# The-Learning-And-Vision-Atelier-LAVA/BUFFER

Measured on AMD Instinct MI355X. Metric: registration pairs/sec, higher is better.
Workload: dtype f32

## Files before the change

buffer_amd/_lib.py:

```python
import ctypes as C
import os

_HERE = os.path.dirname(os.path.abspath(__file__))
LIB_PATH = os.environ.get("BUF_LIB_PATH") or os.path.join(_HERE, "libbuffer_hip.so")

BUF_OK = 0


class BufferHipError(RuntimeError):
    pass


class buf_grid_t(C.Structure):
    _fields_ = [
        ("ws", C.c_void_p), ("ws_bytes", C.c_size_t),
        ("ns", C.c_int), ("nb", C.c_int),
        ("cells_per_elem", C.c_int64),
        ("radius", C.c_float),
        ("supports", C.c_void_p),
        ("desc", C.c_void_p), ("s_off", C.c_void_p), ("table", C.c_void_p),
        ("sorted", C.c_void_p), ("order", C.c_void_p), ("scan_tmp", C.c_void_p),
    ]


class buf_voxel_map_t(C.Structure):
    _fields_ = [
        ("buf", C.c_void_p), ("buf_bytes", C.c_size_t),
        ("nclouds", C.c_int), ("nrows", C.c_int), ("n", C.c_int),
        ("max_cells", C.c_int64),
        ("voxel", C.c_double), ("epsilon", C.c_double),
        ("clouds", C.c_void_p), ("table", C.c_void_p), ("rows", C.c_void_p), ("keys", C.c_void_p), ("row_off", C.c_void_p),
    ]


_lib = None

_vp, _i, _f, _i64, _sz = C.c_void_p, C.c_int, C.c_float, C.c_int64, C.c_size_t

_SIGNATURES = {
    "buf_last_error": (C.c_char_p, []),
    "buf_version": (_i, []),
    "buf_device_count": (_i, []),
    "buf_timing_enable": (None, [_i]),
    "buf_timing_collect": (C.c_longlong, [C.POINTER(C.c_double), C.POINTER(C.c_double)]),
    "buf_timing_collect_kernel": (C.c_longlong, [_i, C.POINTER(C.c_double), C.POINTER(C.c_double)]),
    "buf_grid_default_cells": (_i64, [_i, _i]),
    "buf_grid_ws_bytes": (_sz, [_i, _i, _i64]),
    "buf_grid_cell_dims": (_i, [C.POINTER(C.c_double), _f, _i64, C.POINTER(C.c_double), C.POINTER(C.c_int)]),
    "buf_grid_build": (_i, [C.POINTER(buf_grid_t), _vp, _i, _vp, _i, _f, _i64, _vp, _sz, _vp]),
    "buf_grid_query": (_i, [C.POINTER(buf_grid_t), _vp, _i, _vp, _vp, _f, _i, _vp, _vp, _vp, _vp, _vp]),
    "buf_radius_neighbors": (_i, [_vp, _i, _vp, _i, _vp, _vp, _i, _f, _i, _vp, _vp, _vp, _vp, _sz, _vp]),
    "buf_grid_subsample_ws_bytes": (_sz, [_i, _i, _i64, _i]),
    "buf_grid_subsample_batch": (_i, [_vp, _i, _vp, _i, _f, _i, _vp, _i, _vp, _vp, _vp, _vp, _i64, _vp, _sz, _vp]),
    "buf_fps_ws_bytes": (_sz, [_i, _i]),
    "buf_fps": (_i, [_vp, _i, _i, _i, _vp, _vp, _sz, _vp]),
    "buf_gather": (_i, [_vp, _vp, _i, _i, _i, _i, _vp, _vp]),
    "buf_group": (_i, [_vp, _vp, _i, _i, _i, _i, _i, _vp, _vp]),
    "buf_ball_query": (_i, [_vp, _vp, _i, _i, _i, _f, _i, _vp, _vp]),
    "buf_three_nn": (_i, [_vp, _vp, _i, _i, _i, _vp, _vp, _vp]),
    "buf_select_patches": (_i, [_vp, _vp, _i, _i, _f, _i, _vp, _vp]),
    "buf_select_patches_batched_ws_bytes": (_sz, [_i, _i]),
    "buf_select_patches_batched": (_i, [_vp, _vp, _i, _vp, _i, _f, _i, _vp, _vp, _sz, _vp]),
    "buf_permute_clouds": (_i, [_vp, _vp, _vp, _i, _vp, _vp]),
    "buf_compact_ws_bytes": (_sz, [_i]),
    "buf_compact_greater": (_i, [_vp, _i, _i, _f, _vp, _vp, _vp, _sz, _vp]),
    "buf_knn_ws_bytes": (_sz, [_i, _i, _i]),
    "buf_knn1_ws_bytes": (_sz, [_i, _i, _i]),
    "buf_knn": (_i, [_vp, _vp, _i, _i, _i, _i, _i, _vp, _vp, _vp, _sz, _vp]),
    "buf_fps_ragged": (_i, [_vp, _vp, _i, _i, _vp, _vp, _sz, _vp]),
    "buf_svd3x3_batched": (_i, [_vp, _i, _vp, _vp, _vp, _vp]),
    "buf_vn_gather_block": (_i, [_vp, _vp, _vp, _vp, _i, _i, _i, _i, _i, _i, _f, _vp, _vp, _vp, _vp, _f, _vp, _vp]),
    "buf_vn_gather_pre_supported": (_i, [_i, _i, _i]),
    "buf_vn_gather_pre_ws_bytes": (_sz, [_i, _i]),
    "buf_vn_gather_block_pre": (_i, [_vp, _vp, _vp, _vp, _i, _i, _i, _i, _i, _f, _vp, _vp, _vp, _vp, _f, _vp, _vp, _sz, _vp]),
    "buf_vn_pointwise": (_i, [_vp, _vp, _i, _i, _i, _vp, _i, _i, _i, _vp, _vp, _vp, _vp, _f, _vp, _vp, _vp]),
    "buf_gather_max": (_i, [_vp, _vp, _i, _i, _i, _i, _vp, _vp]),
    "buf_vn_std": (_i, [_vp, _vp, _i, _i, _vp, _vp]),
    "buf_score_head_ws_bytes": (_sz, [_i, _i]),
    "buf_score_head": (_i, [_vp, _i, _vp, _i, _vp, _vp, _vp, _vp, _f, _vp, _vp, _vp, _vp, _f, _vp, _vp, _vp, _vp, _vp, _i, _vp, _vp, _i, _f,
                            _vp, _vp, _sz, _vp]),
    "buf_patch_voxelize_ws_bytes": (_sz, [_i]),
    "buf_patch_voxelize": (_i, [_vp, _vp, _i, _i, _f, _vp, _i, _i, _vp, _f, _i, _vp, _vp, _vp, _vp, _vp, _vp, _vp,
                                _vp, _vp, _sz, _vp]),
    "buf_cylindrical_net_wg": (_i, [_vp, _i, _vp, _vp, _vp, _vp, _vp, _vp, _vp]),
    "buf_cylindrical_net_wg_form": (_i, [_vp, _i, _vp, _vp, _vp, _vp, _vp, _i, _vp, _vp]),
    "buf_cylindrical_net_wg_all": (_i, [_vp, _i, _vp, _vp, _vp, _vp, _vp, _vp, _vp, _vp]),
    "buf_cylindrical_net_wg_all_flags": (_i, [_vp, _vp, _vp, _vp]),
    "buf_cylindrical_net_wg_supports": (_i, [_vp, _vp]),
    "buf_cylindrical_net_wg_flags": (_i, [_vp, _vp, _vp]),
    "buf_cylindrical_net_split_safe": (_i, [_vp, _i, _vp, _vp, _vp, _vp, _vp, _vp, _vp, _vp, _vp, _vp, _vp, _vp]),
    "buf_cylindrical_net_split_safe_form": (_i, [_vp, _i, _vp, _vp, _vp, _vp, _vp, _vp, _i, _vp, _vp, _vp, _vp, _vp, _vp]),
    "buf_cost_volume_net_split_safe": (_i, [_vp, _vp, _i, _vp, _vp, _i, _vp, _vp, _vp, _vp, _vp, _vp, _vp, _vp]),
    "buf_cylindrical_net_split_safe_all": (_i, [_vp, _i, _vp, _vp, _vp, _vp, _vp, _vp, _vp, _vp, _vp, _vp, _vp, _vp, _vp]),
    "buf_cylindrical_net_split": (_i, [_vp, _i, _vp, _vp, _vp, _vp, _vp, _vp, _vp, _vp]),
    "buf_cylindrical_net_split_head": (_i, [_vp, _i, _vp, _vp, _vp, _vp, _vp, _vp, _vp, _vp, _vp, _vp]),
    "buf_split_gemm_count": (C.c_longlong, [_i, _i, _i, _i]),
    "buf_split_tile_gemm": (_i, [_vp, _i, _i, _i, _i, _vp]),
    "buf_cost_volume_net_split": (_i, [_vp, _vp, _i, _vp, _vp, _vp, _vp, _vp]),
    "buf_cost_volume_net_split_gather": (_i, [_vp, _i, _vp, _vp, _i, _vp, _vp, _vp, _vp, _vp]),
    "buf_split_filter_count": (C.c_longlong, [_i, _i]),
    "buf_split_tile_filters": (_i, [_vp, _i, _i, _vp]),
    "buf_winograd_tile_weights": (_i, [_vp, _i, _i, _vp]),
    "buf_winograd_f24_tile_weights": (_i, [_vp, _i, _i, _vp]),
    "buf_winograd_group": (_i, [_i, _i]),
    "buf_cost_winograd_group": (_i, [_i]),
    "buf_winograd_tile_filters": (_i, [_vp, _i, _i, _i, _i, _vp]),
    "buf_voxel_downsample_ws_bytes": (_sz, [_i, _i64]),
    "buf_voxel_downsample": (_i, [_vp, _vp, _i, _i, C.c_double, _vp, _vp, _vp, _i64, _vp, _sz, _vp]),
    "buf_voxel_downsample_batch_ws_bytes": (_sz, [_i, _i, _i64]),
    "buf_voxel_downsample_batch": (_i, [_vp, _i, _i, _vp, _i, C.c_double, _vp, _vp, _i64, _vp, _sz, _vp]),
    "buf_knn_normals": (_i, [_vp, _i, _vp, _i, _vp, _i, _i, _vp, _i, _vp, _vp, _vp]),
    "buf_icp_ws_bytes": (_sz, [_i, _i, _i, _i]),
    "buf_icp_batched": (_i, [_vp, _vp, _vp, _vp, _vp, _i, _i, _f, _vp, _i, C.c_double, C.c_double, _vp, _vp, _vp, _vp, _vp,
                             _vp, _sz, _vp]),
    "buf_gicp_batched": (_i, [_vp, _vp, _vp, _vp, _vp, _vp, _i, _f, C.c_double, _vp, _i, C.c_double, C.c_double, _vp, _vp, _vp, _vp,
                              _vp, _vp, _sz, _vp]),
    "buf_pair_stats_ws_bytes": (_sz, [_i, _i, _i, _i, _i64]),
    "buf_pair_stats": (_i, [_vp, _vp, _i, _vp, _vp, _i, _vp, _f, _i64, _vp, _vp, _vp, _vp, _sz, _vp]),
    "buf_pose_graph_ws_bytes": (_sz, [_i, _i, _i, _i]),
    "buf_pose_graph_optimize": (_i, [_vp, _vp, _i, _vp, _vp, _vp, _vp, _vp, _vp, _vp, _vp, _i, C.c_double, C.c_double, C.c_double,
                                     _vp, _vp, _vp, _vp, _vp, _sz, _vp]),
    "buf_fpfh_ws_bytes": (_sz, [_i]),
    "buf_fpfh": (_i, [_vp, _vp, _i, _vp, _i, _i, _vp, _vp, _vp, _sz, _vp]),
    "buf_fgr_ws_bytes": (_sz, [_i, _i, _i]),
    "buf_fgr_batched": (_i, [_vp, _vp, _vp, _vp, _vp, _vp, _i, _vp, C.c_double, _i, _i, C.c_double, C.c_double, _i, C.c_double, _i, _i,
                             _vp, _vp, _vp, _vp, _vp, _sz, _vp]),
    "buf_sc2_ws_bytes": (_sz, [_vp, _i, _i]),
    "buf_sc2_batched": (_i, [_vp, _vp, _vp, _vp, _vp, _vp, _i, C.c_double, C.c_double, C.c_double, _i, _i, C.c_double, _i, _i,
                             _vp, _vp, _vp, _vp, _vp, _vp, _vp, _vp, _sz, _vp]),
    "buf_clique_ws_bytes": (_sz, [_vp, _i, _i, _i]),
    "buf_clique_batched": (_i, [_vp, _vp, _vp, _vp, _vp, _vp, _i, C.c_double, C.c_double, C.c_double, C.c_double, _i, _i, C.c_double, _i,
                                _i, _vp, _vp, _vp, _vp, _vp, _vp, _vp, _vp, _vp, _vp, _vp, _sz, _vp]),
    "buf_voxel_map_bytes": (_sz, [_i, _i, _i64]),
    "buf_voxel_map_ws_bytes": (_sz, [_i, _i, _i64]),
    "buf_voxel_map_build": (_i, [C.POINTER(buf_voxel_map_t), _vp, _vp, _vp, _i, C.c_double, C.c_double, _i64, _vp, _sz, _vp, _sz, _vp]),
    "buf_voxel_map_export": (_i, [C.POINTER(buf_voxel_map_t), _i, _vp, _vp, _vp, _vp, _vp, _vp]),
    "buf_vgicp_ws_bytes": (_sz, [_i, _i]),
    "buf_vgicp_batched": (_i, [C.POINTER(buf_voxel_map_t), _vp, _vp, _vp, _vp, _i, _i, _vp, _i, C.c_double, C.c_double, _vp, _vp, _vp,
                               _vp, _vp, _vp, _sz, _vp]),
    "buf_match_metrics":(_i, [_vp, _vp, _vp, _i, _i, _vp, _vp, _f, _f, _f, _vp, _vp, _vp]),
    "buf_row_linear": (_i, [_vp, _i, _i, _i, _vp, _vp, _i, _vp, _vp]),
    "buf_segment_instance_norm_ws_bytes": (_sz, [_i, _i]),
    "buf_segment_instance_norm": (_i, [_vp, _i, _i, _vp, _i, _f, _vp, _vp, _sz, _vp]),
    "buf_descriptor_head": (_i, [_vp, _i, _vp, _vp, _vp, _vp]),
    "buf_cost_volume_net": (_i, [_vp, _vp, _i, _vp, _vp, _vp, _vp]),
    "buf_cost_volume_net_gather": (_i, [_vp, _i, _vp, _vp, _i, _vp, _vp, _vp, _vp]),
    "buf_hypotheses_score": (_i, [_vp, _vp, _vp, _vp, _vp, _i, _i, _f, _vp, _vp, _vp, _vp, _vp, _vp]),
    "buf_ransac_ws_bytes": (_sz, [_i]),
    "buf_ransac_kabsch": (_i, [_vp, _vp, _vp, _i, _i, C.c_uint64, _f, _f, _vp, _vp, _vp, _sz, _vp]),
    "buf_ransac_masked_ws_bytes": (_sz, [_i, _i]),
    "buf_ransac_kabsch_masked": (_i, [_vp, _vp, _vp, _i, _i, C.c_uint64, _f, _f, _vp, _vp, _vp, _sz, _vp]),
    "buf_post_refine": (_i, [_vp, _vp, _vp, _i, _f, _i, _vp, _vp, _vp]),
    "buf_recover_poses_ws_bytes": (_sz, [_i, _i, _i]),
    "buf_recover_poses_batched": (_i, [_vp, _vp, _vp, _vp, _vp, _vp, _i, _vp, _i, _f, _i, _f, _f, _f, _i, _vp, _vp, _sz, _vp]),
}


def exported_symbols():
    return sorted(_SIGNATURES)


def lib():
    global _lib
    if _lib is None:
        if not os.path.exists(LIB_PATH):
            raise BufferHipError(
                f"{LIB_PATH} is missing: build it with `python -m buffer_amd.build` "
                "(hipcc --offload-arch=gfx950). buffer_amd has no CPU fallback.")
        import torch
        l = C.CDLL(LIB_PATH)
        for name, (res, args) in _SIGNATURES.items():
            fn = getattr(l, name)
            fn.restype = res
            fn.argtypes = args
        _lib = l
    return _lib


def check(rc, what=""):
    if rc != BUF_OK:
        msg = lib().buf_last_error().decode(errors="replace")
        raise BufferHipError(f"{what} failed ({rc}): {msg}")
```

buffer_amd/csrc/buffer_hip.hip:

```cpp
#include <stdlib.h>
#include "core.hip"
#include "radius.hip"
#include "icp.hip"
#include "pairstats.hip"
#include "posegraph.hip"
#include "metrics.hip"
#include "subsample.hip"
#include "pointops.hip"
#include "vn.hip"
#include "voxelize.hip"
#include "registration.hip"
#include "convnet.hip"
#include "convnet_h3.hip"
#include "costnet_h3.hip"
#include "preprocess.hip"
#include "convnet_wg.hip"
#include "convnet_w24.hip"
#include "convnet_w24k.hip"
#include "convnet_w24p.hip"
#include "convnet_w24a.hip"
#include "costnet.hip"
#include "split_safe.hip"
#include "fpfh.hip"
#include "fgr.hip"
#include "sc2.hip"
#include "clique.hip"
#include "vgicp.hip"
```

buffer_amd/csrc/convnet_w24.hip:

```cpp
#include "common.h"

#define W24_WSTRIDE 768
#define W24_SET_F22(CIN) (16 * 128 * (CIN))

__device__ __forceinline__ void w24_tile(int li, int& ty, int& tx)
{
    const bool last = li == 15;
    ty = last ? 3 : li / 5;
    tx = last ? 4 : li - 5 * ty;
}

__device__ __forceinline__ unsigned w24_row_addr(unsigned act_addr, int a, int li, int lk)
{
    int ty, tx;
    w24_tile(li, ty, tx);
    const int row = 2 * ty - 1 + a;
    return act_addr + 4u * (unsigned)(lk * WG_CS + ((row >= 0 && row <= 6) ? row * WG_ROW + 4 * tx : WG_ZERO));
}

struct W24AddrPark { float a[4]; };
__device__ __forceinline__ void w24_park_addresses(const float* act, int li, int lk, W24AddrPark& pk)
{
    const unsigned act_addr = (unsigned)(size_t)(__attribute__((address_space(3))) const float*)act;
#pragma unroll
    for (int a = 0; a < 4; a++) {
        const unsigned v = w24_row_addr(act_addr, a, li, lk);
        asm volatile("v_accvgpr_write_b32 %0, %1" : "=a"(pk.a[a]) : "v"(v));
    }
}

#define W24_LOAD(DST, A0, A1_, OFS)                                                                       \
    {                                                                                                     \
        _Pragma("unroll") for (int q_ = 0; q_ < 3; q_++) {                                                \
            DST[q_] = *(wg_lds_f2)(size_t)((A0) + (OFS) + 8 * q_);                                        \
            asm volatile("" : "+v"(A0));                                                                  \
        }                                                                                                 \
        _Pragma("unroll") for (int q_ = 0; q_ < 3; q_++) {                                                \
            DST[3 + q_] = *(wg_lds_f2)(size_t)((A1_) + (OFS) + 8 * q_);                                   \
            asm volatile("" : "+v"(A1_));                                                                 \
        }                                                                                                 \
    }

__device__ __forceinline__ wgf2 w24_ldw2(__amdgpu_buffer_rsrc_t rs, unsigned uniform_float_ofs, unsigned lane_byte_ofs)
{
    return __builtin_bit_cast(wgf2, __builtin_amdgcn_raw_buffer_load_b64(rs, lane_byte_ofs, uniform_float_ofs * 4, 0));
}

#define W24_U(n, k, j) ((j) < 3 ? W4[n][k][j] : ((j) == 5 ? W4[n][k][3] : W2[n][k][(j) - 3]))

template <int I, bool PRIMED, int INEXT>
__device__ __forceinline__ void w24_pass(unsigned (&RA)[4], __amdgpu_buffer_rsrc_t rs, unsigned wp, unsigned wp_next, unsigned lofs4, unsigned lofs2,
                                         int niter, wgf4 (&W4)[2][2], wgf2 (&W2)[2][2], wgf4 (&acc)[2][6], wgf2 (&D)[2][6])
{
    constexpr int A1 = wg_a1(I), A2 = wg_a2(I);
    constexpr int A1N = wg_a1(INEXT < 0 ? 0 : INEXT), A2N = wg_a2(INEXT < 0 ? 0 : INEXT);
    float V[2][6];
    unsigned P0 = RA[A1], P1 = RA[A2];
    if constexpr (!PRIMED) {
        W24_LOAD(D[0], P0, P1, 0)
        W24_LOAD(D[1], P0, P1, WG_KSTEP)
    }
#define W24_XFORM(BUF)                                                                                    \
    {                                                                                                     \
        float r_[6];                                                                                      \
        _Pragma("unroll") for (int b = 0; b < 6; b++) {                                                   \
            const float da_ = D[BUF][b >> 1][b & 1];                                                      \
            const float db_ = D[BUF][3 + (b >> 1)][b & 1];                                                \
            r_[b] = I == 1 ? wg_add(da_, db_) : (I == 2 ? wg_sub(db_, da_) : wg_sub(da_, db_));           \
        }                                                                                                 \
        const float c_ = wg_sub(r_[4], r_[2]), e_ = wg_sub(r_[3], r_[1]);                                 \
        const float a_ = __builtin_fmaf(-4.f, r_[2], r_[4]), b_ = __builtin_fmaf(-4.f, r_[1], r_[3]);     \
        V[BUF][0] = __builtin_fmaf(4.f, r_[0], __builtin_fmaf(-4.f, r_[2], c_));                          \
        V[BUF][1] = wg_add(a_, b_); V[BUF][2] = wg_sub(a_, b_);                                           \
        V[BUF][3] = __builtin_fmaf(2.f, e_, c_); V[BUF][4] = __builtin_fmaf(-2.f, e_, c_);                \
        V[BUF][5] = __builtin_fmaf(-4.f, e_, wg_sub(r_[5], r_[3]));                                       \
    }
    W24_XFORM(0)
#pragma unroll 1
    for (int it = 0; it < niter; it++) {
        const bool more = it + 1 < niter;
        const unsigned wcur = wp + 4 * it * W24_WSTRIDE;
        const unsigned wn = more ? wcur + 4 * W24_WSTRIDE : wp_next;
        const unsigned adv = more ? 4u * WG_KSTEP : 0u;
        __builtin_amdgcn_sched_barrier(0);
#pragma unroll
        for (int s = 0; s < 4; s++) {
            if (s < 2) W24_LOAD(D[s & 1], P0, P1, (s + 2) * WG_KSTEP)
            else {
                if (s == 2) { P0 += adv; P1 += adv; }
                if constexpr (INEXT >= 0) {
                    unsigned q0 = more ? P0 : RA[A1N], q1 = more ? P1 : RA[A2N];
                    W24_LOAD(D[s & 1], q0, q1, (s - 2) * WG_KSTEP)
                } else
                    W24_LOAD(D[s & 1], P0, P1, (s - 2) * WG_KSTEP)
            }
            __builtin_amdgcn_sched_barrier(0);
#pragma unroll
            for (int n = 0; n < 2; n++)
#pragma unroll
                for (int j = 0; j < 6; j++)
                    acc[n][j] = __builtin_amdgcn_mfma_f32_16x16x4f32(W24_U(n, s & 1, j), V[s & 1][j], acc[n][j], 0, 0, 0);
            __builtin_amdgcn_sched_barrier(0);
            W24_XFORM((s + 1) & 1)
#pragma unroll
            for (int n = 0; n < 2; n++) {
                const unsigned o = s < 2 ? wcur + (s + 2) * W24_WSTRIDE : wn + (s - 2) * W24_WSTRIDE;
                W4[n][s & 1] = wg_ldw(rs, o + n * 256, lofs4);
                W2[n][s & 1] = w24_ldw2(rs, o + 512 + n * 128, lofs2);
            }
            __builtin_amdgcn_sched_barrier(0);
        }
    }
#undef W24_XFORM
}

template <bool NOBIAS = false>
__device__ __forceinline__ void w24_round(unsigned (&RA)[4], __amdgpu_buffer_rsrc_t rs, unsigned wp, unsigned wp_after, unsigned lofs4, unsigned lofs2,
                                          int niter, unsigned pstride, const float* __restrict__ bias_lane, wgf4 (&W4)[2][2], wgf2 (&W2)[2][2],
                                          wgf4 (&Y)[2][2][4])
{
    using std::integral_constant;
    wgf2 D[2][6];
    wgf4 bv[2];
#pragma unroll
    for (int n = 0; n < 2; n++) {
        if constexpr (NOBIAS) bv[n] = bias_lane ? *reinterpret_cast<const wgf4*>(bias_lane + n * 16) : (wgf4){ 0.f, 0.f, 0.f, 0.f };
        else bv[n] = *reinterpret_cast<const wgf4*>(bias_lane + n * 16);
    }
    wgf4 acc[2][6];
    float zero = 0.f;
    asm volatile("" : "+v"(zero));
#pragma unroll
    for (int n = 0; n < 2; n++)
#pragma unroll
        for (int j = 0; j < 6; j++) acc[n][j] = (wgf4){ zero, zero, zero, zero };
    auto run = [&](auto ic) __attribute__((always_inline)) {
        constexpr int I = decltype(ic)::value;
        constexpr int INEXT = I == 3 ? 0 : I + 1;
        if constexpr (I == 1) {
#pragma unroll
            for (int n = 0; n < 2; n++) acc[n][1] += bv[n];
        }
        constexpr int ICHAIN = (INEXT != 0 && wg_chains(I)) ? INEXT : -1;
        w24_pass<I, wg_chains(I - 1), ICHAIN>(RA, rs, wp + I * pstride, INEXT == 0 ? wp_after : wp + (I + 1) * pstride, lofs4, lofs2, niter, W4, W2, acc, D);
        __builtin_amdgcn_sched_barrier(0);
#pragma unroll
        for (int n = 0; n < 2; n++) {
            wgf4 f[4];
#pragma unroll
            for (int r = 0; r < 4; r++) {
                const float p = acc[n][1][r] + acc[n][2][r], q = acc[n][1][r] - acc[n][2][r];
                const float t = acc[n][3][r] + acc[n][4][r], d = acc[n][3][r] - acc[n][4][r];
                f[0][r] = acc[n][0][r] + p + t;
                f[1][r] = __builtin_fmaf(2.f, d, q);
                f[2][r] = __builtin_fmaf(4.f, t, p);
                f[3][r] = __builtin_fmaf(8.f, d, q) + acc[n][5][r];
            }
#pragma unroll
            for (int v = 0; v < 4; v++) {
                if constexpr (I == 0) Y[n][1][v] = f[v];
                else if constexpr (I == 1) {
#pragma unroll
                    for (int r = 0; r < 4; r++) Y[n][1][v][r] = __builtin_fmaf(2.f, f[v][r], -Y[n][1][v][r]);
                }
                else if constexpr (I == 2) Y[n][0][v] = f[v];
                else Y[n][1][v] -= f[v];
                if constexpr (I == 2) asm volatile("" : "+v"(Y[n][0][v]));
                else asm volatile("" : "+v"(Y[n][1][v]));
            }
        }
    };
    run(integral_constant<int, 0>{});
    run(integral_constant<int, 1>{});
    run(integral_constant<int, 2>{});
    run(integral_constant<int, 3>{});
}

template <bool NOBIAS = false>
__device__ __forceinline__ void w24_round_direct(unsigned row5, __amdgpu_buffer_rsrc_t rs, unsigned wp, unsigned lofs, int niter, unsigned pstride,
                                                 const float* __restrict__ bias_lane, wgf4 (&W4)[2][2], wgf4 (&Y)[2])
{
    constexpr int wstride = W24_WSTRIDE;
    wgf4 Wr[3][2][2];
#pragma unroll
    for (int n = 0; n < 2; n++)
#pragma unroll
        for (int k = 0; k < 2; k++) {
            Wr[0][n][k] = W4[n][k];
            Wr[1][n][k] = wg_ldw(rs, wp + pstride + n * 256 + k * wstride, lofs);
            Wr[2][n][k] = wg_ldw(rs, wp + 2 * pstride + n * 256 + k * wstride, lofs);
        }
    float X[2][6];
    unsigned pa = row5;
    WG_LOADD(X[0], pa, 0)
    WG_LOADD(X[1], pa, WG_KSTEP)
    wgf4 acc[2][3];
    float zero = 0.f;
    asm volatile("" : "+v"(zero));
#pragma unroll
    for (int n = 0; n < 2; n++) {
        acc[n][0] = (wgf4){ zero, zero, zero, zero };
        acc[n][1] = (wgf4){ zero, zero, zero, zero };
        if constexpr (NOBIAS) acc[n][2] = bias_lane ? *reinterpret_cast<const wgf4*>(bias_lane + n * 16) : (wgf4){ zero, zero, zero, zero };
        else acc[n][2] = *reinterpret_cast<const wgf4*>(bias_lane + n * 16);
    }
    float G[2][6];
#define W24_TAPS(SLOT)                                                                                    \
    _Pragma("unroll") for (int n = 0; n < 2; n++) {                                                       \
        const wgf4 u0_ = Wr[0][n][SLOT], u1_ = Wr[1][n][SLOT], u2_ = Wr[2][n][SLOT];                      \
        const float d1_ = wg_sub(u1_[1], u2_[1]), d2_ = wg_sub(u1_[2], u2_[2]);                           \
        G[n][0] = u0_[0]; G[n][1] = wg_sub(u0_[1], u0_[2]); G[n][2] = u0_[3];                             \
        G[n][3] = wg_sub(u1_[0], u2_[0]); G[n][4] = wg_sub(d1_, d2_); G[n][5] = wg_sub(u1_[3], u2_[3]);   \
    }
#define W24_RELOAD(SLOT, OFS)                                                                             \
    _Pragma("unroll") for (int n = 0; n < 2; n++)                                                         \
        _Pragma("unroll") for (int blk = 0; blk < 3; blk++) Wr[blk][n][SLOT] = wg_ldw(rs, (OFS) + blk * pstride + n * 256, lofs);
    W24_TAPS(0)
    W24_RELOAD(0, wp + 2 * wstride)
#pragma unroll 1
    for (int it = 0; it < niter; it++) {
        const bool more = it + 1 < niter;
        const unsigned wcur = wp + 4 * it * wstride;
        const unsigned wn = more ? wcur + 4 * wstride : wp;
        const unsigned adv = more ? 4u * WG_KSTEP : 0u;
        __builtin_amdgcn_sched_barrier(0);
#pragma unroll
        for (int s = 0; s < 4; s++) {
#pragma unroll
            for (int b = 0; b < 3; b++)
#pragma unroll
                for (int a = 0; a < 2; a++)
#pragma unroll
                    for (int n = 0; n < 2; n++)
                        acc[n][b] = __builtin_amdgcn_mfma_f32_16x16x4f32(G[n][a * 3 + b], X[s & 1][a * 3 + b], acc[n][b], 0, 0, 0);
            __builtin_amdgcn_sched_barrier(0);
            if (s < 2) WG_LOADD(X[s & 1], pa, (s + 2) * WG_KSTEP)
            else {
                if (s == 2) pa += adv;
                WG_LOADD(X[s & 1], pa, (s - 2) * WG_KSTEP)
            }
            __builtin_amdgcn_sched_barrier(0);
            W24_TAPS((s + 1) & 1)
            if (s == 0) W24_RELOAD(1, wcur + 3 * wstride)
            else W24_RELOAD((s + 1) & 1, wn + (s - 1) * wstride)
            __builtin_amdgcn_sched_barrier(0);
        }
    }
#undef W24_TAPS
#undef W24_RELOAD
#pragma unroll
    for (int n = 0; n < 2; n++)
#pragma unroll
        for (int r = 0; r < 4; r++) Y[n][r] = __builtin_fmaf(4.f, acc[n][0][r], __builtin_fmaf(-3.f, acc[n][1][r], acc[n][2][r]));
}

__device__ __forceinline__ void w24_store_tile(const wgf4 (&Yt)[2][4], int nt, int relu, float* __restrict__ act, int li, int lk)
{
    const int n0 = nt * 16 + lk * 4;
    const float lo = relu ? 0.f : -__builtin_inff();
    int ty, tx;
    w24_tile(li, ty, tx);
#pragma unroll
    for (int u = 0; u < 2; u++) {
        const int row = 2 * ty + u;
        const bool ok = row < 7;
        int pos[4];
#pragma unroll
        for (int v = 0; v < 4; v++) pos[v] = ok ? row * WG_ROW + 4 * tx + 1 + v : WG_ZERO + 4;
        const int h0 = (ok && tx == 0) ? row * WG_ROW + 21 : WG_ZERO + 4;
        const int h1 = (ok && tx == 4) ? row * WG_ROW : WG_ZERO + 5;
        float* p = act + n0 * WG_CS;
#pragma unroll
        for (int r = 0; r < 4; r++) {
            float val[4];
#pragma unroll
            for (int v = 0; v < 4; v++) { val[v] = fmaxf(Yt[u][v][r], lo); p[r * WG_CS + pos[v]] = val[v]; }
            p[r * WG_CS + h0] = val[0]; p[r * WG_CS + h1] = val[3];
        }
    }
}

__device__ __forceinline__ void w24_layer_pair(float* __restrict__ act, const float* __restrict__ wt, const float* __restrict__ bias, int cin, int relu,
                                               int pair, const WgAddrPark& pk, const W24AddrPark& pk24)
{
    act[(threadIdx.x >> 1) * WG_CS + WG_ZERO + 4 + (threadIdx.x & 1)] = 0.f;
    __syncthreads();
    int lane = threadIdx.x & (WAVE - 1);
    asm volatile("" : "+v"(lane));
    const int lk = lane >> 4;
    const int k4 = cin >> 2;
    unsigned RA[4];
#pragma unroll
    for (int a = 0; a < 4; a++) asm volatile("v_accvgpr_read_b32 %0, %1" : "=v"(RA[a]) : "a"(pk24.a[a]));
    const unsigned row5 = wg_parked(pk, 2, 0);
    const __amdgpu_buffer_rsrc_t rs = wg_weights(wt);
    const unsigned pstride = (unsigned)(k4 * W24_WSTRIDE);
    const unsigned wp = (unsigned)pair * 4 * pstride;
    const unsigned lofs4 = lane * 16, lofs2 = lane * 8;
    const float* bv = bias + (2 * pair) * 16 + lk * 4;
    wgf4 W4[2][2];
    wgf2 W2[2][2];
#pragma unroll
    for (int n = 0; n < 2; n++)
#pragma unroll
        for (int k = 0; k < 2; k++) {
            W4[n][k] = wg_ldw(rs, wp + k * W24_WSTRIDE + n * 256, lofs4);
            W2[n][k] = w24_ldw2(rs, wp + k * W24_WSTRIDE + 512 + n * 128, lofs2);
        }
    wgf4 Y[2][2][4];
    float park[2][36];
    w24_round(RA, rs, wp, wp, lofs4, lofs2, k4 >> 2, pstride, bv, W4, W2, Y);
#pragma unroll
    for (int n = 0; n < 2; n++)
#pragma unroll
        for (int q = 0; q < 32; q++) asm volatile("v_accvgpr_write_b32 %0, %1" : "=a"(park[n][q]) : "v"(Y[n][q >> 4][(q >> 2) & 3][q & 3]));
    wgf4 Yb[2];
    w24_round_direct(row5, rs, wp, lofs4, k4 >> 2, pstride, bv, W4, Yb);
#pragma unroll
    for (int n = 0; n < 2; n++)
#pragma unroll
        for (int q = 0; q < 4; q++) asm volatile("v_accvgpr_write_b32 %0, %1" : "=a"(park[n][32 + q]) : "v"(Yb[n][q]));
    __syncthreads();
    int lane_s = threadIdx.x & (WAVE - 1);
    asm volatile("" : "+v"(lane_s));
#pragma unroll
    for (int n = 0; n < 2; n++) {
#pragma unroll
        for (int q = 0; q < 32; q++) asm volatile("v_accvgpr_read_b32 %0, %1" : "=v"(Y[n][q >> 4][(q >> 2) & 3][q & 3]) : "a"(park[n][q]));
#pragma unroll
        for (int q = 0; q < 4; q++) asm volatile("v_accvgpr_read_b32 %0, %1" : "=v"(Yb[n][q]) : "a"(park[n][32 + q]));
        w24_store_tile(Y[n], 2 * pair + n, relu, act, lane_s & 15, lane_s >> 4);
        wg_store_row6<false>(Yb[n], 2 * pair + n, relu, act, nullptr, lane_s & 15, lane_s >> 4);
    }
}

__device__ __forceinline__ void cyl_net_w24_body(const float* __restrict__ x, const CylWgParams& P, float* __restrict__ y, float* __restrict__ lds)
{
    float* act = lds;
    const int patch = blockIdx.x;
    const int w = __builtin_amdgcn_readfirstlane(threadIdx.x / WAVE);
    wg_load_input(x, P, act, patch);
    WgAddrPark pk;
    W24AddrPark pk24;
    {
        int lane0 = threadIdx.x & (WAVE - 1);
        asm volatile("" : "+v"(lane0));
        wg_park_addresses(act, lane0 & 15, lane0 >> 4, pk);
        w24_park_addresses(act, lane0 & 15, lane0 >> 4, pk24);
    }
#pragma unroll 1
    for (int l = 0; l < WG_LAYERS; l++) {
        const int cin = P.cin[l], cout = P.cout[l];
        if (cout == 128) w24_layer_pair(act, P.wt[l], P.bias[l], cin, P.relu[l], w, pk, pk24);
        else if (cout == 64) wg_layer_msplit(act, P.wt[l], P.bias[l], cin, cout, P.relu[l], w, pk);
        else if (l < WG_LAYERS - 1) wg_layer_mksplit<false>(act, nullptr, P.wt[l], P.bias[l], cin, cout, P.relu[l], w, pk);
        else wg_layer_mksplit<true>(act, y + (size_t)patch * cout * 140, P.wt[l], P.bias[l], cin, cout, P.relu[l], w, pk);
        __syncthreads();
    }
}

__global__ void __launch_bounds__(WG_THREADS, 2) k_cyl_net_w24(const float* __restrict__ x, CylWgParams P, float* __restrict__ y)
{
    extern __shared__ float lds[];
    cyl_net_w24_body(x, P, y, lds);
}

__global__ void __launch_bounds__(WG_THREADS, 2) k_cyl_net_w24_rerun(const float* __restrict__ x, CylWgParams P, float* __restrict__ y)
{
    extern __shared__ float lds[];
    if (P.only_if[blockIdx.x] == 0) return;
    cyl_net_w24_body(x, P, y, lds);
}

extern "C" int buf_winograd_f24_tile_weights(const float* w_host, int cout, int cin, float* out_host)
{
    BUF_REQUIRE(w_host && out_host, BUF_EINVAL, "buf_winograd_f24_tile_weights: null argument");
    BUF_REQUIRE(cout > 0 && cin > 0 && cout % 32 == 0 && cin % 4 == 0, BUF_EINVAL, "buf_winograd_f24_tile_weights: widths %d -> %d", cin, cout);
    static const double G2[4][3] = { { 1, 0, 0 }, { .5, .5, .5 }, { .5, -.5, .5 }, { 0, 0, 1 } };
    const double s6 = 1.0 / 6, s12 = 1.0 / 12, s24 = 1.0 / 24;
    const double G4[6][3] = { { .25, 0, 0 }, { -s6, -s6, -s6 }, { -s6, s6, -s6 }, { s24, s12, s6 }, { s24, -s12, s6 }, { 0, 0, 1 } };
    const int k4 = cin / 4;
    for (int o = 0; o < cout; o++)
        for (int c = 0; c < cin; c++) {
            const float* g = w_host + ((size_t)o * cin + c) * 9;
            const int n = o / 16, lane = (c % 4) * 16 + o % 16;
            for (int i = 0; i < 4; i++) {
                float* blk = out_host + (((size_t)(n / 2) * 4 + i) * k4 + c / 4) * W24_WSTRIDE;
                for (int j = 0; j < 6; j++) {
                    double u = 0;
                    for (int a = 0; a < 3; a++)
                        for (int b = 0; b < 3; b++) u += G2[i][a] * (double)g[3 * a + b] * G4[j][b];
                    if (j == 3 || j == 4) blk[512 + (n % 2) * 128 + lane * 2 + (j - 3)] = (float)u;
                    else blk[(n % 2) * 256 + lane * 4 + (j == 5 ? 3 : j)] = (float)u;
                }
            }
        }
    return BUF_OK;
}

static int w24_check_flags(const int* cin, const int* cout, const int* relu)
{
    for (int l = 0; l < WG_LAYERS; l++) {
        BUF_REQUIRE(relu[l] >= 0 && relu[l] <= (BUF_CYL_F24K | WG_F24_FLAG | 1), BUF_EINVAL,
                    "buf_cylindrical_net_wg: layer %d has the relu word %d (bit 0: ReLU, bits 1 and 2: the F(2x4) flags, nothing above)", l, relu[l]);
        BUF_REQUIRE(!(relu[l] & BUF_CYL_F24K) || (cout[l] == 64 && cin[l] % 64 == 0), BUF_EINVAL,
                    "buf_cylindrical_net_wg: the K-split F(2x4) flag (bit 2) goes only on layers with 64 output channels and Cin %% 64 == 0 "
                    "(layer %d: %d -> %d, flags %d)", l, cin[l], cout[l], relu[l]);
        BUF_REQUIRE(((relu[l] & WG_F24_FLAG) != 0) == (cout[l] == 128), BUF_EINVAL,
                    "buf_cylindrical_net_wg: the F(2x4) flag goes on every layer with 128 output channels and on no other (layer %d: %d -> %d, flags %d)",
                    l, cin[l], cout[l], relu[l]);
    }
    return BUF_OK;
}

extern "C" int buf_cylindrical_net_wg_flags(const int* cin_host, const int* cout_host, const int* relu_host)
{
    BUF_REQUIRE(cin_host && cout_host && relu_host, BUF_EINVAL, "buf_cylindrical_net_wg_flags: null argument");
    if (int rc = wg_check_widths(cin_host, cout_host)) return rc;
    for (int l = 0; l < WG_LAYERS; l++)
        if (relu_host[l] >= 2) return w24_check_flags(cin_host, cout_host, relu_host);
    return BUF_OK;
}

#define BUF_CYL_FORM_LIBRARY BUF_CYL_FORM_PASS_SPLIT
static int w24k_launch(const float* x, int npatch, CylWgParams P, float* y, void* stream);
static int w24p_launch(const float* x, int npatch, CylWgParams P, float* y, void* stream);
static int w24_launch(const float* x, int npatch, CylWgParams P, float* y, void* stream, int form)
{
    if (int rc = w24_check_flags(P.cin, P.cout, P.relu)) return rc;
    bool ksplit = false;
    for (int l = 0; l < WG_LAYERS; l++) {
        if (P.relu[l] & WG_F24_FLAG) P.wt[l] += W24_SET_F22(P.cin[l]);
        ksplit |= (P.relu[l] & BUF_CYL_F24K) != 0;
        P.relu[l] &= ~WG_F24_FLAG;
    }
    if (form == BUF_CYL_FORM_DEFAULT) form = BUF_CYL_FORM_LIBRARY;
    if (ksplit) return form == BUF_CYL_FORM_PASS_SPLIT ? w24p_launch(x, npatch, P, y, stream) : w24k_launch(x, npatch, P, y, stream);
    size_t lds = sizeof(float) * WG_BUF;
    static LdsGrant grant, grant_rerun;
    if (int rc = P.only_if ? grant_dynamic_lds((const void*)k_cyl_net_w24_rerun, lds, grant_rerun) : grant_dynamic_lds((const void*)k_cyl_net_w24, lds, grant)) return rc;
    double macs = 0;
    for (int l = 0; l < WG_LAYERS; l++) macs += 9.0 * P.cin[l] * P.cout[l];
    TimedSpan span;
    bool timed = !P.only_if && timing_begin((hipStream_t)stream, &span, 2.0 * 140 * macs * npatch, BUF_TIMED_CYL_NET);
    if (P.only_if) k_cyl_net_w24_rerun<<<npatch, WG_THREADS, lds, (hipStream_t)stream>>>(x, P, y);
    else k_cyl_net_w24<<<npatch, WG_THREADS, lds, (hipStream_t)stream>>>(x, P, y);
    if (timed) timing_end((hipStream_t)stream, &span);
    BUF_LAUNCH_CHECK();
    return BUF_OK;
}
```

buffer_amd/csrc/costnet.hip:

```cpp
#include "common.h"
#include <type_traits>

#define CV_THREADS 256
#define CV_BUF 20480
#define CV_LAYERS 10
#define CV_C32 36
#define CV_C64 68
#define CV_C128 132

typedef float cvx4 __attribute__((ext_vector_type(4)));

#define CV_SCHED_TAIL(NMFMA, NMEM)                                                      \
    _Pragma("unroll") for (int i_ = 0; i_ < (NMFMA); i_++) {                            \
        __builtin_amdgcn_sched_group_barrier(0x008, 1, 0);                              \
        __builtin_amdgcn_sched_group_barrier(0x006, 4, 0);                              \
        __builtin_amdgcn_sched_group_barrier(0x120, ((NMEM) + (NMFMA) - 1) / (NMFMA), 0); \
    }
typedef const __attribute__((address_space(1))) cvx4* cv_gptr;

struct CostNetParams {
    const float* wt[CV_LAYERS];
    const float* bias[CV_LAYERS];
    const long long* s_rows;
    const long long* t_rows;
    int row_floats, chan_floats, skip_floats;
    const int* only_if;
};

template <int MT, int NT, int D, int TOTAL, typename Loader>
__device__ __forceinline__ void cv_gemm_static(cvx4 (&acc)[MT][NT], Loader& L, const float* __restrict__ wl, int ntot)
{
    float a[D][4][MT], b[D][4][NT];
#define CVS_LOAD(SLOT, G)                                                                                 \
    {                                                                                                     \
                           \
        cv_gptr wg_ = (cv_gptr)(wl + (size_t)(G) * ntot * 256);                                           \
        asm volatile("" : "+v"(wg_));                                                                     \
        _Pragma("unroll") for (int u = 0; u < NT; u++) {                                                  \
            const cvx4 bv_ = wg_[u * 64];                                                                 \
            _Pragma("unroll") for (int p = 0; p < 4; p++) b[SLOT][p][u] = bv_[p];                         \
        }                                                                                                 \
        L.load(a[SLOT], (G));                                                                             \
    }
#pragma unroll
    for (int i = 0; i < D - 1; i++) CVS_LOAD(i, i)
#pragma unroll
    for (int g = 0; g < TOTAL; g++) {
        __builtin_amdgcn_sched_barrier(0);
        if (g + D - 1 < TOTAL) CVS_LOAD((g + D - 1) % D, g + D - 1)
#pragma unroll
        for (int p = 0; p < 4; p++)
#pragma unroll
            for (int t = 0; t < MT; t++)
#pragma unroll
                for (int u = 0; u < NT; u++)
                    acc[t][u] = __builtin_amdgcn_mfma_f32_16x16x4f32(a[g % D][p][t], b[g % D][p][u], acc[t][u], 0, 0, 0);
        CV_SCHED_TAIL(4 * MT * NT, MT + NT)
    }
#undef CVS_LOAD
}

#define CVA_SP 0
#define CVA_TP 4320
#define CVA_SM 16376
#define CVA_TB 18536
#define CVA_XC 0
#define CW_RSX 18
#define CW_CSX 112
#define CVA_XCH (96 * CW_CSX)
static_assert(CVA_XCH + 2 * 8 * 64 * 4 <= CVA_SM, "the exchange slots fit between the chunk and the layer-0 maps");

struct SLoader {
    const float* base;
    __device__ __forceinline__ void load(float (&a)[4][1], int g) const
    {
        const int tap = g >> 1, cg = g & 1, dk = tap / 5, e2 = tap - dk * 5;
        const cvx4 v = *reinterpret_cast<const cvx4*>(base + (dk * 24 + e2) * CV_C32 + cg * 16);
#pragma unroll
        for (int p = 0; p < 4; p++) a[p][0] = v[p];
    }
};

struct TLoader {
    const float* base;
    __device__ __forceinline__ void load(float (&a)[4][1], int g) const
    {
        const int tap = g >> 1, cg = g & 1, dk = tap / 3, dl = tap - dk * 3;
        const cvx4 v = *reinterpret_cast<const cvx4*>(base + (dk * 20 + dl) * CV_C32 + cg * 16);
#pragma unroll
        for (int p = 0; p < 4; p++) a[p][0] = v[p];
    }
};

template <int MT, int NT, int CIN, int COUT, int WIN, int KW, bool INPLACE>
__device__ __forceinline__ void cv_conv_layer(const float* in, float* out, const float* __restrict__ wt,
                                              const float* __restrict__ bias, int nt0, bool relu)
{
    constexpr int WOUT = WIN - KW + 1, P = WOUT * WOUT, GPT = CIN / 16, TAPS = KW * KW, NTOT = COUT / 16;
    constexpr int CSI = CIN + 4, CSO = COUT + 4;
    static_assert(GPT % 2 == 0, "two pipeline slots alternate per channel group");
    int lane = threadIdx.x & (WAVE - 1);
    asm volatile("" : "+v"(lane));
    const int li = lane & 15, lk = lane >> 4;
    const float* pa[MT];
#pragma unroll
    for (int t = 0; t < MT; t++) {
        int m = t * 16 + li;
        m = m < P ? m : P - 1;
        pa[t] = in + ((m / WOUT) * WIN + (m % WOUT)) * CSI + lk * 4;
    }
    const float* wl = wt + ((size_t)nt0 * 64 + lane) * 4;
    cvx4 acc[MT][NT];
#pragma unroll
    for (int u = 0; u < NT; u++) {
        const float bv = bias[(nt0 + u) * 16 + li];
#pragma unroll
        for (int t = 0; t < MT; t++) acc[t][u] = (cvx4){ bv, bv, bv, bv };
    }
    float a[2][4][MT], b[2][4][NT];
#define CVC_LOAD(SLOT, PTRS, WTAP, CG)                                                                    \
    {                                                                                                     \
        cv_gptr wg_ = (cv_gptr)((WTAP) + (size_t)(CG) * NTOT * 256);                                      \
        asm volatile("" : "+v"(wg_));                                                                     \
        _Pragma("unroll") for (int u = 0; u < NT; u++) {                                                  \
            const cvx4 bv_ = wg_[u * 64];                                                                 \
            _Pragma("unroll") for (int p = 0; p < 4; p++) b[SLOT][p][u] = bv_[p];                         \
        }                                                                                                 \
        _Pragma("unroll") for (int t = 0; t < MT; t++) {                                                  \
            const cvx4 av_ = *reinterpret_cast<const cvx4*>(PTRS[t] + (CG) * 16);                         \
            _Pragma("unroll") for (int p = 0; p < 4; p++) a[SLOT][p][t] = av_[p];                         \
        }                                                                                                 \
    }
    const float* cur[MT];
    const float* nxt[MT];
#pragma unroll
    for (int t = 0; t < MT; t++) cur[t] = pa[t];
    const float* wcur = wl;
    CVC_LOAD(0, cur, wcur, 0)
#pragma unroll 1
    for (int tap = 0; tap < TAPS; tap++) {
        const int tn = tap + 1 < TAPS ? tap + 1 : tap;
        const int offn = ((tn / KW) * WIN + (tn % KW)) * CSI;
#pragma unroll
        for (int t = 0; t < MT; t++) nxt[t] = pa[t] + offn;
        const float* wnxt = wl + (size_t)tn * GPT * NTOT * 256;
#pragma unroll
        for (int cg = 0; cg < GPT; cg++) {
            __builtin_amdgcn_sched_barrier(0);
            if (cg + 1 < GPT) CVC_LOAD((cg + 1) & 1, cur, wcur, cg + 1)
            else              CVC_LOAD((cg + 1) & 1, nxt, wnxt, 0)
    #pragma unroll
            for (int p = 0; p < 4; p++)
#pragma unroll
                for (int t = 0; t < MT; t++)
#pragma unroll
                    for (int u = 0; u < NT; u++)
                        acc[t][u] = __builtin_amdgcn_mfma_f32_16x16x4f32(a[cg & 1][p][t], b[cg & 1][p][u], acc[t][u], 0, 0, 0);
            CV_SCHED_TAIL(4 * MT * NT, MT + NT)
        }
#pragma unroll
        for (int t = 0; t < MT; t++) cur[t] = nxt[t];
        wcur = wnxt;
    }
#undef CVC_LOAD
    if constexpr (INPLACE) __syncthreads();
#pragma unroll
    for (int u = 0; u < NT; u++) {
        const int n = (nt0 + u) * 16 + li;
#pragma unroll
        for (int t = 0; t < MT; t++)
#pragma unroll
            for (int r = 0; r < 4; r++) {
                const int m = t * 16 + lk * 4 + r;
                float v = acc[t][u][r];
                if (relu) v = fmaxf(v, 0.f);
                if (m < P) out[m * CSO + n] = v;
            }
    }
}

template <int HIN, int TYPM>
__device__ __forceinline__ bool cw_tile(int t, int li, int& ty, int& tx)
{
    constexpr int NTY = (HIN - 2) / 2;
    const int q = li / NTY;
    ty = t * TYPM + q; tx = li - q * NTY;
    return q < TYPM && ty < NTY;
}

template <int HIN, int TYPM, int RSO, int CSO, bool POSMAJOR>
__device__ __forceinline__ void cw_store_tile(const wgf4 (&Yt)[2][2], int t, int nt, float* __restrict__ out, int li, int lk)
{
    int ty, tx;
    if (!cw_tile<HIN, TYPM>(t, li, ty, tx)) return;
    const int n0 = nt * 16 + lk * 4;
#pragma unroll
    for (int u = 0; u < 2; u++) {
        const int row = 2 * ty + u, col = 2 * tx;
        if constexpr (POSMAJOR) {
#pragma unroll
            for (int v = 0; v < 2; v++) {
                wgf4 y;
#pragma unroll
                for (int r = 0; r < 4; r++) y[r] = fmaxf(Yt[u][v][r], 0.f);
                *reinterpret_cast<wgf4*>(out + (row * (HIN - 2) + col + v) * CSO + n0) = y;
            }
        } else {
#pragma unroll
            for (int r = 0; r < 4; r++)
                *reinterpret_cast<wgf2*>(out + (n0 + r) * CSO + row * RSO + col) = (wgf2){ fmaxf(Yt[u][0][r], 0.f), fmaxf(Yt[u][1][r], 0.f) };
        }
    }
}

template <int HIN, int RS, int CS, int TYPM, int CIN, int NN, int MT, int MT2, int RSO, int CSO, bool POSMAJOR>
__device__ __forceinline__ void cw_layer(float* __restrict__ map, const float* __restrict__ wt, const float* __restrict__ bias, int ng, int t0)
{
    static_assert(MT >= 1 && MT <= 2 && MT2 >= 0 && MT2 <= 1 && RS % 2 == 0 && CS % 2 == 0, "");
    constexpr unsigned KSTEP = 16u * CS;
    constexpr int k4 = CIN / 4, wstride = 256 * NN;
    int lane = threadIdx.x & (WAVE - 1);
    asm volatile("" : "+v"(lane));
    const int li = lane & 15, lk = lane >> 4;
    const unsigned base = (unsigned)(size_t)(__attribute__((address_space(3))) const float*)map;
    auto rows = [&](int t, unsigned (&ra)[4]) __attribute__((always_inline)) {
        int ty, tx;
        if (!cw_tile<HIN, TYPM>(t, li, ty, tx)) { ty = 0; tx = 0; }
#pragma unroll
        for (int a = 0; a < 4; a++) ra[a] = base + 4u * (unsigned)(lk * CS + (2 * ty + a) * RS + 2 * tx);
    };
    unsigned RA[3][4];
    rows(t0, RA[0]);
    rows(t0 + (MT > 1 ? 1 : 0), RA[1]);
    rows(t0, RA[2]);
    const __amdgpu_buffer_rsrc_t rs = wg_weights(wt);
    const unsigned wp = (unsigned)ng * (CIN * NN * 256);
    const unsigned lofs = lane * 16;
    const float* bl = bias + ng * NN * 16 + lk * 4;
    wgf4 W[NN][2];
    wg_first_weights<NN, 0, 2>(rs, wp, lofs, wstride, W);
    wgf4 Y[NN][3][2][2];
    wg_round<NN, 0, MT, KSTEP, true>(RA, rs, wp, wp, lofs, k4 >> 2, wstride, (unsigned)(k4 * wstride), bl, W, Y);
    wgf4 Y2[NN][3][2][2];
    if constexpr (MT2 > 0) {
        rows(t0 + MT, RA[0]);
        wg_round<NN, 0, 1, KSTEP, true>(RA, rs, wp, wp, lofs, k4 >> 2, wstride, (unsigned)(k4 * wstride), bl, W, Y2);
    }
    __syncthreads();
#pragma unroll
    for (int n = 0; n < NN; n++) {
#pragma unroll
        for (int t = 0; t < MT; t++) cw_store_tile<HIN, TYPM, RSO, CSO, POSMAJOR>(Y[n][t], t0 + t, ng * NN + n, map, li, lk);
        if constexpr (MT2 > 0) cw_store_tile<HIN, TYPM, RSO, CSO, POSMAJOR>(Y2[n][0], t0 + MT, ng * NN + n, map, li, lk);
    }
}
#define CW_CS1 272
#define CW_CS2 208
#define CW_CS3 160

__device__ __forceinline__ void form_rows_cm(float* __restrict__ X, const float* __restrict__ SM, const float* __restrict__ TB, int r0)
{
    for (int i = threadIdx.x; i < 6 * 54 * 8; i += CV_THREADS) {
        const int c4 = i & 7, rem = i >> 3, t = rem / 54, pos = rem - t * 54;
        const int kq = pos / 18, lq = pos - kq * 18;
        int j = lq - (r0 + t);
        j = j < 0 ? j + 20 : j;
        const cvx4 sv = *reinterpret_cast<const cvx4*>(SM + (kq * 20 + j) * CV_C32 + c4 * 4);
        const cvx4 tv = *reinterpret_cast<const cvx4*>(TB + pos * CV_C32 + c4 * 4);
        float* d = X + (kq * 32 + c4 * 4) * CW_CSX + t * CW_RSX + lq;
#pragma unroll
        for (int q = 0; q < 4; q++) d[q * CW_CSX] = fmaxf(sv[q] + tv[q], 0.f);
    }
}

#ifdef CV_STAMP
__device__ long long* cv_stamp_ptr;
#define CV_STAMP_AT(SLOT) if (threadIdx.x == 0) cv_stamp_ptr[(size_t)blockIdx.x * 16 + (SLOT)] = __builtin_amdgcn_s_memtime();
#else
#define CV_STAMP_AT(SLOT)
#endif

__device__ __forceinline__ void cost_net_body(const float* __restrict__ s_eq, const float* __restrict__ t_eq, const CostNetParams& P,
                                              float* __restrict__ ind_out, float* __restrict__ lds)
{
    float* bufA = lds;
    float* bufB = lds;
    float* SP = bufB + CVA_SP;
    float* TP = bufB + CVA_TP;
    float* SM = bufB + CVA_SM;
    float* TB = bufB + CVA_TB;
    const int match = blockIdx.x;
    const int tid = threadIdx.x, lane = tid & (WAVE - 1), li = lane & 15, lk = lane >> 4;
    const int w = __builtin_amdgcn_readfirstlane(tid / WAVE);
    {
        const float* a = s_eq + (P.s_rows ? (size_t)P.s_rows[match] * P.row_floats + P.skip_floats : (size_t)match * 3200);
        const float* b = t_eq + (P.t_rows ? (size_t)P.t_rows[match] * P.row_floats + P.skip_floats : (size_t)match * 3200);
        for (int i = tid; i < 800; i += CV_THREADS) {
            const int c = i / 25, rem = i - c * 25, k = rem / 5, l0 = (rem - k * 5) * 4;
            const cvx4 sv = __builtin_nontemporal_load(reinterpret_cast<const cvx4*>(a + c * P.chan_floats + rem * 4));
            const cvx4 tv = __builtin_nontemporal_load(reinterpret_cast<const cvx4*>(b + c * P.chan_floats + rem * 4));
#pragma unroll
            for (int q = 0; q < 4; q++) {
                const int l = l0 + q;
                SP[(k * 24 + l + 2) * CV_C32 + c] = sv[q];
                if (l >= 18) SP[(k * 24 + l - 18) * CV_C32 + c] = sv[q];
                if (l < 2) SP[(k * 24 + l + 22) * CV_C32 + c] = sv[q];
                TP[(k * 20 + l) * CV_C32 + c] = tv[q];
            }
        }
    }
    __syncthreads();
    CV_STAMP_AT(0)

    {
        const float b0v[2] = { P.bias[0][li], P.bias[0][16 + li] };
        int ms = w * 16 + li, mt = ms;
        ms = ms < 60 ? ms : 59;
        mt = mt < 54 ? mt : 53;
        SLoader LS;
        LS.base = SP + ((ms / 20) * 24 + ms % 20) * CV_C32 + lk * 4;
        TLoader LT;
        LT.base = TP + ((mt / 18) * 20 + mt % 18) * CV_C32 + lk * 4;
        cvx4 accS[1][2] = { { (cvx4){ 0.f, 0.f, 0.f, 0.f }, (cvx4){ 0.f, 0.f, 0.f, 0.f } } };
        cvx4 accT[1][2] = { { (cvx4){ 0.f, 0.f, 0.f, 0.f }, (cvx4){ 0.f, 0.f, 0.f, 0.f } } };
        cv_gemm_static<1, 2, 4, 30>(accS, LS, P.wt[0] + (size_t)lane * 4, 2);
        cv_gemm_static<1, 2, 4, 18>(accT, LT, P.wt[0] + (size_t)30 * 2 * 256 + (size_t)lane * 4, 2);
#pragma unroll
        for (int u = 0; u < 2; u++)
#pragma unroll
            for (int r = 0; r < 4; r++) {
                const int m = w * 16 + lk * 4 + r;
                if (m < 60) SM[m * CV_C32 + u * 16 + li] = accS[0][u][r];
                if (m < 54) TB[m * CV_C32 + u * 16 + li] = b0v[u] - accT[0][u][r];
            }
    }
    __syncthreads();
    CV_STAMP_AT(1)

    {
        int lane_ = threadIdx.x & (WAVE - 1);
        asm volatile("" : "+v"(lane_));
        const int li_ = lane_ & 15, lk_ = lane_ >> 4;
        const int p_ = w & 1, kh = w >> 1;
        float* XC = bufB + CVA_XC;
        constexpr unsigned KSTEP = 16u * CW_CSX;
        const __amdgpu_buffer_rsrc_t rs = wg_weights(P.wt[1]);
        const unsigned wp = (unsigned)p_ * (96 * 512) + (unsigned)(12 * kh) * 512;
        const unsigned lofs = lane_ * 16;
        unsigned RA[3][4];
        {
            const unsigned base = (unsigned)(size_t)(__attribute__((address_space(3))) const float*)XC + (unsigned)(12 * kh) * KSTEP;
#pragma unroll
            for (int a = 0; a < 4; a++) RA[0][a] = RA[1][a] = RA[2][a] = base + 4u * (unsigned)(lk_ * CW_CSX + (2 * (li_ >> 3) + a) * CW_RSX + 2 * (li_ & 7));
        }
        const float* bl = kh ? nullptr : P.bias[1] + p_ * 32 + lk_ * 4;
        wgf4 W[2][2];
        wg_first_weights<2, 0, 2>(rs, wp, lofs, 512, W);
        wgf4* slot = reinterpret_cast<wgf4*>(bufB + CVA_XCH) + (size_t)p_ * 8 * WAVE + lane_;
        wgf4 Yown[2][2][3][2][2];
#pragma unroll
        for (int j = 0; j < 4; j++) {
            form_rows_cm(XC, SM, TB, 4 * j);
            __syncthreads();
            wgf4 Yt[2][3][2][2];
            wg_round<2, 0, 1, KSTEP, true>(RA, rs, wp, wp, lofs, 3, 512, 24u * 512u, bl, W, Yt);
            const bool own = (j < 2) == (kh == 0);
            if (!own) {
#pragma unroll
                for (int q = 0; q < 8; q++) slot[q * WAVE] = Yt[q >> 2][0][(q >> 1) & 1][q & 1];
            }
            __syncthreads();
            if (own) {
#pragma unroll
                for (int q = 0; q < 8; q++) Yown[j & 1][q >> 2][0][(q >> 1) & 1][q & 1] = Yt[q >> 2][0][(q >> 1) & 1][q & 1] + slot[q * WAVE];
            }
        }
        __syncthreads();
#pragma unroll
        for (int jj = 0; jj < 2; jj++)
#pragma unroll
            for (int n = 0; n < 2; n++)
                cw_store_tile<18, 2, 16, CW_CS1, false>(Yown[jj][n][0], 2 * kh + jj, 2 * p_ + n, bufA, li_, lk_);
        __syncthreads();
        CV_STAMP_AT(2)
    }
    cw_layer<16, 16, CW_CS1, 2, 64, 2, 2, 0, 14, CW_CS2, false>(bufA, P.wt[2], P.bias[2], w & 1, 2 * (w >> 1));
    __syncthreads();
    CV_STAMP_AT(3)
    cw_layer<14, 14, CW_CS2, 2, 64, 2, 2, 1, 12, CW_CS3, false>(bufA, P.wt[3], P.bias[3], w, 0);
    __syncthreads();
    CV_STAMP_AT(4)
    cw_layer<12, 12, CW_CS3, 3, 128, 2, 2, 0, 12, CW_CS3, false>(bufA, P.wt[4], P.bias[4], w, 0);
    __syncthreads();
    CV_STAMP_AT(5)
    cw_layer<10, 12, CW_CS3, 4, 128, 1, 1, 0, 0, CV_C64, true>(bufA, P.wt[5], P.bias[5], w, 0);
    __syncthreads();
    CV_STAMP_AT(6)
    cv_conv_layer<3, 1, 64, 64, 8, 3, true>(bufA, bufA, P.wt[6], P.bias[6], w, true);
    __syncthreads();
    CV_STAMP_AT(7)
    float* hop1 = lds + 4096;
    float* hop2 = lds + 8192;
    float* hop3 = lds + 12288;
    if (w < 2) cv_conv_layer<1, 1, 64, 32, 6, 3, false>(bufA, hop1, P.wt[7], P.bias[7], w, true);
    __syncthreads();
    if (w < 2) cv_conv_layer<1, 1, 32, 32, 4, 3, false>(hop1, hop2, P.wt[8], P.bias[8], w, true);
    __syncthreads();
    if (w < 2) cv_conv_layer<1, 1, 32, 32, 2, 2, false>(hop2, hop3, P.wt[9], P.bias[9], w, false);
    __syncthreads();
    CV_STAMP_AT(8)
    if (w == 0) {
        float v = lane < 20 ? hop3[lane] : -3.4e38f;
        float mx = v;
        for (int d = WAVE / 2; d > 0; d >>= 1) mx = fmaxf(mx, __shfl_xor(mx, d, WAVE));
        float e = lane < 20 ? expf(v - mx) : 0.f;
        float se = e, sw = e * (float)lane;
        for (int d = WAVE / 2; d > 0; d >>= 1) { se += __shfl_xor(se, d, WAVE); sw += __shfl_xor(sw, d, WAVE); }
        if (lane == 0) ind_out[match] = sw / se;
    }
}

__global__ void __launch_bounds__(CV_THREADS, 2) k_cost_net(const float* __restrict__ s_eq, const float* __restrict__ t_eq, CostNetParams P,
                                                        float* __restrict__ ind_out)
{
    extern __shared__ float lds[];
    cost_net_body(s_eq, t_eq, P, ind_out, lds);
}

__global__ void __launch_bounds__(CV_THREADS, 2) k_cost_net_rerun(const float* __restrict__ s_eq, const float* __restrict__ t_eq, CostNetParams P,
                                                              float* __restrict__ ind_out)
{
    extern __shared__ float lds[];
    if (P.only_if[blockIdx.x] == 0) return;
    cost_net_body(s_eq, t_eq, P, ind_out, lds);
}

extern "C" int buf_cost_winograd_group(int layer)
{
    static const int group[6] = { 0, 2, 2, 2, 2, 1 };
    return layer >= 0 && layer <= 5 ? group[layer] : 0;
}

static int cost_net_launch(const float* s_eq, const float* t_eq, int m, const float* const* wt_host, const float* const* bias_host,
                           const long long* s_rows, const long long* t_rows, int ele_n, float* ind_out, void* stream, const char* who,
                           const int* only_if = nullptr)
{
    CostNetParams P;
    for (int l = 0; l < CV_LAYERS; l++) {
        P.wt[l] = wt_host[l]; P.bias[l] = bias_host[l];
        BUF_REQUIRE(P.wt[l] && P.bias[l], BUF_EINVAL, "%s: null weights for layer %d", who, l);
    }
    P.s_rows = s_rows; P.t_rows = t_rows;
    P.chan_floats = s_rows ? ele_n * 20 : 100;
    P.row_floats = 32 * P.chan_floats;
    P.skip_floats = s_rows ? 20 : 0;
    P.only_if = only_if;
    size_t lds = sizeof(float) * CV_BUF;
    static LdsGrant grant, grant_rerun;
    if (int rc = only_if ? grant_dynamic_lds((const void*)k_cost_net_rerun, lds, grant_rerun) : grant_dynamic_lds((const void*)k_cost_net, lds, grant)) return rc;
    static const double macs_per_match =
        60.0 * 480 * 32 + 54.0 * 288 * 32 + 16.0 * 64 * 96 * 64 +
        16.0 * (49.0 * 64 * 64 + 36.0 * 64 * 128 + 25.0 * 128 * 128 + 16.0 * 128 * 64) +
        36.0 * 576 * 64 + 16.0 * 576 * 32 + 4.0 * 288 * 32 + 1.0 * 128 * 20;
    TimedSpan span;
    bool timed = !only_if && timing_begin((hipStream_t)stream, &span, 2.0 * macs_per_match * m, BUF_TIMED_COST_NET);
#ifdef CV_STAMP
    long long* stamps = nullptr;
    BUF_CHECK_HIP(hipMalloc(&stamps, (size_t)m * 16 * sizeof(long long)));
    BUF_CHECK_HIP(hipMemcpyToSymbol(HIP_SYMBOL(cv_stamp_ptr), &stamps, sizeof(stamps)));
#endif
    if (only_if) k_cost_net_rerun<<<m, CV_THREADS, lds, (hipStream_t)stream>>>(s_eq, t_eq, P, ind_out);
    else k_cost_net<<<m, CV_THREADS, lds, (hipStream_t)stream>>>(s_eq, t_eq, P, ind_out);
    if (timed) timing_end((hipStream_t)stream, &span);
    BUF_LAUNCH_CHECK();
#ifdef CV_STAMP
    if (m >= 2048) {
        BUF_CHECK_HIP(hipStreamSynchronize((hipStream_t)stream));
        long long* h = (long long*)malloc((size_t)m * 16 * sizeof(long long));
        BUF_CHECK_HIP(hipMemcpy(h, stamps, (size_t)m * 16 * sizeof(long long), hipMemcpyDeviceToHost));
        static const char* name[8] = { "A.1 (layer 0 maps)", "A.2 (layer 1)", "layer 2", "layer 3", "layer 4", "layer 5", "layer 6", "layers 7-9" };
        double d[8] = {};
        for (int b = m / 2; b < m; b++)
            for (int i = 0; i < 8; i++) d[i] += (double)(h[(size_t)b * 16 + i + 1] - h[(size_t)b * 16 + i]);
        for (int i = 0; i < 8; i++) fprintf(stderr, "  CV_STAMP %-20s %8.0f cycles per match\n", name[i], d[i] / (m - m / 2));
        free(h);
    }
    (void)hipFree(stamps);
#endif
    return BUF_OK;
}

extern "C" int buf_cost_volume_net(const float* s_eq, const float* t_eq, int m, const float* const* wt_host,
                                   const float* const* bias_host, float* ind_out, void* stream)
{
    BUF_REQUIRE(m >= 0, BUF_EINVAL, "buf_cost_volume_net: m=%d", m);
    if (m == 0) return BUF_OK;
    BUF_REQUIRE(s_eq && t_eq && wt_host && bias_host && ind_out, BUF_EINVAL, "buf_cost_volume_net: null argument");
    return cost_net_launch(s_eq, t_eq, m, wt_host, bias_host, nullptr, nullptr, 7, ind_out, stream, "buf_cost_volume_net");
}

extern "C" int buf_cost_volume_net_gather(const float* equi, int ele_n, const long long* s_rows, const long long* t_rows, int m,
                                          const float* const* wt_host, const float* const* bias_host, float* ind_out, void* stream)
{
    BUF_REQUIRE(m >= 0 && ele_n == 7, BUF_EINVAL, "buf_cost_volume_net_gather: m=%d ele_n=%d (the kernel is built for ele_n = 7)", m, ele_n);
    if (m == 0) return BUF_OK;
    BUF_REQUIRE(equi && s_rows && t_rows && wt_host && bias_host && ind_out, BUF_EINVAL, "buf_cost_volume_net_gather: null argument");
    return cost_net_launch(equi, equi, m, wt_host, bias_host, s_rows, t_rows, ele_n, ind_out, stream, "buf_cost_volume_net_gather");
}
```

buffer_amd/csrc/split_safe.hip:

```cpp
#include "common.h"

extern "C" int buf_cylindrical_net_split_safe_form(const float* x, int npatch, const void* const* wt_split_host, const float* const* wt_wg_host,
                                                   const float* const* bias_host, const int* cin_host, const int* cout_host, const int* relu_host,
                                                   int form, const float* head_params, float* y_or_equi, float* desc, int* status_dev,
                                                   int* flags_ws, void* stream)
{
    BUF_REQUIRE(npatch >= 0, BUF_EINVAL, "buf_cylindrical_net_split_safe: npatch=%d", npatch);
    if (npatch == 0) return BUF_OK;
    BUF_REQUIRE(x && y_or_equi && flags_ws && wt_split_host && wt_wg_host && bias_host && cin_host && cout_host && relu_host, BUF_EINVAL,
                "buf_cylindrical_net_split_safe: null argument");
    BUF_REQUIRE(!head_params || desc, BUF_EINVAL, "buf_cylindrical_net_split_safe: head without desc");
    BUF_REQUIRE(form >= BUF_CYL_FORM_DEFAULT && form <= BUF_CYL_FORM_PASS_SPLIT, BUF_EINVAL,
                "buf_cylindrical_net_split_safe: form=%d (-1: the library's default, 0: K split, 1: pass split)", form);
    if (int rc = buf_cylindrical_net_wg_flags(cin_host, cout_host, relu_host)) return rc;
    hipStream_t s = (hipStream_t)stream;
    BUF_CHECK_HIP(hipMemsetAsync(flags_ws, 0, sizeof(int) * (size_t)npatch, s));
    int relu_split[WG_LAYERS];
    for (int l = 0; l < WG_LAYERS; l++) relu_split[l] = wg_f24_flagged(relu_host[l]) ? (relu_host[l] & 1) : relu_host[l];
    int rc = h3_launch(x, npatch, wt_split_host, bias_host, cin_host, cout_host, relu_split, head_params ? nullptr : y_or_equi, head_params,
                       desc, head_params ? y_or_equi : nullptr, status_dev, stream, flags_ws);
    if (rc) return rc;
    rc = wg_launch(x, npatch, wt_wg_host, bias_host, cin_host, cout_host, relu_host, y_or_equi, flags_ws, stream, form);
    if (rc) return rc;
    if (head_params) {
        k_desc_head_masked<<<npatch, DH_THREADS, 0, s>>>(y_or_equi, head_params, desc, y_or_equi, flags_ws);
        BUF_LAUNCH_CHECK();
    }
    return BUF_OK;
}

extern "C" int buf_cylindrical_net_split_safe(const float* x, int npatch, const void* const* wt_split_host, const float* const* wt_wg_host,
                                              const float* const* bias_host, const int* cin_host, const int* cout_host, const int* relu_host,
                                              const float* head_params, float* y_or_equi, float* desc, int* status_dev, int* flags_ws,
                                              void* stream)
{
    return buf_cylindrical_net_split_safe_form(x, npatch, wt_split_host, wt_wg_host, bias_host, cin_host, cout_host, relu_host, BUF_CYL_FORM_DEFAULT,
                                               head_params, y_or_equi, desc, status_dev, flags_ws, stream);
}

extern "C" int buf_cylindrical_net_split_safe_all(const float* x, int npatch, const void* const* wt_split_host, const float* const* wt_wg_host,
                                                  const float* const* bias_host, const int* cin_host, const int* cout_host, const int* relu_host,
                                                  const float* const* wt24_host, const float* head_params, float* y_or_equi, float* desc,
                                                  int* status_dev, int* flags_ws, void* stream)
{
    BUF_REQUIRE(npatch >= 0, BUF_EINVAL, "buf_cylindrical_net_split_safe_all: npatch=%d", npatch);
    if (npatch == 0) return BUF_OK;
    BUF_REQUIRE(x && y_or_equi && flags_ws && wt_split_host, BUF_EINVAL, "buf_cylindrical_net_split_safe_all: null argument");
    BUF_REQUIRE(!head_params || desc, BUF_EINVAL, "buf_cylindrical_net_split_safe_all: head without desc");
    CylWgParams P;
    if (int rc = w24a_prepare(wt_wg_host, bias_host, cin_host, cout_host, relu_host, wt24_host, P)) return rc;
    hipStream_t s = (hipStream_t)stream;
    BUF_CHECK_HIP(hipMemsetAsync(flags_ws, 0, sizeof(int) * (size_t)npatch, s));
    int relu_split[WG_LAYERS];
    for (int l = 0; l < WG_LAYERS; l++) relu_split[l] = relu_host[l] & 1;
    int rc = h3_launch(x, npatch, wt_split_host, bias_host, cin_host, cout_host, relu_split, head_params ? nullptr : y_or_equi, head_params,
                       desc, head_params ? y_or_equi : nullptr, status_dev, stream, flags_ws);
    if (rc) return rc;
    P.only_if = flags_ws;
    rc = w24a_launch(x, npatch, P, y_or_equi, stream);
    if (rc) return rc;
    if (head_params) {
        k_desc_head_masked<<<npatch, DH_THREADS, 0, s>>>(y_or_equi, head_params, desc, y_or_equi, flags_ws);
        BUF_LAUNCH_CHECK();
    }
    return BUF_OK;
}

extern "C" int buf_cost_volume_net_split_safe(const float* s_eq, const float* t_eq, int ele_n, const long long* s_rows, const long long* t_rows,
                                              int m, const void* const* wt_split_host, const float* const* bias_split_host,
                                              const float* const* wt_f32_host, const float* const* bias_f32_host, float* ind_out,
                                              int* status_dev, int* flags_ws, void* stream)
{
    BUF_REQUIRE(m >= 0, BUF_EINVAL, "buf_cost_volume_net_split_safe: m=%d", m);
    if (m == 0) return BUF_OK;
    BUF_REQUIRE(s_eq && t_eq && wt_split_host && bias_split_host && wt_f32_host && bias_f32_host && ind_out && flags_ws, BUF_EINVAL,
                "buf_cost_volume_net_split_safe: null argument");
    BUF_REQUIRE((s_rows == nullptr) == (t_rows == nullptr), BUF_EINVAL, "buf_cost_volume_net_split_safe: one row list without the other");
    BUF_REQUIRE(!s_rows || ele_n == 7, BUF_EINVAL, "buf_cost_volume_net_split_safe: ele_n=%d (the kernels are built for ele_n = 7)", ele_n);
    hipStream_t s = (hipStream_t)stream;
    BUF_CHECK_HIP(hipMemsetAsync(flags_ws, 0, sizeof(int) * (size_t)m, s));
    int rc = cost_net_h3_launch(s_eq, t_eq, m, wt_split_host, bias_split_host, s_rows, t_rows, ele_n, ind_out, status_dev, stream,
                                "buf_cost_volume_net_split_safe", flags_ws);
    if (rc) return rc;
    return cost_net_launch(s_eq, t_eq, m, wt_f32_host, bias_f32_host, s_rows, t_rows, ele_n, ind_out, stream, "buf_cost_volume_net_split_safe", flags_ws);
}
```

buffer_amd/ops.py:

```python
import ctypes as C
import time
import os
import numpy as np
import torch

from . import _lib
from ._lib import buf_grid_t, check


def _stream():
    return C.c_void_p(torch.cuda.current_stream().cuda_stream)


def _dev(t, dtype, what):
    if not isinstance(t, torch.Tensor) or not t.is_cuda:
        raise _lib.BufferHipError(f"{what}: expected a tensor in device memory (buffer_amd has no CPU path)")
    if t.dtype != dtype:
        t = t.to(dtype)
    return t.contiguous()


def _ptr(t):
    return C.c_void_p(t.data_ptr()) if t is not None else C.c_void_p(0)


def _host_i32(a):
    if isinstance(a, torch.Tensor):
        a = a.detach().cpu().numpy()
    return np.ascontiguousarray(a, dtype=np.int32).reshape(-1)


def _hptr(a):
    return C.c_void_p(a.ctypes.data)


class CellGrid:

    def __init__(self, supports, s_lengths, radius, cells_per_elem=0):
        L = _lib.lib()
        self.supports = _dev(supports, torch.float32, "CellGrid.supports")
        if self.supports.dim() != 2 or self.supports.shape[1] != 3:
            raise _lib.BufferHipError("Wrong dimensions : support.shape is not (N, 3)")
        self.s_lengths = _host_i32(s_lengths)
        self.ns = int(self.supports.shape[0])
        self.nb = int(self.s_lengths.shape[0])
        self.radius = float(radius)
        if cells_per_elem <= 0:
            cells_per_elem = L.buf_grid_default_cells(self.ns, self.nb)
            f = int(os.environ.get('BUF_GRID_CELLS_PER_POINT', 0))
            if f > 0:
                per = (self.ns + self.nb - 1) // max(self.nb, 1)
                cells_per_elem = min(cells_per_elem, f * per + 65536)
        nbytes = L.buf_grid_ws_bytes(self.ns, self.nb, cells_per_elem)
        self.ws = torch.empty(nbytes, dtype=torch.uint8, device=self.supports.device)
        self.g = buf_grid_t()
        check(L.buf_grid_build(C.byref(self.g), _ptr(self.supports), self.ns, _hptr(self.s_lengths), self.nb,
                               self.radius, cells_per_elem, _ptr(self.ws), nbytes, _stream()), "buf_grid_build")

    @property
    def order(self):
        n = max(self.ns, 1)
        off = self.g.order - self.ws.data_ptr()
        return self.ws[off:off + 4 * n].view(torch.int32)[:self.ns]

    def query(self, queries, q_lengths, k, radius=None, q_order=None, counts=False, max_count=None):
        L = _lib.lib()
        queries = _dev(queries, torch.float32, "CellGrid.query")
        if queries.dim() != 2 or queries.shape[1] != 3:
            raise _lib.BufferHipError("Wrong dimensions : query.shape is not (N, 3)")
        q_lengths = _host_i32(q_lengths)
        if q_lengths.shape[0] != self.nb:
            raise _lib.BufferHipError("Wrong number of batch elements: different for queries and supports ")
        nq = int(queries.shape[0])
        out = torch.empty((nq, k), dtype=torch.int32, device=queries.device)
        cnt = torch.empty((nq,), dtype=torch.int32, device=queries.device) if counts else None
        if q_order is not None:
            q_order = _dev(q_order, torch.int32, "q_order")
        r = self.radius if radius is None else float(radius)
        todo = torch.empty((max(nq, 1),), dtype=torch.int32, device=queries.device) if (k > 0 or q_order is not None) else None
        check(L.buf_grid_query(C.byref(self.g), _ptr(queries), nq, _hptr(q_lengths), _ptr(q_order), r, int(k),
                               _ptr(out), _ptr(cnt), _ptr(max_count), _ptr(todo), _stream()), "buf_grid_query")
        return (out, cnt) if counts else out


def radius_neighbors(queries, supports, q_lengths, s_lengths, radius, k=None):
    grid = CellGrid(supports, s_lengths, radius)
    if k is None:
        mc = torch.zeros(1, dtype=torch.int32, device=grid.supports.device)
        grid.query(queries, q_lengths, 0, max_count=mc)
        k = int(mc.item())
    return grid.query(queries, q_lengths, k)


def grid_cell_dims(ext, radius, cells_per_elem):
    e = (C.c_double * 3)(*[float(v) for v in ext])
    edge, dim = C.c_double(), (C.c_int * 3)()
    check(_lib.lib().buf_grid_cell_dims(e, float(radius), int(cells_per_elem), C.byref(edge), dim), "buf_grid_cell_dims")
    return edge.value, tuple(dim)


HOST_WAIT_S = [0.0]


def grid_subsample_batch(points, lengths, dl, max_p=0, max_cells=0, features=None):
    L = _lib.lib()
    points = _dev(points, torch.float32, "grid_subsample_batch.points")
    if points.dim() != 2 or points.shape[1] != 3:
        raise _lib.BufferHipError("Wrong dimensions : points.shape is not (N, 3)")
    lengths = _host_i32(lengths)
    n, nb = int(points.shape[0]), int(lengths.shape[0])
    if max_cells <= 0:
        max_cells = max(1 << 16, int(os.environ.get('BUF_VOX_CELLS_PER_POINT', 4)) * n, 2 * nb)
    fd = 0
    out_f = None
    if features is not None:
        features = _dev(features, torch.float32, "grid_subsample_batch.features")
        fd = int(features.shape[1])
        out_f = torch.empty((max(n, 1), fd), dtype=torch.float32, device=points.device)
    nbytes = L.buf_grid_subsample_ws_bytes(n, nb, max_cells, fd)
    ws = torch.empty(nbytes, dtype=torch.uint8, device=points.device)
    out = torch.empty((max(n, 1), 3), dtype=torch.float32, device=points.device)
    out_b = np.zeros(nb, np.int32)
    m = C.c_int(0)
    t0 = time.perf_counter()
    check(L.buf_grid_subsample_batch(_ptr(points), n, _hptr(lengths), nb, float(dl), int(max_p), _ptr(features), fd,
                                     _ptr(out), _ptr(out_f), _hptr(out_b), C.byref(m), max_cells, _ptr(ws), nbytes,
                                     _stream()), "buf_grid_subsample_batch")
    HOST_WAIT_S[0] += time.perf_counter() - t0
    if features is not None:
        return out[:m.value], out_b, out_f[:m.value]
    return out[:m.value], out_b


def furthest_point_sample(xyz, npoint):
    L = _lib.lib()
    xyz = _dev(xyz, torch.float32, "furthest_point_sample")
    b, n, _ = xyz.shape
    out = torch.empty((b, npoint), dtype=torch.int32, device=xyz.device)
    nbytes = L.buf_fps_ws_bytes(b, n)
    ws = torch.empty(nbytes, dtype=torch.uint8, device=xyz.device)
    check(L.buf_fps(_ptr(xyz), b, n, int(npoint), _ptr(out), _ptr(ws), nbytes, _stream()), "buf_fps")
    return out


def furthest_point_sample_ragged(xyz, lengths, npoint):
    L = _lib.lib()
    xyz = _dev(xyz, torch.float32, "furthest_point_sample_ragged")
    lengths = _host_i32(lengths)
    b = int(lengths.shape[0])
    out = torch.empty((b, npoint), dtype=torch.int32, device=xyz.device)
    nbytes = L.buf_fps_ws_bytes(1, int(xyz.shape[0]))
    ws = torch.empty(nbytes, dtype=torch.uint8, device=xyz.device)
    check(L.buf_fps_ragged(_ptr(xyz), _hptr(lengths), b, int(npoint), _ptr(out), _ptr(ws), nbytes, _stream()),
          "buf_fps_ragged")
    return out


def gather_operation(feat, idx):
    L = _lib.lib()
    feat, idx = _dev(feat, torch.float32, "gather_operation"), _dev(idx, torch.int32, "gather_operation")
    b, c, n = feat.shape
    m = idx.shape[1]
    out = torch.empty((b, c, m), dtype=torch.float32, device=feat.device)
    check(L.buf_gather(_ptr(feat), _ptr(idx), b, c, n, m, _ptr(out), _stream()), "buf_gather")
    return out


def grouping_operation(feat, idx):
    L = _lib.lib()
    feat, idx = _dev(feat, torch.float32, "grouping_operation"), _dev(idx, torch.int32, "grouping_operation")
    b, c, n = feat.shape
    _, m, s = idx.shape
    out = torch.empty((b, c, m, s), dtype=torch.float32, device=feat.device)
    check(L.buf_group(_ptr(feat), _ptr(idx), b, c, n, m, s, _ptr(out), _stream()), "buf_group")
    return out


def ball_query(radius, nsample, xyz, new_xyz):
    L = _lib.lib()
    xyz, new_xyz = _dev(xyz, torch.float32, "ball_query"), _dev(new_xyz, torch.float32, "ball_query")
    b, n, _ = xyz.shape
    m = new_xyz.shape[1]
    out = torch.zeros((b, m, nsample), dtype=torch.int32, device=xyz.device)
    check(L.buf_ball_query(_ptr(xyz), _ptr(new_xyz), b, n, m, float(radius), int(nsample), _ptr(out), _stream()),
          "buf_ball_query")
    return out


def three_nn(unknown, known):
    L = _lib.lib()
    unknown, known = _dev(unknown, torch.float32, "three_nn"), _dev(known, torch.float32, "three_nn")
    b, n, _ = unknown.shape
    m = known.shape[1]
    dist = torch.empty((b, n, 3), dtype=torch.float32, device=unknown.device)
    idx = torch.empty((b, n, 3), dtype=torch.int32, device=unknown.device)
    check(L.buf_three_nn(_ptr(unknown), _ptr(known), b, n, m, _ptr(dist), _ptr(idx), _stream()), "buf_three_nn")
    return dist, idx


def select_patches(pts, kpts, radius, nsample, out=None):
    L = _lib.lib()
    pts, kpts = _dev(pts, torch.float32, "select_patches"), _dev(kpts, torch.float32, "select_patches")
    if out is None:
        out = torch.empty((kpts.shape[0], nsample, 3), dtype=torch.float32, device=pts.device)
    elif not out.is_contiguous() or tuple(out.shape) != (kpts.shape[0], nsample, 3):
        raise _lib.BufferHipError("select_patches: out must be a contiguous [P,nsample,3] tensor")
    check(L.buf_select_patches(_ptr(pts), _ptr(kpts), pts.shape[0], kpts.shape[0], float(radius), int(nsample),
                               _ptr(out), _stream()), "buf_select_patches")
    return out


_MASK64 = (1 << 64) - 1


def perm_key(seed, cloud):
    x = ((int(seed) * 2 + int(cloud)) * 0x9E3779B97F4A7C15 + 0xD1B54A32D192ED03) & _MASK64
    x = ((x ^ (x >> 30)) * 0xBF58476D1CE4E5B9) & _MASK64
    x = ((x ^ (x >> 27)) * 0x94D049BB133111EB) & _MASK64
    return x ^ (x >> 31)


def permute_clouds(clouds, keys):
    L = _lib.lib()
    clouds = [_dev(c, torch.float32, "permute_clouds") for c in clouds]
    lens = np.array([c.shape[0] for c in clouds], np.int32)
    out = torch.empty((int(lens.sum()), 3), dtype=torch.float32, device=clouds[0].device)
    nc = len(clouds)
    ptrs = (C.c_void_p * nc)(*[c.data_ptr() for c in clouds])
    ks = (C.c_ulonglong * nc)(*[int(k) & _MASK64 for k in keys])
    check(L.buf_permute_clouds(ptrs, _hptr(lens), ks, nc, _ptr(out), _stream()), "buf_permute_clouds")
    return out, lens


def select_patches_batched(sup, lengths, kpts, m, radius, nsample, out=None):
    L = _lib.lib()
    sup = _dev(sup, torch.float32, "select_patches_batched.sup")
    kpts = _dev(kpts, torch.float32, "select_patches_batched.kpts")
    lengths = _host_i32(lengths)
    nc = int(lengths.shape[0])
    if kpts.shape[0] != nc * m:
        raise _lib.BufferHipError(f"select_patches_batched: {kpts.shape[0]} keypoints for {nc} clouds x {m}")
    if out is None:
        out = torch.empty((nc * m, nsample, 3), dtype=torch.float32, device=sup.device)
    nbytes = L.buf_select_patches_batched_ws_bytes(int(sup.shape[0]), nc)
    ws = torch.empty(nbytes, dtype=torch.uint8, device=sup.device)
    check(L.buf_select_patches_batched(_ptr(sup), _hptr(lengths), nc, _ptr(kpts), int(m), float(radius), int(nsample), _ptr(out),
                                       _ptr(ws), nbytes, _stream()), "buf_select_patches_batched")
    return out


def compact_greater(x, threshold):
    L = _lib.lib()
    x = _dev(x, torch.float32, "compact_greater").reshape(-1)
    n = int(x.shape[0])
    idx = torch.empty((max(n, 1),), dtype=torch.int32, device=x.device)
    cnt = torch.zeros((1,), dtype=torch.int32, device=x.device)
    nbytes = L.buf_compact_ws_bytes(n)
    ws = torch.empty(nbytes, dtype=torch.uint8, device=x.device)
    check(L.buf_compact_greater(_ptr(x), 1, n, float(threshold), _ptr(idx), _ptr(cnt), _ptr(ws), nbytes, _stream()),
          "buf_compact_greater")
    return idx[:int(cnt.item())]


def knn(ref, query, k):
    L = _lib.lib()
    ref, query = _dev(ref, torch.float32, "knn"), _dev(query, torch.float32, "knn")
    b, n, d = ref.shape
    q = query.shape[1]
    dist = torch.empty((b, q, k), dtype=torch.float32, device=ref.device)
    idx = torch.empty((b, q, k), dtype=torch.int64, device=ref.device)
    nbytes = L.buf_knn1_ws_bytes(b, n, q) if (int(k) == 1 and d == 32 and n > 0) else L.buf_knn_ws_bytes(b, q, int(k))
    ws = torch.empty(nbytes, dtype=torch.uint8, device=ref.device)
    check(L.buf_knn(_ptr(ref), _ptr(query), b, n, q, d, int(k), _ptr(dist), _ptr(idx), _ptr(ws), nbytes, _stream()),
          "buf_knn")
    return dist, idx


def svd3x3(a):
    L = _lib.lib()
    a = _dev(a, torch.float32, "svd3x3")
    n = a.shape[0]
    u, v = torch.empty_like(a), torch.empty_like(a)
    s = torch.empty((n, 3), dtype=torch.float32, device=a.device)
    check(L.buf_svd3x3_batched(_ptr(a), n, _ptr(u), _ptr(s), _ptr(v), _stream()), "buf_svd3x3_batched")
    return u, s, v


class VnLayer:

    def __init__(self, W, prefix, device, slope=0.2, linear_only=False):
        if linear_only:
            self.wf = torch.as_tensor(W[prefix + '.weight'], dtype=torch.float32, device=device).contiguous()
            self.wd = self.bsc = self.bsh = None
        else:
            self.wf = torch.as_tensor(W[prefix + '.map_to_feat.weight'], dtype=torch.float32, device=device).contiguous()
            self.wd = torch.as_tensor(W[prefix + '.map_to_dir.weight'], dtype=torch.float32, device=device).contiguous()
            self.bsc = self.bsh = None
            if self.wf.shape[0] != 1:
                g = np.asarray(W[prefix + '.batchnorm.bn.weight'], np.float64)
                b = np.asarray(W[prefix + '.batchnorm.bn.bias'], np.float64)
                m = np.asarray(W[prefix + '.batchnorm.bn.running_mean'], np.float64)
                v = np.asarray(W[prefix + '.batchnorm.bn.running_var'], np.float64)
                sc = g / np.sqrt(v + 1e-5)
                self.bsc = torch.tensor(sc, dtype=torch.float32, device=device)
                self.bsh = torch.tensor(b - m * sc, dtype=torch.float32, device=device)
        self.cout, self.cin = int(self.wf.shape[0]), int(self.wf.shape[1])
        self.slope = float(slope)


PF_BYTES = [0.0]


def vn_gather_block(layer, q_pts, s_pts, feats, idx, mode, scale=1.0):
    L = _lib.lib()
    nq, k = idx.shape
    ns = s_pts.shape[0]
    cin = feats.shape[1] // 3
    out = torch.empty((nq, 3 * layer.cout), dtype=torch.float32, device=feats.device)
    if int(mode) == 1 and not os.environ.get('BUF_VN_GATHER_DIRECT') and L.buf_vn_gather_pre_supported(k, cin, layer.cout):
        wsb = L.buf_vn_gather_pre_ws_bytes(ns, layer.cout)
        ws = torch.empty((wsb,), dtype=torch.uint8, device=feats.device)
        PF_BYTES[0] += 48.0 * layer.cout * ns
        check(L.buf_vn_gather_block_pre(_ptr(q_pts), _ptr(s_pts), _ptr(feats), _ptr(idx), nq, ns, k, cin, layer.cout, float(scale),
                                        _ptr(layer.wf), _ptr(layer.wd), _ptr(layer.bsc), _ptr(layer.bsh), layer.slope, _ptr(out),
                                        _ptr(ws), wsb, _stream()), "buf_vn_gather_block_pre")
        return out
    check(L.buf_vn_gather_block(_ptr(q_pts), _ptr(s_pts), _ptr(feats), _ptr(idx), nq, ns, k, cin, layer.cout, int(mode),
                                float(scale), _ptr(layer.wf), _ptr(layer.wd), _ptr(layer.bsc), _ptr(layer.bsh),
                                layer.slope, _ptr(out), _stream()), "buf_vn_gather_block")
    return out


def vn_pointwise(layer, b, a=None, ind_a=None, residual=None):
    L = _lib.lib()
    n = b.shape[0] if b is not None else (ind_a.shape[0] if ind_a is not None else a.shape[0])
    ca = a.shape[1] // 3 if a is not None else 0
    cb = b.shape[1] // 3 if b is not None else 0
    dev = (b if b is not None else a).device
    out = torch.empty((n, 3 * layer.cout), dtype=torch.float32, device=dev)
    stride = ind_a.shape[1] if ind_a is not None else 0
    check(L.buf_vn_pointwise(_ptr(a), _ptr(ind_a), stride, a.shape[0] if a is not None else 0, ca, _ptr(b), cb, n,
                             layer.cout, _ptr(layer.wf), _ptr(layer.wd), _ptr(layer.bsc), _ptr(layer.bsh), layer.slope,
                             _ptr(residual), _ptr(out), _stream()), "buf_vn_pointwise")
    return out


def gather_max(feats, idx):
    L = _lib.lib()
    nq, k = idx.shape
    out = torch.empty((nq, feats.shape[1]), dtype=torch.float32, device=feats.device)
    check(L.buf_gather_max(_ptr(feats), _ptr(idx), nq, feats.shape[0], k, feats.shape[1], _ptr(out), _stream()),
          "buf_gather_max")
    return out


def vn_std(x, z):
    L = _lib.lib()
    n, c = x.shape[0], x.shape[1] // 3
    out = torch.empty((n, 3 * c), dtype=torch.float32, device=x.device)
    check(L.buf_vn_std(_ptr(x), _ptr(z), n, c, _ptr(out), _stream()), "buf_vn_std")
    return out


def patch_voxelize(patches, axis, des_r, centres, azi_cs, voxel_r, nsample, mlp_w, mlp_b, bn_scale, bn_shift,
                   azi_n=20, want_patches=False):
    L = _lib.lib()
    P, S, _ = patches.shape
    nc = centres.shape[0]
    dev = patches.device
    x = torch.empty((P, 16, nc), dtype=torch.float32, device=dev)
    R = torch.empty((P, 3, 3), dtype=torch.float32, device=dev)
    ra = torch.empty((P, 3), dtype=torch.float32, device=dev)
    pn = torch.empty((P, S, 3), dtype=torch.float32, device=dev) if want_patches else None
    hw = [np.ascontiguousarray(a, dtype=np.float32) for a in (mlp_w, mlp_b, bn_scale, bn_shift)]
    wsb = L.buf_patch_voxelize_ws_bytes(nc)
    ws = torch.empty((wsb,), dtype=torch.uint8, device=dev)
    check(L.buf_patch_voxelize(_ptr(patches), _ptr(axis), P, S, float(des_r), _ptr(centres), nc, int(azi_n),
                               _ptr(azi_cs), float(voxel_r), int(nsample), _hptr(hw[0]), _hptr(hw[1]), _hptr(hw[2]),
                               _hptr(hw[3]), _ptr(x), _ptr(R), _ptr(ra), _ptr(pn), _ptr(ws), wsb, _stream()), "buf_patch_voxelize")
    return x, R, ra, pn


def row_linear(x, w, b, activation=None):
    L = _lib.lib()
    x = _dev(x, torch.float32, "row_linear")
    n, cin = int(x.shape[0]), int(x.shape[1])
    cout = int(w.shape[0])
    out = torch.empty((n, cout), dtype=torch.float32, device=x.device)
    act = {None: 0, 'sigmoid': 1, 'softplus': 2}[activation]
    check(L.buf_row_linear(_ptr(x), n, cin, cout, _ptr(w.contiguous()), _ptr(b.contiguous()), act, _ptr(out), _stream()),
          "buf_row_linear")
    return out


def score_head(x, seg_lengths, vn1, vn2, lin, w, b, final, eps=1e-5):
    L = _lib.lib()
    x = _dev(x, torch.float32, "score_head")
    n = int(x.shape[0])
    lens = _host_i32(seg_lengths)
    nseg = int(lens.shape[0])
    out = torch.empty((n, 1), dtype=torch.float32, device=x.device)
    nbytes = L.buf_score_head_ws_bytes(n, nseg)
    ws = torch.empty(nbytes, dtype=torch.uint8, device=x.device)
    act = {None: 0, 'sigmoid': 1, 'softplus': 2}[final]
    check(L.buf_score_head(_ptr(x), n, _hptr(lens), nseg, _ptr(vn1.wf), _ptr(vn1.wd), _ptr(vn1.bsc), _ptr(vn1.bsh), vn1.slope,
                           _ptr(vn2.wf), _ptr(vn2.wd), _ptr(vn2.bsc), _ptr(vn2.bsh), vn2.slope, _ptr(lin.wf),
                           _ptr(w[0]), _ptr(b[0]), _ptr(w[1]), _ptr(b[1]), int(w[1].shape[0]), _ptr(w[2]), _ptr(b[2]), act, float(eps),
                           _ptr(out), _ptr(ws), nbytes, _stream()), "buf_score_head")
    return out


def score_head_supported(x_width, vn1, vn2, lin, w):
    return (x_width == 30 and tuple(vn1.wf.shape) == (10, 10) and tuple(vn2.wf.shape) == (5, 10) and tuple(lin.wf.shape) == (3, 5)
            and vn1.wd is not None and vn2.wd is not None and tuple(w[0].shape) == (20, 30) and w[1].shape[1] == 20 and w[1].shape[0] <= 10
            and tuple(w[2].shape) == (1, int(w[1].shape[0])))


def segment_instance_norm(x, seg_lengths, eps=1e-5):
    L = _lib.lib()
    x = _dev(x, torch.float32, "segment_instance_norm")
    n, c = int(x.shape[0]), int(x.shape[1])
    lens = _host_i32(seg_lengths)
    nseg = int(lens.shape[0])
    out = torch.empty_like(x)
    nbytes = L.buf_segment_instance_norm_ws_bytes(nseg, c)
    ws = torch.empty(nbytes, dtype=torch.uint8, device=x.device)
    check(L.buf_segment_instance_norm(_ptr(x), n, c, _hptr(lens), nseg, float(eps), _ptr(out), _ptr(ws), nbytes, _stream()),
          "buf_segment_instance_norm")
    return out


def hypotheses_score(ind, ss_kpts, tt_kpts, ss_R, tt_R, azi_n=20, inlier_th=1 / 3):
    L = _lib.lib()
    m = ind.shape[0]
    dev = ind.device
    R = torch.empty((m, 3, 3), dtype=torch.float32, device=dev)
    t = torch.empty((m, 3), dtype=torch.float32, device=dev)
    num = torch.empty((m,), dtype=torch.int32, device=dev)
    best = torch.zeros((1,), dtype=torch.int32, device=dev)
    mask = torch.zeros((m,), dtype=torch.uint8, device=dev)
    check(L.buf_hypotheses_score(_ptr(ind.contiguous()), _ptr(ss_kpts.contiguous()), _ptr(tt_kpts.contiguous()),
                                 _ptr(ss_R.contiguous()), _ptr(tt_R.contiguous()), m, int(azi_n), float(inlier_th),
                                 _ptr(R), _ptr(t), _ptr(num), _ptr(best), _ptr(mask), _stream()),
          "buf_hypotheses_score")
    return R, t, num, best, mask


def ransac_kabsch(src, tgt, corr, nhyp=4096, seed=0, max_dist=0.10, edge_similarity=0.8):
    L = _lib.lib()
    dev = src.device
    corr = _dev(corr, torch.int32, "ransac_kabsch")
    T = torch.empty((4, 4), dtype=torch.float32, device=dev)
    info = torch.zeros((2,), dtype=torch.int32, device=dev)
    nbytes = L.buf_ransac_ws_bytes(int(nhyp))
    ws = torch.empty(nbytes, dtype=torch.uint8, device=dev)
    check(L.buf_ransac_kabsch(_ptr(src.contiguous()), _ptr(tgt.contiguous()), _ptr(corr), corr.shape[0], int(nhyp),
                              int(seed), float(max_dist), float(edge_similarity), _ptr(T), _ptr(info), _ptr(ws), nbytes,
                              _stream()), "buf_ransac_kabsch")
    return T, info


def ransac_kabsch_masked(src, tgt, mask, nhyp=4096, seed=0, max_dist=0.10, edge_similarity=0.8):
    L = _lib.lib()
    dev = src.device
    mask = _dev(mask, torch.uint8, "ransac_kabsch_masked")
    m = int(mask.shape[0])
    T = torch.empty((4, 4), dtype=torch.float32, device=dev)
    info = torch.zeros((2,), dtype=torch.int32, device=dev)
    nbytes = L.buf_ransac_masked_ws_bytes(m, int(nhyp))
    ws = torch.empty(nbytes, dtype=torch.uint8, device=dev)
    check(L.buf_ransac_kabsch_masked(_ptr(src.contiguous()), _ptr(tgt.contiguous()), _ptr(mask), m, int(nhyp), int(seed),
                                     float(max_dist), float(edge_similarity), _ptr(T), _ptr(info), _ptr(ws), nbytes, _stream()),
          "buf_ransac_kabsch_masked")
    return T, info


def post_refine(T_init, src, tgt, thr=0.10, iters=20):
    L = _lib.lib()
    dev = src.device
    T_init = _dev(T_init, torch.float32, "post_refine").reshape(4, 4)
    T = torch.empty((4, 4), dtype=torch.float32, device=dev)
    info = torch.zeros((2,), dtype=torch.int32, device=dev)
    check(L.buf_post_refine(_ptr(T_init), _ptr(src.contiguous()), _ptr(tgt.contiguous()), src.shape[0], float(thr),
                            int(iters), _ptr(T), _ptr(info), _stream()), "buf_post_refine")
    return T, info


ICP_METHODS = {'point_to_point': 0, 'point_to_plane': 1, 'generalized': 2}


def icp_batched(src, src_lengths, tgt, tgt_lengths, max_dist, T_init, method='point_to_point', tgt_normals=None, max_iteration=30,
                relative_fitness=1e-6, relative_rmse=1e-6, correspondences=False, src_normals=None, epsilon=1e-3):
    L = _lib.lib()
    src, tgt = _dev(src, torch.float32, "icp_batched.src"), _dev(tgt, torch.float32, "icp_batched.tgt")
    sl, tl = _host_i32(src_lengths), _host_i32(tgt_lengths)
    B, dev = int(sl.shape[0]), src.device
    m = ICP_METHODS[method]
    nrm = _dev(tgt_normals, torch.float32, "icp_batched.tgt_normals") if tgt_normals is not None else None
    T_init = _dev(T_init, torch.float64, "icp_batched.T_init").reshape(B, 4, 4)
    T = torch.empty((B, 4, 4), dtype=torch.float64, device=dev)
    fit = torch.empty((B,), dtype=torch.float64, device=dev)
    rmse = torch.empty((B,), dtype=torch.float64, device=dev)
    iters = torch.empty((B,), dtype=torch.int32, device=dev)
    nn = torch.empty((max(int(src.shape[0]), 1),), dtype=torch.int32, device=dev) if correspondences else None
    nbytes = max(L.buf_icp_ws_bytes(int(src.shape[0]), int(tgt.shape[0]), max(B, 1), m), 1)
    ws = torch.empty(nbytes, dtype=torch.uint8, device=dev)
    if method == 'generalized':
        if src_normals is None or nrm is None:
            raise ValueError("icp_batched: method 'generalized' needs src_normals and tgt_normals")
        if not (0.0 < float(epsilon) <= 1.0):
            raise ValueError(f"icp_batched: epsilon={epsilon} (must be in (0, 1])")
        snrm = _dev(src_normals, torch.float32, "icp_batched.src_normals")
        if tuple(snrm.shape) != tuple(src.shape) or tuple(nrm.shape) != tuple(tgt.shape):
            raise ValueError("icp_batched: src_normals / tgt_normals must be shaped like src / tgt")
        check(L.buf_gicp_batched(_ptr(src), _ptr(snrm), _hptr(sl), _ptr(tgt), _ptr(nrm), _hptr(tl), B, float(max_dist), float(epsilon),
                                 _ptr(T_init), int(max_iteration), float(relative_fitness), float(relative_rmse), _ptr(T), _ptr(fit),
                                 _ptr(rmse), _ptr(iters), _ptr(nn), _ptr(ws), nbytes, _stream()), "buf_gicp_batched")
    else:
        check(L.buf_icp_batched(_ptr(src), _hptr(sl), _ptr(tgt), _ptr(nrm), _hptr(tl), B, m, float(max_dist), _ptr(T_init),
                                int(max_iteration), float(relative_fitness), float(relative_rmse), _ptr(T), _ptr(fit), _ptr(rmse),
                                _ptr(iters), _ptr(nn), _ptr(ws), nbytes, _stream()), "buf_icp_batched")
    return T, fit, rmse, iters, (nn[:int(src.shape[0])] if nn is not None else None)


VGICP_NEIGHBORS = (1, 7, 27)
VOXEL_MAP_CELLS = (1 << 22, 1 << 25, 1 << 28)


class VoxelMap:

    def __init__(self, m, buf):
        self.m, self.buf = m, buf
        self.nclouds, self.nrows, self.voxel, self.epsilon = int(m.nclouds), int(m.nrows), float(m.voxel), float(m.epsilon)

    def rows(self):
        dev, R = self.buf.device, self.nrows
        out = dict(keys=torch.empty((R,), dtype=torch.int64, device=dev), counts=torch.empty((R,), dtype=torch.int32, device=dev),
                   means=torch.empty((R, 3), dtype=torch.float64, device=dev), covs=torch.empty((R, 6), dtype=torch.float64, device=dev),
                   row_off=torch.empty((self.nclouds + 1,), dtype=torch.int32, device=dev))
        check(_lib.lib().buf_voxel_map_export(C.byref(self.m), R, _ptr(out['keys']), _ptr(out['counts']), _ptr(out['means']),
                                              _ptr(out['covs']), _ptr(out['row_off']), _stream()), "buf_voxel_map_export")
        return out


def voxel_map_build(points, lengths, voxel, normals=None, epsilon=1e-3, max_cells=0):
    L = _lib.lib()
    points = _dev(points, torch.float32, "voxel_map_build.points").reshape(-1, 3)
    lengths = _host_i32(lengths)
    n, nb = int(points.shape[0]), int(lengths.shape[0])
    if normals is not None:
        normals = _dev(normals, torch.float32, "voxel_map_build.normals").reshape(-1, 3)
        if tuple(normals.shape) != tuple(points.shape):
            raise ValueError("voxel_map_build: normals must be shaped like points")
    sizes = (int(max_cells),) if max_cells > 0 else VOXEL_MAP_CELLS
    for k, cells in enumerate(sizes):
        nbytes, wbytes = max(L.buf_voxel_map_bytes(n, nb, cells), 1), max(L.buf_voxel_map_ws_bytes(n, nb, cells), 1)
        buf = torch.empty(nbytes, dtype=torch.uint8, device=points.device)
        ws = torch.empty(wbytes, dtype=torch.uint8, device=points.device)
        m = _lib.buf_voxel_map_t()
        rc = L.buf_voxel_map_build(C.byref(m), _ptr(points), _ptr(normals), _hptr(lengths), nb, float(voxel), float(epsilon), cells,
                                   _ptr(buf), nbytes, _ptr(ws), wbytes, _stream())
        if rc == -4 and k + 1 < len(sizes):
            continue
        check(rc, "buf_voxel_map_build")
        return VoxelMap(m, buf)


def vgicp_batched(src, src_lengths, vmap, T_init, neighbors=7, src_normals=None, pair_cloud=None, max_iteration=30, rel_fitness=1e-6,
                  rel_rmse=1e-6, rows=False):
    L = _lib.lib()
    if neighbors not in VGICP_NEIGHBORS:
        raise ValueError(f"vgicp_batched: neighbors={neighbors} (one of {VGICP_NEIGHBORS})")
    src = _dev(src, torch.float32, "vgicp_batched.src").reshape(-1, 3)
    sl = _host_i32(src_lengths)
    B, dev, ns = int(sl.shape[0]), src.device, int(src.shape[0])
    snrm = None
    if src_normals is not None:
        snrm = _dev(src_normals, torch.float32, "vgicp_batched.src_normals").reshape(-1, 3)
        if tuple(snrm.shape) != tuple(src.shape):
            raise ValueError("vgicp_batched: src_normals must be shaped like src")
    pc = None
    if pair_cloud is not None:
        pc = _host_i32(pair_cloud)
        if pc.shape[0] != B:
            raise ValueError(f"vgicp_batched: {B} pairs but {pc.shape[0]} pair_cloud entries")
    T_init = _dev(T_init, torch.float64, "vgicp_batched.T_init").reshape(B, 4, 4)
    T = torch.empty((B, 4, 4), dtype=torch.float64, device=dev)
    fit = torch.empty((B,), dtype=torch.float64, device=dev)
    rmse = torch.empty((B,), dtype=torch.float64, device=dev)
    iters = torch.empty((B,), dtype=torch.int32, device=dev)
    row = torch.empty((max(ns, 1),), dtype=torch.int32, device=dev) if rows else None
    nbytes = max(L.buf_vgicp_ws_bytes(ns, max(B, 1)), 1)
    ws = torch.empty(nbytes, dtype=torch.uint8, device=dev)
    check(L.buf_vgicp_batched(C.byref(vmap.m), _ptr(src), _ptr(snrm), _hptr(sl), _hptr(pc) if pc is not None else C.c_void_p(0), B,
                              int(neighbors), _ptr(T_init), int(max_iteration), float(rel_fitness), float(rel_rmse), _ptr(T), _ptr(fit),
                              _ptr(rmse), _ptr(iters), _ptr(row), _ptr(ws), nbytes, _stream()), "buf_vgicp_batched")
    return T, fit, rmse, iters, (row[:ns] if row is not None else None)


def fpfh(points, normals, nbr, max_nn=100, return_spfh=False):
    L = _lib.lib()
    points, normals = _dev(points, torch.float32, "fpfh.points"), _dev(normals, torch.float32, "fpfh.normals")
    nbr = _dev(nbr, torch.int32, "fpfh.nbr")
    if points.dim() != 2 or points.shape[1] != 3 or normals.shape != points.shape:
        raise ValueError(f"fpfh: points {tuple(points.shape)} and normals {tuple(normals.shape)} are not both [N,3]")
    n = int(points.shape[0])
    if nbr.dim() != 2 or nbr.shape[0] != n:
        raise ValueError(f"fpfh: nbr {tuple(nbr.shape)} is not [{n},k]")
    out = torch.empty((n, 33), dtype=torch.float64, device=points.device)
    spfh = torch.empty((n, 33), dtype=torch.float64, device=points.device)
    check(L.buf_fpfh(_ptr(points), _ptr(normals), n, _ptr(nbr), int(nbr.shape[1]), int(max_nn), _ptr(out), _ptr(spfh), None, 0,
                     _stream()), "buf_fpfh")
    return (out, spfh) if return_spfh else out


FGR_STATUS = ('NOTHING', 'OK', 'FAILED')
FGR_MAX_TUPLES = 4096


def fgr_batched(src, src_lengths, tgt, tgt_lengths, corr, corr_lengths, seeds=None, tuple_scale=0.95, max_tuples=1000, trial_factor=100,
                mu_start=1.0, delta=0.025, delta_absolute=False, division_factor=1.4, decrease_every=4, iterations=64,
                return_rows=False):
    L = _lib.lib()
    src, tgt = _dev(src, torch.float32, "fgr_batched.src"), _dev(tgt, torch.float32, "fgr_batched.tgt")
    corr = _dev(corr, torch.int32, "fgr_batched.corr")
    sl, tl, cl = _host_i32(src_lengths), _host_i32(tgt_lengths), _host_i32(corr_lengths)
    B, dev = int(sl.shape[0]), src.device
    if tl.shape[0] != B or cl.shape[0] != B:
        raise ValueError(f"fgr_batched: {B} source lengths but {tl.shape[0]} target and {cl.shape[0]} correspondence lengths")
    for name, t, ln, w in (("src", src, sl, 3), ("tgt", tgt, tl, 3), ("corr", corr, cl, 2)):
        if t.dim() != 2 or t.shape[1] != w:
            raise ValueError(f"fgr_batched: {name} {tuple(t.shape)} is not [N,{w}]")
        if (ln < 0).any() or int(ln.astype(np.int64).sum()) != int(t.shape[0]):
            raise ValueError(f"fgr_batched: {name} lengths sum to {int(ln.astype(np.int64).sum())}, {name} holds {int(t.shape[0])} rows")
    if not (1 <= int(max_tuples) <= FGR_MAX_TUPLES):
        raise ValueError(f"fgr_batched: max_tuples={max_tuples} (1..{FGR_MAX_TUPLES})")
    sd = np.arange(B, dtype=np.uint64) if seeds is None else np.array([int(s) & _MASK64 for s in seeds], dtype=np.uint64).reshape(-1)
    if sd.shape[0] != B:
        raise ValueError(f"fgr_batched: {B} pairs but {sd.shape[0]} seeds")
    mt = int(max_tuples)
    T = torch.empty((B, 4, 4), dtype=torch.float64, device=dev)
    info = torch.zeros((B, 4), dtype=torch.int32, device=dev)
    rows = torch.empty((B, 3 * mt, 2), dtype=torch.int32, device=dev) if return_rows else None
    weights = torch.empty((B, 3 * mt), dtype=torch.float64, device=dev) if return_rows else None
    nbytes = max(L.buf_fgr_ws_bytes(int(corr.shape[0]), max(B, 1), mt), 1)
    ws = torch.empty(nbytes, dtype=torch.uint8, device=dev)
    check(L.buf_fgr_batched(_ptr(src), _hptr(sl), _ptr(tgt), _hptr(tl), _ptr(corr), _hptr(cl), B, _hptr(sd), float(tuple_scale), mt,
                            int(trial_factor), float(mu_start), float(delta), int(bool(delta_absolute)), float(division_factor),
                            int(decrease_every), int(iterations), _ptr(T), _ptr(info), _ptr(rows), _ptr(weights), _ptr(ws), nbytes,
                            _stream()), "buf_fgr_batched")
    return T, info, rows, weights


SC2_STATUS = ('NOTHING', 'OK')
SC2_MAX_ROWS, SC2_MAX_SEEDS, SC2_MAX_K1 = 16384, 1024, 128


def sc2_batched(src, src_lengths, tgt, tgt_lengths, corr, corr_lengths, d_thr, inlier_thr, seed_ratio=0.2, max_seeds=512, k1=30,
                nms_radius=0.0, power_iterations=10, refine_iterations=20, return_detail=False):
    L = _lib.lib()
    src, tgt = _dev(src, torch.float32, "sc2_batched.src"), _dev(tgt, torch.float32, "sc2_batched.tgt")
    corr = _dev(corr, torch.int32, "sc2_batched.corr")
    sl, tl, cl = _host_i32(src_lengths), _host_i32(tgt_lengths), _host_i32(corr_lengths)
    B, dev = int(sl.shape[0]), src.device
    if tl.shape[0] != B or cl.shape[0] != B:
        raise ValueError(f"sc2_batched: {B} source lengths but {tl.shape[0]} target and {cl.shape[0]} correspondence lengths")
    for name, t, ln, w in (("src", src, sl, 3), ("tgt", tgt, tl, 3), ("corr", corr, cl, 2)):
        if t.dim() != 2 or t.shape[1] != w:
            raise ValueError(f"sc2_batched: {name} {tuple(t.shape)} is not [N,{w}]")
        if (ln < 0).any() or int(ln.astype(np.int64).sum()) != int(t.shape[0]):
            raise ValueError(f"sc2_batched: {name} lengths sum to {int(ln.astype(np.int64).sum())}, {name} holds {int(t.shape[0])} rows")
    if B and int(cl.max()) > SC2_MAX_ROWS:
        raise ValueError(f"sc2_batched: {int(cl.max())} correspondences in one pair (at most {SC2_MAX_ROWS})")
    if not (1 <= int(max_seeds) <= SC2_MAX_SEEDS) or not (3 <= int(k1) <= SC2_MAX_K1):
        raise ValueError(f"sc2_batched: max_seeds={max_seeds} (1..{SC2_MAX_SEEDS}), k1={k1} (3..{SC2_MAX_K1})")
    ms, n = int(max_seeds), int(corr.shape[0])
    T = torch.empty((B, 4, 4), dtype=torch.float64, device=dev)
    info = torch.zeros((B, 6), dtype=torch.int32, device=dev)
    detail = None
    if return_detail:
        detail = dict(confidence=torch.empty(n, dtype=torch.float64, device=dev), seeds=torch.empty((B, ms), dtype=torch.int32, device=dev),
                      hyp_counts=torch.empty((B, ms), dtype=torch.int32, device=dev),
                      counts=torch.empty(ms * n, dtype=torch.int32, device=dev), inlier_mask=torch.empty(n, dtype=torch.uint8, device=dev))
    d = detail or {}
    nbytes = max(L.buf_sc2_ws_bytes(_hptr(cl), B, ms), 1) if B else 1
    ws = torch.empty(nbytes, dtype=torch.uint8, device=dev)
    check(L.buf_sc2_batched(_ptr(src), _hptr(sl), _ptr(tgt), _hptr(tl), _ptr(corr), _hptr(cl), B, float(d_thr), float(inlier_thr),
                            float(seed_ratio), ms, int(k1), float(nms_radius), int(power_iterations), int(refine_iterations), _ptr(T),
                            _ptr(info), _ptr(d.get('confidence')), _ptr(d.get('seeds')), _ptr(d.get('hyp_counts')), _ptr(d.get('counts')),
                            _ptr(d.get('inlier_mask')), _ptr(ws), nbytes, _stream()), "buf_sc2_batched")
    return T, info, detail


CLIQUE_STATUS = ('NOTHING', 'OK')
CLIQUE_MAX_SEEDS, CLIQUE_MAX_MEMBERS = 1024, 512


def clique_batched(src, src_lengths, tgt, tgt_lengths, corr, corr_lengths, d_thr, tim_thr=None, t_thr=None, inlier_thr=None,
                   max_seeds=64, max_members=256, gnc_factor=1.4, gnc_iterations=100, refine_iterations=20, return_detail=False):
    L = _lib.lib()
    src, tgt = _dev(src, torch.float32, "clique_batched.src"), _dev(tgt, torch.float32, "clique_batched.tgt")
    corr = _dev(corr, torch.int32, "clique_batched.corr")
    sl, tl, cl = _host_i32(src_lengths), _host_i32(tgt_lengths), _host_i32(corr_lengths)
    B, dev = int(sl.shape[0]), src.device
    if tl.shape[0] != B or cl.shape[0] != B:
        raise ValueError(f"clique_batched: {B} source lengths but {tl.shape[0]} target and {cl.shape[0]} correspondence lengths")
    for name, t, ln, w in (("src", src, sl, 3), ("tgt", tgt, tl, 3), ("corr", corr, cl, 2)):
        if t.dim() != 2 or t.shape[1] != w:
            raise ValueError(f"clique_batched: {name} {tuple(t.shape)} is not [N,{w}]")
        if (ln < 0).any() or int(ln.astype(np.int64).sum()) != int(t.shape[0]):
            raise ValueError(f"clique_batched: {name} lengths sum to {int(ln.astype(np.int64).sum())}, {name} holds {int(t.shape[0])} rows")
    if B and int(cl.max()) > SC2_MAX_ROWS:
        raise ValueError(f"clique_batched: {int(cl.max())} correspondences in one pair (at most {SC2_MAX_ROWS})")
    if not (1 <= int(max_seeds) <= CLIQUE_MAX_SEEDS) or not (3 <= int(max_members) <= CLIQUE_MAX_MEMBERS):
        raise ValueError(f"clique_batched: max_seeds={max_seeds} (1..{CLIQUE_MAX_SEEDS}), max_members={max_members} "
                         f"(3..{CLIQUE_MAX_MEMBERS})")
    d_thr = float(d_thr)
    tim_thr = d_thr if tim_thr is None else float(tim_thr)
    t_thr = d_thr / 2 if t_thr is None else float(t_thr)
    inlier_thr = d_thr if inlier_thr is None else float(inlier_thr)
    ms, mm, n = int(max_seeds), int(max_members), int(corr.shape[0])
    T = torch.empty((B, 4, 4), dtype=torch.float64, device=dev)
    info = torch.zeros((B, 8), dtype=torch.int32, device=dev)
    detail = None
    if return_detail:
        i32 = lambda *shape: torch.empty(shape, dtype=torch.int32, device=dev)
        detail = dict(deg=i32(n), core=i32(n), rank=i32(n), sizes=i32(B, ms), members=i32(B, mm),
                      weights=torch.empty((B, mm * (mm - 1) // 2), dtype=torch.float64, device=dev),
                      pose0=torch.empty((B, 12), dtype=torch.float64, device=dev), inlier_mask=torch.empty(n, dtype=torch.uint8, device=dev))
    d = detail or {}
    nbytes = max(L.buf_clique_ws_bytes(_hptr(cl), B, ms, mm), 1) if B else 1
    ws = torch.empty(nbytes, dtype=torch.uint8, device=dev)
    check(L.buf_clique_batched(_ptr(src), _hptr(sl), _ptr(tgt), _hptr(tl), _ptr(corr), _hptr(cl), B, d_thr, tim_thr, t_thr, inlier_thr, ms,
                               mm, float(gnc_factor), int(gnc_iterations), int(refine_iterations), _ptr(T), _ptr(info), _ptr(d.get('deg')),
                               _ptr(d.get('core')), _ptr(d.get('rank')), _ptr(d.get('sizes')), _ptr(d.get('members')),
                               _ptr(d.get('weights')), _ptr(d.get('pose0')), _ptr(d.get('inlier_mask')), _ptr(ws), nbytes, _stream()),
          "buf_clique_batched")
    return T, info, detail


def pair_stats(points, lengths, pair_src, pair_tgt, T, radius, correspondences=False, cells_per_elem=0):
    L = _lib.lib()
    points = _dev(points, torch.float32, "pair_stats.points")
    if points.dim() != 2 or points.shape[1] != 3:
        raise ValueError(f"pair_stats: points {tuple(points.shape)} is not [N,3]")
    ln, pa, pb = _host_i32(lengths), _host_i32(pair_src), _host_i32(pair_tgt)
    if pa.shape != pb.shape:
        raise ValueError(f"pair_stats: {pa.shape[0]} sources but {pb.shape[0]} targets")
    if int(ln.sum()) != int(points.shape[0]):
        raise ValueError(f"pair_stats: lengths sum to {int(ln.sum())}, points holds {int(points.shape[0])} rows")
    Cn, P, dev = int(ln.shape[0]), int(pa.shape[0]), points.device
    T = _dev(T, torch.float64, "pair_stats.T").reshape(P, 4, 4)
    ok = (pa >= 0) & (pa < Cn)
    rows = int(ln[pa[ok]].astype(np.int64).sum())
    matched = torch.zeros((P,), dtype=torch.int32, device=dev)
    moments = torch.zeros((P, 10), dtype=torch.float64, device=dev)
    nn = torch.empty((max(rows, 1),), dtype=torch.int32, device=dev) if correspondences else None
    nbytes = max(L.buf_pair_stats_ws_bytes(int(points.shape[0]), max(Cn, 1), max(P, 1), rows, int(cells_per_elem)), 1)
    ws = torch.empty(nbytes, dtype=torch.uint8, device=dev)
    check(L.buf_pair_stats(_ptr(points), _hptr(ln), Cn, _hptr(pa), _hptr(pb), P, _ptr(T), float(radius), int(cells_per_elem),
                           _ptr(matched), _ptr(moments), _ptr(nn), _ptr(ws), nbytes, _stream()), "buf_pair_stats")
    return matched, moments, (nn[:rows] if nn is not None else None)


PG_MAX_NODES = 128
PG_STATUS = ('NOTHING', 'CONVERGED_STEP', 'CONVERGED_COST', 'MAX_ITER', 'STALLED', 'FAILED')
PG_TICK_HZ = 1e8


def pose_graph_optimize(nodes, edges, edge_i, edge_j, Z, info, uncertain, fixed, mu, X_init, max_iterations=100, eps_step=1e-9,
                        eps_cost=1e-10, tau0=1e-5, want_ticks=False):
    L = _lib.lib()
    nd, ed, fx = _host_i32(nodes), _host_i32(edges), _host_i32(fixed)
    ei, ej = _host_i32(edge_i), _host_i32(edge_j)
    un = np.ascontiguousarray(uncertain, dtype=np.uint8).reshape(-1)
    mu = np.ascontiguousarray(mu, dtype=np.float64).reshape(-1)
    G = int(nd.shape[0])
    if not (ed.shape[0] == G and fx.shape[0] == G and mu.shape[0] == G):
        raise ValueError(f"pose_graph_optimize: {G} graphs but {ed.shape[0]} edge counts, {fx.shape[0]} fixed nodes, {mu.shape[0]} weights")
    if (nd < 0).any() or (ed < 0).any():
        raise ValueError("pose_graph_optimize: negative node or edge count")
    N, E = int(nd.astype(np.int64).sum()), int(ed.astype(np.int64).sum())
    if not (ei.shape[0] == E and ej.shape[0] == E and un.shape[0] == E):
        raise ValueError(f"pose_graph_optimize: {E} edges but {ei.shape[0]} / {ej.shape[0]} node ids, {un.shape[0]} flags")
    X_init = _dev(X_init, torch.float64, "pose_graph_optimize.X_init").reshape(N, 4, 4)
    dev = X_init.device
    Z = _dev(Z, torch.float64, "pose_graph_optimize.Z").reshape(E, 4, 4)
    info = _dev(info, torch.float64, "pose_graph_optimize.info").reshape(E, 6, 6)
    X = torch.empty((N, 4, 4), dtype=torch.float64, device=dev)
    status = torch.zeros((G, 3), dtype=torch.int32, device=dev)
    cost = torch.zeros((G, 2), dtype=torch.float64, device=dev)
    edge = torch.zeros((E, 2), dtype=torch.float64, device=dev)
    nbytes = max(L.buf_pose_graph_ws_bytes(max(G, 1), N, E, min(int(nd.max()) if G else 0, PG_MAX_NODES)), 1)
    ws = torch.zeros(nbytes, dtype=torch.uint8, device=dev)
    check(L.buf_pose_graph_optimize(_hptr(nd), _hptr(ed), G, _hptr(ei), _hptr(ej), _ptr(Z), _ptr(info), _hptr(un), _hptr(fx), _hptr(mu),
                                    _ptr(X_init), int(max_iterations), float(eps_step), float(eps_cost), float(tau0), _ptr(X), _ptr(status),
                                    _ptr(cost), _ptr(edge), _ptr(ws), nbytes, _stream()), "buf_pose_graph_optimize")
    if want_ticks:
        return X, status, cost, edge, ws[:32 * G].view(torch.int64).reshape(G, 4).clone()
    return X, status, cost, edge


METRIC_COLUMNS = ('rep_src', 'rep_tgt', 'nn_inl', 'mutual', 'mutual_inl', 'cons', 'cons_true')


def match_metrics(kp, s_nn, t_nn, T_gt, T_est, tau_kp, tau_match, dist_th, want_d2=False):
    L = _lib.lib()
    kp = _dev(kp, torch.float32, "match_metrics.kp")
    s_nn, t_nn = _dev(s_nn, torch.int32, "match_metrics.s_nn"), _dev(t_nn, torch.int32, "match_metrics.t_nn")
    if s_nn.dim() != 2 or s_nn.shape != t_nn.shape:
        raise ValueError(f"match_metrics: s_nn {tuple(s_nn.shape)} and t_nn {tuple(t_nn.shape)} must both be [B,P]")
    B, P = int(s_nn.shape[0]), int(s_nn.shape[1])
    if kp.dim() != 2 or tuple(kp.shape) != (2 * B * P, 3):
        raise ValueError(f"match_metrics: kp {tuple(kp.shape)} is not [2*{B}*{P},3]")
    dev = kp.device
    T_gt = torch.as_tensor(T_gt, dtype=torch.float64).to(dev).reshape(B, 4, 4).contiguous()
    T_est = _dev(T_est, torch.float32, "match_metrics.T_est").reshape(B, 4, 4).contiguous()
    counts = torch.empty((B, len(METRIC_COLUMNS)), dtype=torch.int32, device=dev)
    d2 = torch.empty((2 * B * P,), dtype=torch.float32, device=dev) if want_d2 else None
    check(L.buf_match_metrics(_ptr(kp), _ptr(s_nn), _ptr(t_nn), B, P, _ptr(T_gt), _ptr(T_est), float(tau_kp), float(tau_match),
                              float(dist_th), _ptr(counts), _ptr(d2), _stream()), "buf_match_metrics")
    return (counts, d2) if want_d2 else counts


def recover_poses_batched(ind, ss_kpts, tt_kpts, ss_R, tt_R, seg_lengths, seeds, cfg):
    L = _lib.lib()
    seg = _host_i32(seg_lengths)
    nb, M = int(seg.shape[0]), int(seg.sum())
    dev = ss_kpts.device
    poses = torch.empty((nb, 4, 4), dtype=torch.float32, device=dev)
    if nb == 0:
        return poses
    nbytes = L.buf_recover_poses_ws_bytes(M, nb, int(cfg.ransac_hypotheses))
    ws = torch.empty(nbytes, dtype=torch.uint8, device=dev)
    sd = (C.c_ulonglong * nb)(*[int(x) & _MASK64 for x in seeds])
    check(L.buf_recover_poses_batched(_ptr(ind.contiguous()), _ptr(ss_kpts.contiguous()), _ptr(tt_kpts.contiguous()),
                                      _ptr(ss_R.contiguous()), _ptr(tt_R.contiguous()), _hptr(seg), nb, sd, int(cfg.azi_n),
                                      float(cfg.inlier_th), int(cfg.ransac_hypotheses), float(cfg.dist_th), float(cfg.similar_th),
                                      float(cfg.refine_threshold), 20 if cfg.pose_refine else 0, _ptr(poses), _ptr(ws), nbytes,
                                      _stream()), "buf_recover_poses_batched")
    return poses


def mfma_tile_weights(wt, lk_major=False):
    K, cout = wt.shape
    assert K % 16 == 0 and cout % 16 == 0
    t = wt.reshape(K // 16, 4, 4, cout // 16, 16)
    perm = (0, 3, 1, 4, 2) if lk_major else (0, 3, 2, 4, 1)
    return np.ascontiguousarray(np.transpose(t, perm), dtype=np.float32).reshape(-1)


def winograd_tile_weights(w, ng=None, blocks=4):
    cout, cin = w.shape[0], w.shape[1]
    assert cin % 4 == 0 and cout % 16 == 0
    if ng is None:
        ng = _lib.lib().buf_winograd_group(cin, cout)
    G = np.array([[1, 0, 0], [.5, .5, .5], [.5, -.5, .5], [0, 0, 1]], np.float64)
    G5 = np.concatenate([G, [[0, 1, 0]]])
    U = np.einsum('ia,ocab,jb->ijoc', G5, np.asarray(w, np.float64), G)
    U = U[:blocks].reshape(blocks, 4, cout // (16 * ng), ng, 16, cin // 4, 4)
    return np.ascontiguousarray(np.transpose(U, (2, 0, 5, 3, 6, 4, 1)), dtype=np.float32).reshape(-1)


def winograd_f24_tile_weights(w):
    cout, cin = w.shape[0], w.shape[1]
    assert cin % 4 == 0 and cout % 32 == 0
    U = winograd_f24_filters(w)
    U = U.reshape(4, 6, cout // 32, 2, 16, cin // 4, 4)
    U = np.transpose(U, (2, 0, 5, 3, 6, 4, 1))
    lead = U.shape[:3]
    wide = U[..., [0, 1, 2, 5]].reshape(*lead, 512)
    narrow = U[..., [3, 4]].reshape(*lead, 256)
    return np.ascontiguousarray(np.concatenate([wide, narrow], axis=-1), dtype=np.float32).reshape(-1)


F24_G2 = np.array([[1, 0, 0], [.5, .5, .5], [.5, -.5, .5], [0, 0, 1]], np.float64)
F24_G4 = np.array([[.25, 0, 0], [-1 / 6, -1 / 6, -1 / 6], [-1 / 6, 1 / 6, -1 / 6], [1 / 24, 1 / 12, 1 / 6], [1 / 24, -1 / 12, 1 / 6], [0, 0, 1]],
                  np.float64)


def winograd_f24_filters(w):
    w64 = np.asarray(w, np.float64)
    U = np.zeros((4, 6) + w64.shape[:2], np.float64)
    for a in range(3):
        for b in range(3):
            U += (F24_G2[:, a][:, None, None, None] * w64[None, None, :, :, a, b]) * F24_G4[:, b][None, :, None, None]
    return U


F24_FLAG = 2
F24K_FLAG = 4
F24P_DEFAULT = True
F24A_DEFAULT = 'all'
F24A_PARTS = {'all': (64, 32), 'out64': (64,), 'out32': (32,), 'off': (), None: ()}


def cyl_layer_filters(w, f24k=True):
    wt = winograd_tile_weights(w)
    cout, cin = w.shape[0], w.shape[1]
    if cout == 128:
        flag = F24_FLAG
    elif f24k and cout == 64 and cin % 64 == 0:
        flag = F24K_FLAG
    else:
        return wt, 0
    return np.concatenate([wt, winograd_f24_tile_weights(w)]), flag


def cyl_f24a_parts(f24, f24k, f24p, f24a):
    explicit = not (f24 is None and f24k is None and f24p is None)
    f24, f24k, f24p = (True if f24 is None else f24), (True if f24k is None else f24k), (F24P_DEFAULT if f24p is None else f24p)
    if f24a is None:
        f24a = None if explicit else F24A_DEFAULT
    if f24a is True:
        f24a = 'all'
    if f24a is False:
        f24a = 'off'
    if f24a not in F24A_PARTS:
        raise ValueError(f"f24a = {f24a!r}: one of 'all', 'out64', 'out32', 'off'")
    if F24A_PARTS[f24a] and not (f24 and f24k and f24p):
        raise ValueError("f24a goes with the default forms of the other layers (f24, f24k, f24p left alone or true)")
    return f24, f24k, f24p, F24A_PARTS[f24a]


def cyl_f24a_filters(layers, flags, parts, device):
    sets = [torch.from_numpy(winograd_f24_tile_weights(w)).to(device)
            if (flag == 0 and w.shape[0] in parts and w.shape[0] in (32, 64) and w.shape[1] % 16 == 0) else None
            for (w, _, _), flag in zip(layers, flags)]
    return sets, (C.c_void_p * len(sets))(*[None if t is None else t.data_ptr() for t in sets])


class CylindricalNet:

    def __init__(self, layers, device, f24=None, f24k=None, f24p=None, f24a=None):
        f24, f24k, f24p, parts = cyl_f24a_parts(f24, f24k, f24p, f24a)
        self.wt, self.bias, self.cin, self.cout, self.relu = [], [], [], [], []
        self.entry = "buf_cylindrical_net_wg"
        self.form = 1 if f24p else 0
        flags = []
        for w, b, relu in layers:
            cout, cin = w.shape[0], w.shape[1]
            wt, flag = cyl_layer_filters(w, f24k) if f24 else (winograd_tile_weights(w), 0)
            flags.append(flag)
            self.wt.append(torch.from_numpy(wt).to(device))
            self.bias.append(torch.from_numpy(np.ascontiguousarray(b, dtype=np.float32)).to(device))
            self.cin.append(cin); self.cout.append(cout); self.relu.append(1 if relu else 0)
        n = len(layers)
        self._wp = (C.c_void_p * n)(*[t.data_ptr() for t in self.wt])
        self._bp = (C.c_void_p * n)(*[t.data_ptr() for t in self.bias])
        self._ci = (C.c_int * n)(*self.cin)
        self._co = (C.c_int * n)(*self.cout)
        self._re = (C.c_int * n)(*[r | f for r, f in zip(self.relu, flags)])
        self.wt24, self._w24p = cyl_f24a_filters(layers, flags, parts, device)
        self.f24_layers = [l for l, t in enumerate(self.wt24) if t is not None]
        self.f24_all = bool(self.f24_layers) and all(f or t is not None for f, t in zip(flags, self.wt24))

    def __call__(self, x):
        L = _lib.lib()
        x = x.contiguous()
        P = x.shape[0]
        y = torch.empty((P, self.cout[-1], 7, 20), dtype=torch.float32, device=x.device)
        if self.f24_layers:
            check(L.buf_cylindrical_net_wg_all(_ptr(x), P, self._wp, self._bp, self._ci, self._co, self._re, self._w24p, _ptr(y), _stream()),
                  "buf_cylindrical_net_wg_all")
            return y
        check(L.buf_cylindrical_net_wg_form(_ptr(x), P, self._wp, self._bp, self._ci, self._co, self._re, self.form, _ptr(y), _stream()), self.entry)
        return y


def split_tile_filters(w):
    L = _lib.lib()
    w = np.ascontiguousarray(w, dtype=np.float32)
    cout, cin = w.shape[0], w.shape[1]
    out = np.empty(L.buf_split_filter_count(cout, cin), dtype=np.uint16)
    check(L.buf_split_tile_filters(w.ctypes.data, cout, cin, out.ctypes.data), "buf_split_tile_filters")
    return out


class CylindricalNetSplit:

    def __init__(self, layers, device, f24k=None, f24p=None, f24a=None):
        _, f24k, f24p, parts = cyl_f24a_parts(None, f24k, f24p, f24a)
        self.wt, self.bias, self.cin, self.cout, self.relu = [], [], [], [], []
        self.entry = "buf_cylindrical_net_split"
        self.f24_layers, self.f24_all = [], False
        self.form = 1 if f24p else 0
        for w, b, relu in layers:
            cout, cin = w.shape[0], w.shape[1]
            self.wt.append(torch.from_numpy(split_tile_filters(w).view(np.int16)).to(device))
            self.bias.append(torch.from_numpy(np.ascontiguousarray(b, dtype=np.float32)).to(device))
            self.cin.append(cin); self.cout.append(cout); self.relu.append(1 if relu else 0)
        n = len(layers)
        self.status = torch.zeros(1, dtype=torch.int32, device=device)
        self._wp = (C.c_void_p * n)(*[t.data_ptr() for t in self.wt])
        self._bp = (C.c_void_p * n)(*[t.data_ptr() for t in self.bias])
        self._ci = (C.c_int * n)(*self.cin)
        self._co = (C.c_int * n)(*self.cout)
        self._re = (C.c_int * n)(*self.relu)
        self.last_flags = None
        self.safe = n == 8 and _lib.lib().buf_cylindrical_net_wg_supports(self._ci, self._co) == 0 and not os.environ.get('BUF_SPLIT_UNSAFE')
        if self.safe:
            tiled = [cyl_layer_filters(w, f24k) for w, _, _ in layers]
            self.wt_wg = [torch.from_numpy(wt).to(device) for wt, _ in tiled]
            self._wwp = (C.c_void_p * n)(*[t.data_ptr() for t in self.wt_wg])
            self._re_safe = (C.c_int * n)(*[r | f for r, (_, f) in zip(self.relu, tiled)])
            self.wt24, self._w24p = cyl_f24a_filters(layers, [f for _, f in tiled], parts, device)
            self.f24_layers = [l for l, t in enumerate(self.wt24) if t is not None]
            self.f24_all = bool(self.f24_layers) and all(f or t is not None for (_, f), t in zip(tiled, self.wt24))

    def _safe_call(self, x, head):
        L = _lib.lib()
        x = x.contiguous()
        P = x.shape[0]
        out = torch.empty((P, self.cout[-1], 7, 20), dtype=torch.float32, device=x.device)
        desc = torch.empty((P, 32), dtype=torch.float32, device=x.device) if head is not None else None
        self.last_flags = torch.empty((max(P, 1),), dtype=torch.int32, device=x.device)
        if self.f24_layers:
            check(L.buf_cylindrical_net_split_safe_all(_ptr(x), P, self._wp, self._wwp, self._bp, self._ci, self._co, self._re_safe, self._w24p,
                                                       _ptr(head.params) if head is not None else None, _ptr(out), _ptr(desc), _ptr(self.status),
                                                       _ptr(self.last_flags), _stream()), "buf_cylindrical_net_split_safe_all")
            return (desc, out) if head is not None else out
        check(L.buf_cylindrical_net_split_safe_form(_ptr(x), P, self._wp, self._wwp, self._bp, self._ci, self._co, self._re_safe, self.form,
                                                    _ptr(head.params) if head is not None else None, _ptr(out), _ptr(desc), _ptr(self.status),
                                                    _ptr(self.last_flags), _stream()), "buf_cylindrical_net_split_safe_form")
        return (desc, out) if head is not None else out

    def __call__(self, x):
        if self.safe:
            return self._safe_call(x, None)
        L = _lib.lib()
        x = x.contiguous()
        P = x.shape[0]
        y = torch.empty((P, self.cout[-1], 7, 20), dtype=torch.float32, device=x.device)
        check(L.buf_cylindrical_net_split(_ptr(x), P, self._wp, self._bp, self._ci, self._co, self._re, _ptr(y), _ptr(self.status), _stream()),
              self.entry)
        return y

    def with_head(self, x, head):
        if self.safe:
            return self._safe_call(x, head)
        L = _lib.lib()
        x = x.contiguous()
        P = x.shape[0]
        desc = torch.empty((P, 32), dtype=torch.float32, device=x.device)
        equi = torch.empty((P, 32, 7, 20), dtype=torch.float32, device=x.device)
        check(L.buf_cylindrical_net_split_head(_ptr(x), P, self._wp, self._bp, self._ci, self._co, self._re, _ptr(head.params),
                                               _ptr(desc), _ptr(equi), _ptr(self.status), _stream()), "buf_cylindrical_net_split_head")
        return desc, equi

    def range_fallbacks(self):
        return 0 if self.last_flags is None else int((self.last_flags != 0).sum().item())

    def check_range(self):
        if int(self.status.item()) != 0:
            self.status.zero_()
            if not self.safe:
                raise FloatingPointError("buf_cylindrical_net_split: an activation left the f16 range (|v| >= 65504); use the fp32 kernel")


class DescriptorHead:

    def __init__(self, w0, b0, w3, b3, device):
        f = lambda a, n: np.asarray(a, dtype=np.float32).reshape(n)
        self.params = torch.from_numpy(np.concatenate([f(w0, 512), f(b0, 16), f(w3, 16), f(b3, 1)])).to(device)

    def __call__(self, y):
        L = _lib.lib()
        y = y.contiguous()
        P = y.shape[0]
        assert y.dtype == torch.float32 and y.numel() == P * 32 * 140
        desc = torch.empty((P, 32), dtype=torch.float32, device=y.device)
        equi = torch.empty((P, 32, 7, 20), dtype=torch.float32, device=y.device)
        check(L.buf_descriptor_head(_ptr(y), P, _ptr(self.params), _ptr(desc), _ptr(equi), _stream()), "buf_descriptor_head")
        return desc, equi


def split_tile_gemm(w, nt):
    L = _lib.lib()
    w = np.ascontiguousarray(w, dtype=np.float32)
    cout, cin, ntaps = w.shape
    out = np.empty(L.buf_split_gemm_count(cout, cin, ntaps, nt), dtype=np.uint16)
    check(L.buf_split_tile_gemm(w.ctypes.data, cout, cin, ntaps, nt, out.ctypes.data), "buf_split_tile_gemm")
    return out


def separate_cost_layer0(w):
    w = np.asarray(w, np.float64)
    cout, cin = w.shape[0], w.shape[1]
    ws = np.zeros((3, 5, cin, cout))
    for dn in range(3):
        for dl in range(3):
            ws[:, dl - dn + 2] += np.transpose(w[:, :, dn, :, dl], (2, 1, 0))
    wt = np.transpose(w.sum(2), (2, 3, 1, 0))
    return ws.reshape(-1, cout).astype(np.float32), wt.reshape(-1, cout).astype(np.float32)


class CostVolumeNet:

    def __init__(self, layers, device):
        assert len(layers) == 10
        self.wt, self.bias = [], []
        for i, (w, b) in enumerate(layers):
            cout, cin = w.shape[0], w.shape[1]
            b = np.asarray(b, np.float32)
            if i == 0:
                assert tuple(w.shape) == (32, 32, 3, 3, 3), w.shape
                tiled = np.concatenate([mfma_tile_weights(m, lk_major=True) for m in separate_cost_layer0(w)])
                self.wt.append(torch.from_numpy(tiled).to(device))
                self.bias.append(torch.from_numpy(np.ascontiguousarray(b)).to(device))
                continue
            if i == 1:
                assert tuple(w.shape) == (64, 32, 3, 3, 3), w.shape
                w2d = np.ascontiguousarray(np.transpose(w, (0, 3, 1, 2, 4)).reshape(64, 96, 3, 3))
                self.wt.append(torch.from_numpy(winograd_tile_weights(w2d, ng=_lib.lib().buf_cost_winograd_group(1))).to(device))
                self.bias.append(torch.from_numpy(np.ascontiguousarray(b)).to(device))
                continue
            if 2 <= i <= 5:
                assert tuple(w.shape[2:]) == (3, 1, 3), w.shape
                tiled = winograd_tile_weights(np.ascontiguousarray(w[:, :, :, 0, :]), ng=_lib.lib().buf_cost_winograd_group(i))
                self.wt.append(torch.from_numpy(tiled).to(device))
                self.bias.append(torch.from_numpy(np.ascontiguousarray(b)).to(device))
                continue
            wt = np.transpose(w, (2, 3, 4, 1, 0)).reshape(-1, cout)
            if i == 9:
                wt = np.concatenate([wt, np.zeros((wt.shape[0], 32 - cout), np.float32)], 1)
                b = np.concatenate([b, np.zeros(32 - cout, np.float32)])
            self.wt.append(torch.from_numpy(mfma_tile_weights(np.ascontiguousarray(wt, dtype=np.float32), lk_major=True)).to(device))
            self.bias.append(torch.from_numpy(np.ascontiguousarray(b)).to(device))
        self._wp = (C.c_void_p * 10)(*[t.data_ptr() for t in self.wt])
        self._bp = (C.c_void_p * 10)(*[t.data_ptr() for t in self.bias])

    def __call__(self, s_eq, t_eq):
        L = _lib.lib()
        s_eq, t_eq = s_eq.contiguous(), t_eq.contiguous()
        m = s_eq.shape[0]
        out = torch.empty((m,), dtype=torch.float32, device=s_eq.device)
        check(L.buf_cost_volume_net(_ptr(s_eq), _ptr(t_eq), m, self._wp, self._bp, _ptr(out), _stream()),
              "buf_cost_volume_net")
        return out

    def gathered(self, equi, s_rows, t_rows):
        L = _lib.lib()
        equi = _dev(equi, torch.float32, "CostVolumeNet.gathered")
        if equi.dim() != 4 or tuple(equi.shape[1:]) != (32, 7, 20):
            raise _lib.BufferHipError(f"CostVolumeNet.gathered: expected [rows,32,7,20] maps, got {tuple(equi.shape)}")
        s_rows, t_rows = _dev(s_rows, torch.int64, "s_rows"), _dev(t_rows, torch.int64, "t_rows")
        m = int(s_rows.shape[0])
        out = torch.empty((m,), dtype=torch.float32, device=equi.device)
        check(L.buf_cost_volume_net_gather(_ptr(equi), 7, _ptr(s_rows), _ptr(t_rows), m, self._wp, self._bp, _ptr(out), _stream()),
              "buf_cost_volume_net_gather")
        return out


class CostVolumeNetSplit:

    def __init__(self, layers, device):
        assert len(layers) == 10
        mats = []
        w0 = layers[0][0]
        assert tuple(w0.shape) == (32, 32, 3, 3, 3), w0.shape
        ws, wt = separate_cost_layer0(w0)
        mats.append((np.transpose(ws.reshape(15, 32, 32), (2, 1, 0)), 2))
        mats.append((np.transpose(wt.reshape(9, 32, 32), (2, 1, 0)), 2))
        w1 = layers[1][0]
        assert tuple(w1.shape) == (64, 32, 3, 3, 3), w1.shape
        mats.append((np.transpose(w1, (0, 3, 1, 2, 4)).reshape(64, 96, 9), 2))
        for i in range(2, 9):
            w = layers[i][0]
            assert tuple(w.shape[2:]) == (3, 1, 3), w.shape
            mats.append((np.ascontiguousarray(w[:, :, :, 0, :]).reshape(w.shape[0], w.shape[1], 9), 2 if i < 7 else 1))
        w9 = layers[9][0]
        assert tuple(w9.shape) == (20, 32, 2, 1, 2), w9.shape
        mats.append((np.ascontiguousarray(w9[:, :, :, 0, :]).reshape(20, 32, 4), 1))
        self.wt = [torch.from_numpy(split_tile_gemm(m, nt).view(np.int16)).to(device) for m, nt in mats]
        self.bias = []
        for i, (_, b) in enumerate(layers):
            b = np.asarray(b, np.float32)
            if i == 9:
                b = np.concatenate([b, np.zeros(32 - b.shape[0], np.float32)])
            self.bias.append(torch.from_numpy(np.ascontiguousarray(b)).to(device))
        self.status = torch.zeros(1, dtype=torch.int32, device=device)
        self._wp = (C.c_void_p * 11)(*[t.data_ptr() for t in self.wt])
        self._bp = (C.c_void_p * 10)(*[t.data_ptr() for t in self.bias])
        self.safe = not os.environ.get('BUF_SPLIT_UNSAFE')
        self.f32 = CostVolumeNet(layers, device) if self.safe else None
        self.last_flags = None

    def _safe(self, s_eq, t_eq, s_rows, t_rows, m, dev):
        L = _lib.lib()
        out = torch.empty((m,), dtype=torch.float32, device=dev)
        self.last_flags = torch.empty((max(m, 1),), dtype=torch.int32, device=dev)
        check(L.buf_cost_volume_net_split_safe(_ptr(s_eq), _ptr(t_eq), 7, _ptr(s_rows), _ptr(t_rows), m, self._wp, self._bp, self.f32._wp,
                                               self.f32._bp, _ptr(out), _ptr(self.status), _ptr(self.last_flags), _stream()),
              "buf_cost_volume_net_split_safe")
        return out

    def __call__(self, s_eq, t_eq):
        L = _lib.lib()
        s_eq, t_eq = s_eq.contiguous(), t_eq.contiguous()
        m = s_eq.shape[0]
        if self.safe:
            return self._safe(s_eq, t_eq, None, None, m, s_eq.device)
        out = torch.empty((m,), dtype=torch.float32, device=s_eq.device)
        check(L.buf_cost_volume_net_split(_ptr(s_eq), _ptr(t_eq), m, self._wp, self._bp, _ptr(out), _ptr(self.status), _stream()),
              "buf_cost_volume_net_split")
        return out

    def gathered(self, equi, s_rows, t_rows):
        L = _lib.lib()
        equi = _dev(equi, torch.float32, "CostVolumeNetSplit.gathered")
        if equi.dim() != 4 or tuple(equi.shape[1:]) != (32, 7, 20):
            raise _lib.BufferHipError(f"CostVolumeNetSplit.gathered: expected [rows,32,7,20] maps, got {tuple(equi.shape)}")
        s_rows, t_rows = _dev(s_rows, torch.int64, "s_rows"), _dev(t_rows, torch.int64, "t_rows")
        m = int(s_rows.shape[0])
        if self.safe:
            return self._safe(equi, equi, s_rows, t_rows, m, equi.device)
        out = torch.empty((m,), dtype=torch.float32, device=equi.device)
        check(L.buf_cost_volume_net_split_gather(_ptr(equi), 7, _ptr(s_rows), _ptr(t_rows), m, self._wp, self._bp, _ptr(out),
                                                 _ptr(self.status), _stream()), "buf_cost_volume_net_split_gather")
        return out

    def range_fallbacks(self):
        return 0 if self.last_flags is None else int((self.last_flags != 0).sum().item())

    def check_range(self):
        if int(self.status.item()) != 0:
            self.status.zero_()
            if not self.safe:
                raise FloatingPointError("buf_cost_volume_net_split: a value left the f16 range (|v| >= 65504); use the fp32 kernel")
```

buffer_amd/registration.py:

```python
import numpy as np

from . import ops
from .patch_embedder import _fold_bn


class CostVolume:

    def __init__(self, W, device, azi_n=20, arith='f32'):
        if arith not in ('f32', 'split'):
            raise ValueError(f"cnn_arith must be 'f32' or 'split', got {arith!r}")
        if azi_n != 20:
            raise NotImplementedError(f'CostVolume: the fused kernel is built for azi_n = 20 (got {azi_n})')
        self.azi_n = azi_n
        p = 'Inlier.conv.ops'
        layers = []
        for i, bn in ((0, 1), (3, 4), (6, 7), (9, 10), (12, 13), (15, 16), (18, 19), (21, 22), (24, 25)):
            layers.append(_fold_bn(W[f'{p}.{i}.weight'], W[f'{p}.{i}.bias'], W[f'{p}.{bn}.running_mean'], W[f'{p}.{bn}.running_var']))
        layers.append((np.asarray(W[f'{p}.27.weight'], np.float32), np.asarray(W[f'{p}.27.bias'], np.float32)))
        self.fused = ops.CostVolumeNetSplit(layers, device) if arith == 'split' else ops.CostVolumeNet(layers, device)

    def __call__(self, d1, d2):
        if tuple(d1.shape[1:]) != (32, 5, 20) or d1.shape != d2.shape:
            raise ValueError(f'CostVolume: expected two [M,32,5,20] maps, got {tuple(d1.shape)} and {tuple(d2.shape)}')
        return self.fused(d1, d2)

    def gathered(self, equi, s_rows, t_rows):
        return self.fused.gathered(equi, s_rows, t_rows)
```

include/buffer_hip.h:

```cpp
#ifndef BUFFER_HIP_H
#define BUFFER_HIP_H
#include <stddef.h>
#include <stdint.h>
#ifdef __cplusplus
extern "C" {
#endif

#define BUF_OK            0
#define BUF_EINVAL       -1
#define BUF_EHIP         -2
#define BUF_EWORKSPACE   -3
#define BUF_ECAPACITY    -4
#define BUF_ENODEVICE    -5

const char* buf_last_error(void);
int         buf_version(void);
int         buf_device_count(void);
#define BUF_TIMED_GRID_QUERY 0
#define BUF_TIMED_CYL_NET    1
#define BUF_TIMED_COST_NET   2
#define BUF_TIMED_SELECT_PATCHES 3
#define BUF_TIMED_PATCH_VOXELIZE 4
#define BUF_TIMED_FPS            5
#define BUF_TIMED_NN1            6
#define BUF_TIMED_VN_GATHER      7
#define BUF_TIMED_GRID_SUBSAMPLE 8
#define BUF_TIMED_DESC_HEAD      9
#define BUF_TIMED_CYL_NET_SPLIT  10
#define BUF_TIMED_COST_NET_SPLIT 11
#define BUF_TIMED_SPFH           12
#define BUF_TIMED_FPFH           13
#define BUF_TIMED_SC2_COMPAT     14
#define BUF_TIMED_SC2_CONF       15
#define BUF_TIMED_SC2_COUNTS     16
#define BUF_TIMED_SC2_HYP        17
#define BUF_TIMED_SC2_REFINE     18
#define BUF_TIMED_CLIQUE_GRAPH   19
#define BUF_TIMED_CLIQUE_PEEL    20
#define BUF_TIMED_CLIQUE_ORDER   21
#define BUF_TIMED_CLIQUE_WALK    22
#define BUF_TIMED_CLIQUE_POSE    23
#define BUF_TIMED_CLIQUE_POLISH  24
#define BUF_TIMED_NKERNELS       25
void        buf_timing_enable(int on);
long long   buf_timing_collect(double* total_ms, double* total_bytes);
long long   buf_timing_collect_kernel(int kernel_id, double* total_ms, double* total_work);

typedef struct buf_grid {
    void*   ws;
    size_t  ws_bytes;
    int     ns, nb;
    int64_t cells_per_elem;
    float   radius;
    const float* supports;
    void*   desc;
    int*    s_off;
    int*    table;
    void*   sorted;
    int*    order;
    void*   scan_tmp;
} buf_grid_t;

int64_t buf_grid_default_cells(int ns, int nb);
size_t  buf_grid_ws_bytes(int ns, int nb, int64_t cells_per_elem);
int     buf_grid_cell_dims(const double* ext, float radius, int64_t cells_per_elem, double* edge_out, int* dim_out);
int     buf_grid_build(buf_grid_t* g, const float* supports, int ns, const int* s_batches_host, int nb,
                       float radius, int64_t cells_per_elem, void* ws, size_t ws_bytes, void* stream);
int     buf_grid_query(const buf_grid_t* g, const float* queries, int nq, const int* q_batches_host,
                       const int* q_order, float radius, int k_out, int* nbr_out, int* counts_out,
                       int* max_count_out, void* todo_ws, void* stream);
int     buf_radius_neighbors(const float* queries, int nq, const float* supports, int ns,
                             const int* q_batches_host, const int* s_batches_host, int nb, float radius,
                             int k_out, int* nbr_out, int* counts_out, int* max_count_out,
                             void* ws, size_t ws_bytes, void* stream);

size_t  buf_grid_subsample_ws_bytes(int n, int nb, int64_t max_cells, int fdim);
int     buf_grid_subsample_batch(const float* pts, int n, const int* batches_host, int nb, float dl,
                                 int max_p, const float* feats, int fdim, float* out_pts, float* out_feats,
                                 int* out_batches_host, int* out_m_host,
                                 int64_t max_cells, void* ws, size_t ws_bytes, void* stream);

size_t  buf_fps_ws_bytes(int b, int n);
int     buf_fps(const float* xyz, int b, int n, int m, int* idx_out, void* ws, size_t ws_bytes, void* stream);
int     buf_fps_ragged(const float* xyz, const int* lengths_host, int b, int m, int* idx_out, void* ws, size_t ws_bytes,
                       void* stream);
int     buf_gather(const float* feat, const int* idx, int b, int c, int n, int m, float* out, void* stream);
int     buf_group(const float* feat, const int* idx, int b, int c, int n, int m, int nsample, float* out, void* stream);
int     buf_ball_query(const float* xyz, const float* new_xyz, int b, int n, int m, float radius, int nsample,
                       int* idx, void* stream);
int     buf_three_nn(const float* unknown, const float* known, int b, int n, int m, float* dist, int* idx, void* stream);
int     buf_select_patches(const float* pts, const float* kpts, int n, int m, float radius, int nsample,
                           float* patches, void* stream);
size_t  buf_select_patches_batched_ws_bytes(int n_total, int nc);
int     buf_select_patches_batched(const float* pts, const int* lengths_host, int nc, const float* kpts, int m, float radius,
                                   int nsample, float* patches, void* ws, size_t ws_bytes, void* stream);
int     buf_permute_clouds(const float* const* clouds_host, const int* lengths_host, const unsigned long long* keys_host,
                           int nc, float* out, void* stream);

size_t  buf_compact_ws_bytes(int n);
int     buf_compact_greater(const float* x, int stride, int n, float threshold, int* idx_out, int* count_out,
                            void* ws, size_t ws_bytes, void* stream);

size_t  buf_knn_ws_bytes(int b, int q, int k);
size_t  buf_knn1_ws_bytes(int b, int n, int q);
int     buf_knn(const float* ref, const float* query, int b, int n, int q, int d, int k, float* dist,
                long long* idx, void* ws, size_t ws_bytes, void* stream);

int     buf_svd3x3_batched(const float* a, int n, float* u, float* s, float* v, void* stream);

int     buf_vn_gather_block(const float* q_pts, const float* s_pts, const float* feats, const int* idx,
                            int nq, int ns, int k, int cin, int cout, int mode, float scale,
                            const float* wf, const float* wd, const float* bn_scale, const float* bn_shift,
                            float slope, float* out, void* stream);
int     buf_vn_gather_pre_supported(int k, int cin, int cout);
size_t  buf_vn_gather_pre_ws_bytes(int ns, int cout);
int     buf_vn_gather_block_pre(const float* q_pts, const float* s_pts, const float* feats, const int* idx,
                                int nq, int ns, int k, int cin, int cout, float scale,
                                const float* wf, const float* wd, const float* bn_scale, const float* bn_shift,
                                float slope, float* out, void* ws, size_t ws_bytes, void* stream);
int     buf_vn_pointwise(const float* a, const int* ind_a, int ind_stride, int na, int ca, const float* b, int cb,
                         int n, int cout, const float* wf, const float* wd, const float* bn_scale,
                         const float* bn_shift, float slope, const float* residual, float* out, void* stream);
int     buf_gather_max(const float* feats, const int* idx, int nq, int ns, int k, int width, float* out, void* stream);
int     buf_row_linear(const float* x, int n, int cin, int cout, const float* w, const float* b, int activation, float* out,
                       void* stream);
size_t  buf_segment_instance_norm_ws_bytes(int nseg, int c);
int     buf_segment_instance_norm(const float* x, int n, int c, const int* lens_host, int nseg, float eps, float* out,
                                  void* ws, size_t ws_bytes, void* stream);
int     buf_vn_std(const float* x, const float* z, int n, int c, float* out, void* stream);
size_t  buf_score_head_ws_bytes(int n, int nseg);
int     buf_score_head(const float* x, int n, const int* lens_host, int nseg,
                       const float* vn1_wf, const float* vn1_wd, const float* vn1_bsc, const float* vn1_bsh, float vn1_slope,
                       const float* vn2_wf, const float* vn2_wd, const float* vn2_bsc, const float* vn2_bsh, float vn2_slope,
                       const float* lin, const float* w0, const float* b0, const float* w1, const float* b1, int c1,
                       const float* w2, const float* b2, int final_activation, float eps, float* out,
                       void* ws, size_t ws_bytes, void* stream);

size_t  buf_patch_voxelize_ws_bytes(int ncentres);
int     buf_patch_voxelize(const float* patches, const float* axis, int npatch, int npts, float des_r,
                           const float* centres, int ncentres, int azi_n, const float* azi_cs, float voxel_r,
                           int nsample, const float* mlp_w_host, const float* mlp_b_host, const float* bn_scale_host,
                           const float* bn_shift_host, float* out_x, float* out_R, float* out_rand, float* out_patches,
                           void* ws, size_t ws_bytes, void* stream);

int     buf_winograd_group(int cin, int cout);
int     buf_winograd_tile_weights(const float* w_host, int cout, int cin, float* out_host);
int     buf_winograd_tile_filters(const float* w_host, int cout, int cin, int ng, int nblk, float* out_host);
#define BUF_CYL_F24 2
#define BUF_CYL_F24K 4
int     buf_cylindrical_net_wg_flags(const int* cin_host, const int* cout_host, const int* relu_host);
int     buf_winograd_f24_tile_weights(const float* w_host, int cout, int cin, float* out_host);
int     buf_cylindrical_net_wg(const float* x, int npatch, const float* const* wt_host, const float* const* bias_host,
                               const int* cin_host, const int* cout_host, const int* relu_host, float* y, void* stream);
#define BUF_CYL_FORM_DEFAULT (-1)
#define BUF_CYL_FORM_K_SPLIT 0
#define BUF_CYL_FORM_PASS_SPLIT 1
int     buf_cylindrical_net_wg_form(const float* x, int npatch, const float* const* wt_host, const float* const* bias_host,
                                    const int* cin_host, const int* cout_host, const int* relu_host, int form, float* y, void* stream);
int     buf_cylindrical_net_wg_supports(const int* cin_host, const int* cout_host);
int     buf_cylindrical_net_wg_all_flags(const int* cin_host, const int* cout_host, const int* relu_host, const float* const* wt24_host);
int     buf_cylindrical_net_wg_all(const float* x, int npatch, const float* const* wt_host, const float* const* bias_host,
                                   const int* cin_host, const int* cout_host, const int* relu_host, const float* const* wt24_host,
                                   float* y, void* stream);

long long buf_split_filter_count(int cout, int cin);
int     buf_split_tile_filters(const float* w_host, int cout, int cin, unsigned short* out_host);
int     buf_cylindrical_net_split(const float* x, int npatch, const void* const* wt_host, const float* const* bias_host,
                                  const int* cin_host, const int* cout_host, const int* relu_host, float* y, int* status_dev, void* stream);
int     buf_cylindrical_net_split_head(const float* x, int npatch, const void* const* wt_host, const float* const* bias_host,
                                       const int* cin_host, const int* cout_host, const int* relu_host, const float* head_params,
                                       float* desc, float* equi, int* status_dev, void* stream);

int     buf_cylindrical_net_split_safe(const float* x, int npatch, const void* const* wt_split_host, const float* const* wt_wg_host,
                                       const float* const* bias_host, const int* cin_host, const int* cout_host, const int* relu_host,
                                       const float* head_params, float* y_or_equi, float* desc, int* status_dev, int* flags_ws, void* stream);

int     buf_cylindrical_net_split_safe_form(const float* x, int npatch, const void* const* wt_split_host, const float* const* wt_wg_host,
                                            const float* const* bias_host, const int* cin_host, const int* cout_host, const int* relu_host,
                                            int form, const float* head_params, float* y_or_equi, float* desc, int* status_dev, int* flags_ws,
                                            void* stream);
int     buf_cylindrical_net_split_safe_all(const float* x, int npatch, const void* const* wt_split_host, const float* const* wt_wg_host,
                                           const float* const* bias_host, const int* cin_host, const int* cout_host, const int* relu_host,
                                           const float* const* wt24_host, const float* head_params, float* y_or_equi, float* desc,
                                           int* status_dev, int* flags_ws, void* stream);

int     buf_descriptor_head(const float* y, int npatch, const float* params, float* desc, float* equi, void* stream);

int     buf_cost_winograd_group(int layer);
int     buf_cost_volume_net(const float* s_eq, const float* t_eq, int m, const float* const* wt_host,
                            const float* const* bias_host, float* ind_out, void* stream);
int     buf_cost_volume_net_gather(const float* equi, int ele_n, const long long* s_rows, const long long* t_rows, int m,
                                   const float* const* wt_host, const float* const* bias_host, float* ind_out, void* stream);

long long buf_split_gemm_count(int cout, int cin, int ntaps, int nt);
int     buf_split_tile_gemm(const float* w_host, int cout, int cin, int ntaps, int nt, unsigned short* out_host);
int     buf_cost_volume_net_split(const float* s_eq, const float* t_eq, int m, const void* const* wt_host,
                                  const float* const* bias_host, float* ind_out, int* status_dev, void* stream);
int     buf_cost_volume_net_split_gather(const float* equi, int ele_n, const long long* s_rows, const long long* t_rows, int m,
                                         const void* const* wt_host, const float* const* bias_host, float* ind_out,
                                         int* status_dev, void* stream);
int     buf_cost_volume_net_split_safe(const float* s_eq, const float* t_eq, int ele_n, const long long* s_rows, const long long* t_rows,
                                       int m, const void* const* wt_split_host, const float* const* bias_split_host,
                                       const float* const* wt_f32_host, const float* const* bias_f32_host, float* ind_out,
                                       int* status_dev, int* flags_ws, void* stream);

int     buf_hypotheses_score(const float* ind, const float* ss_kpts, const float* tt_kpts, const float* ss_R,
                             const float* tt_R, int m, int azi_n, float inlier_th, float* R_out, float* t_out,
                             int* inlier_num, int* best_out, unsigned char* best_mask, void* stream);
size_t  buf_ransac_ws_bytes(int nhyp);
int     buf_ransac_kabsch(const float* src, const float* tgt, const int* corr, int ncorr, int nhyp,
                          unsigned long long seed, float max_dist, float edge_similarity, float* T_out,
                          int* info_out, void* ws, size_t ws_bytes, void* stream);
size_t  buf_ransac_masked_ws_bytes(int m, int nhyp);
int     buf_ransac_kabsch_masked(const float* src, const float* tgt, const unsigned char* mask, int m, int nhyp,
                                 unsigned long long seed, float max_dist, float edge_similarity, float* T_out,
                                 int* info_out, void* ws, size_t ws_bytes, void* stream);
int     buf_post_refine(const float* T_init, const float* src, const float* tgt, int m, float inlier_threshold,
                        int iters, float* T_out, int* info_out, void* stream);
size_t  buf_recover_poses_ws_bytes(int m_total, int nb, int nhyp);
int     buf_recover_poses_batched(const float* ind, const float* ss_kpts, const float* tt_kpts, const float* ss_R, const float* tt_R,
                                  const int* seg_host, int nb, const unsigned long long* seeds_host, int azi_n, float inlier_th,
                                  int nhyp, float max_dist, float edge_similarity, float refine_threshold, int refine_iters,
                                  float* poses_out, void* ws, size_t ws_bytes, void* stream);

size_t  buf_voxel_downsample_ws_bytes(int n, int64_t max_cells);
int     buf_voxel_downsample(const void* pts, const void* normals, int is_f64, int n, double voxel_size, double* out_pts,
                             double* out_normals, int* out_m_host, int64_t max_cells, void* ws, size_t ws_bytes, void* stream);
size_t  buf_voxel_downsample_batch_ws_bytes(int n, int nb, int64_t max_cells);
int     buf_voxel_downsample_batch(const void* pts, int is_f64, int n, const int* lengths_host, int nb, double voxel_size,
                                   double* out_pts, int* out_lengths_host, int64_t max_cells, void* ws, size_t ws_bytes, void* stream);
int     buf_knn_normals(const float* pts, int ns, const int* qidx, int nq, const int* cand, int ncand, int knn,
                        const double* camera_host, int orient, float* normals, unsigned char* deficient, void* stream);

#define BUF_ICP_POINT_TO_POINT 0
#define BUF_ICP_POINT_TO_PLANE 1
#define BUF_ICP_GENERALIZED 2
size_t  buf_icp_ws_bytes(int n_src_total, int n_tgt_total, int npairs, int method);
int     buf_icp_batched(const float* src, const int* src_lengths_host, const float* tgt, const float* tgt_normals,
                        const int* tgt_lengths_host, int npairs, int method, float max_dist, const double* T_init_f64,
                        int max_iteration, double rel_fitness, double rel_rmse, double* T_out_f64, double* fitness_out,
                        double* rmse_out, int* iters_out, int* nn_out, void* ws, size_t ws_bytes, void* stream);
int     buf_gicp_batched(const float* src, const float* src_normals, const int* src_lengths_host, const float* tgt,
                         const float* tgt_normals, const int* tgt_lengths_host, int npairs, float max_dist, double epsilon,
                         const double* T_init_f64, int max_iteration, double rel_fitness, double rel_rmse, double* T_out_f64,
                         double* fitness_out, double* rmse_out, int* iters_out, int* nn_out, void* ws, size_t ws_bytes, void* stream);

size_t  buf_fpfh_ws_bytes(int n);
int     buf_fpfh(const float* pts, const float* normals, int n, const int* nbr, int k_nbr, int max_nn,
                 double* fpfh_out , double* spfh_out ,
                 void* ws, size_t ws_bytes, void* stream);

#define BUF_FGR_NOTHING 0
#define BUF_FGR_OK      1
#define BUF_FGR_FAILED  2
size_t  buf_fgr_ws_bytes(int n_corr_total, int npairs, int max_tuples);
int     buf_fgr_batched(const float* src, const int* src_lengths_host, const float* tgt, const int* tgt_lengths_host,
                        const int* corr ,
                        const int* corr_lengths_host, int npairs, const unsigned long long* seeds_host,
                        double tuple_scale, int max_tuples, int trial_factor,
                        double mu_start, double delta, int delta_absolute,
                        double division_factor, int decrease_every, int iterations,
                        double* T_out , int* info_out ,
                        int* rows_out , double* weights_out ,
                        void* ws, size_t ws_bytes, void* stream);

#define BUF_SC2_NOTHING 0
#define BUF_SC2_OK      1
#define BUF_SC2_MAX_ROWS 16384
size_t  buf_sc2_ws_bytes(const int* corr_lengths_host, int npairs, int max_seeds);
int     buf_sc2_batched(const float* src, const int* src_lengths_host, const float* tgt, const int* tgt_lengths_host,
                        const int* corr ,
                        const int* corr_lengths_host, int npairs,
                        double d_thr, double inlier_thr, double seed_ratio, int max_seeds,
                        int k1, double nms_radius, int power_iterations, int refine_iterations,
                        double* T_out , int* info_out ,
                        double* conf_out, int* seeds_out, int* hyp_counts_out, int* counts_out, unsigned char* inliers_out ,
                        void* ws, size_t ws_bytes, void* stream);

typedef struct buf_voxel_map {
    void*   buf;
    size_t  buf_bytes;
    int     nclouds, nrows, n;
    int64_t max_cells;
    double  voxel, epsilon;
    void*   clouds;
    int*    table;
    double* rows;
    long long* keys;
    int*    row_off;
} buf_voxel_map_t;
size_t  buf_voxel_map_bytes(int n_total, int nclouds, int64_t max_cells);
size_t  buf_voxel_map_ws_bytes(int n_total, int nclouds, int64_t max_cells);
int     buf_voxel_map_build(buf_voxel_map_t* map, const float* pts, const float* normals, const int* lengths_host, int nclouds,
                            double voxel, double epsilon, int64_t max_cells, void* buf, size_t buf_bytes, void* ws, size_t ws_bytes,
                            void* stream);
int     buf_voxel_map_export(const buf_voxel_map_t* map, int n, long long* keys, int* counts, double* means, double* covs,
                             int* row_off, void* stream);
size_t  buf_vgicp_ws_bytes(int n_src_total, int npairs);
int     buf_vgicp_batched(const buf_voxel_map_t* map, const float* src, const float* src_normals, const int* src_lengths_host,
                          const int* pair_cloud_host, int npairs, int neighbors, const double* T_init_f64, int max_iteration,
                          double rel_fitness, double rel_rmse, double* T_out_f64, double* fitness_out, double* rmse_out,
                          int* iters_out, int* row_out, void* ws, size_t ws_bytes, void* stream);

#define BUF_CLIQUE_NOTHING 0
#define BUF_CLIQUE_OK      1
size_t  buf_clique_ws_bytes(const int* corr_lengths_host, int npairs, int max_seeds, int max_members);
int     buf_clique_batched(const float* src, const int* src_lengths_host, const float* tgt, const int* tgt_lengths_host,
                           const int* corr ,
                           const int* corr_lengths_host, int npairs,
                           double d_thr, double tim_thr, double t_thr, double inlier_thr,
                           int max_seeds, int max_members, double gnc_factor, int gnc_iterations,
                           int refine_iterations,
                           double* T_out , int* info_out ,
                           int* deg_out, int* core_out, int* rank_out, int* sizes_out, int* members_out, double* weights_out,
                           double* pose0_out, unsigned char* inliers_out ,
                           void* ws, size_t ws_bytes, void* stream);

size_t  buf_pair_stats_ws_bytes(int n_total, int nclouds, int npairs, int n_src_rows, int64_t cells_per_elem);
int     buf_pair_stats(const float* pts, const int* lengths_host, int nclouds, const int* pair_src_host, const int* pair_tgt_host,
                       int npairs, const double* T_f64, float radius, int64_t cells_per_elem, int* matched_out,
                       double* moments_out, int* nn_out , void* ws, size_t ws_bytes, void* stream);

#define BUF_METRICS_NCOUNT     7
#define BUF_METRICS_REP_SRC    0
#define BUF_METRICS_REP_TGT    1
#define BUF_METRICS_NN_INL     2
#define BUF_METRICS_MUTUAL     3
#define BUF_METRICS_MUTUAL_INL 4
#define BUF_METRICS_CONS       5
#define BUF_METRICS_CONS_TRUE  6
int     buf_match_metrics(const float* kp, const int* s_nn, const int* t_nn, int npairs, int P, const double* T_gt_f64,
                          const float* T_est_f32, float tau_kp, float tau_match, float dist_th, int* out_counts,
                          float* out_nn_d2 , void* stream);

#define BUF_PG_MAX_NODES        128
#define BUF_PG_NOTHING          0
#define BUF_PG_CONVERGED_STEP   1
#define BUF_PG_CONVERGED_COST   2
#define BUF_PG_MAX_ITER         3
#define BUF_PG_STALLED          4
#define BUF_PG_FAILED           5
size_t  buf_pose_graph_ws_bytes(int ngraphs, int nodes_total, int edges_total, int max_nodes);
int     buf_pose_graph_optimize(const int* nodes_host, const int* edges_host, int ngraphs, const int* edge_i_host,
                                const int* edge_j_host, const double* Z_f64, const double* info_f64,
                                const unsigned char* uncertain_host, const int* fixed_host, const double* mu_host,
                                const double* X_init_f64, int max_iterations, double eps_step, double eps_cost, double tau0,
                                double* X_out_f64, int* status_out, double* cost_out, double* edge_out, void* ws, size_t ws_bytes,
                                void* stream);

#ifdef __cplusplus
}
#endif
#endif
```

Before: 173.8.

## Use Winograd F(2x2,4x3) tiles for cost-volume net layers 2, 4 and 6

Adds a cost-volume network kernel variant that runs conv layers 2 and 4 with the existing Winograd F24 pass, parameterised on a new per-layer K stride. Layer 6 goes through the Winograd cw_layer path, with layer 5 writing a new layout for it. Filters are pre-transformed on the host once at construction, and the variant is on by default ('all'). This cuts the multiply count of these 3x3 convolutions, at the cost of extra LDS zeroing, a transform stage and possible rounding differences from the plain convolution path.

```diff
diff --git a/buffer_amd/_lib.py b/buffer_amd/_lib.py
--- a/buffer_amd/_lib.py
+++ b/buffer_amd/_lib.py
@@ -145,6 +145,9 @@
     "buf_descriptor_head": (_i, [_vp, _i, _vp, _vp, _vp, _vp]),
     "buf_cost_volume_net": (_i, [_vp, _vp, _i, _vp, _vp, _vp, _vp]),
     "buf_cost_volume_net_gather": (_i, [_vp, _i, _vp, _vp, _i, _vp, _vp, _vp, _vp]),
+    "buf_cost_volume_net_w24": (_i, [_vp, _vp, _i, _vp, _vp, _vp, _vp, _vp]),
+    "buf_cost_volume_net_w24_gather": (_i, [_vp, _i, _vp, _vp, _i, _vp, _vp, _vp, _vp, _vp]),
+    "buf_cost_volume_net_split_safe_w24": (_i, [_vp, _vp, _i, _vp, _vp, _i, _vp, _vp, _vp, _vp, _vp, _vp, _vp, _vp, _vp]),
     "buf_hypotheses_score": (_i, [_vp, _vp, _vp, _vp, _vp, _i, _i, _f, _vp, _vp, _vp, _vp, _vp, _vp]),
     "buf_ransac_ws_bytes": (_sz, [_i]),
     "buf_ransac_kabsch": (_i, [_vp, _vp, _vp, _i, _i, C.c_uint64, _f, _f, _vp, _vp, _vp, _sz, _vp]),
diff --git a/buffer_amd/csrc/buffer_hip.hip b/buffer_amd/csrc/buffer_hip.hip
--- a/buffer_amd/csrc/buffer_hip.hip
+++ b/buffer_amd/csrc/buffer_hip.hip
@@ -20,6 +20,7 @@
 #include "convnet_w24p.hip"
 #include "convnet_w24a.hip"
 #include "costnet.hip"
+#include "costnet_w24.hip"
 #include "split_safe.hip"
 #include "fpfh.hip"
 #include "fgr.hip"
diff --git a/buffer_amd/csrc/convnet_w24.hip b/buffer_amd/csrc/convnet_w24.hip
--- a/buffer_amd/csrc/convnet_w24.hip
+++ b/buffer_amd/csrc/convnet_w24.hip
@@ -48,7 +48,7 @@
 
 #define W24_U(n, k, j) ((j) < 3 ? W4[n][k][j] : ((j) == 5 ? W4[n][k][3] : W2[n][k][(j) - 3]))
 
-template <int I, bool PRIMED, int INEXT>
+template <int I, bool PRIMED, int INEXT, unsigned KSTEP = WG_KSTEP>
 __device__ __forceinline__ void w24_pass(unsigned (&RA)[4], __amdgpu_buffer_rsrc_t rs, unsigned wp, unsigned wp_next, unsigned lofs4, unsigned lofs2,
                                          int niter, wgf4 (&W4)[2][2], wgf2 (&W2)[2][2], wgf4 (&acc)[2][6], wgf2 (&D)[2][6])
 {
@@ -58,7 +58,7 @@
     unsigned P0 = RA[A1], P1 = RA[A2];
     if constexpr (!PRIMED) {
         W24_LOAD(D[0], P0, P1, 0)
-        W24_LOAD(D[1], P0, P1, WG_KSTEP)
+        W24_LOAD(D[1], P0, P1, KSTEP)
     }
 #define W24_XFORM(BUF)                                                                                    \
     {                                                                                                     \
@@ -81,18 +81,18 @@
         const bool more = it + 1 < niter;
         const unsigned wcur = wp + 4 * it * W24_WSTRIDE;
         const unsigned wn = more ? wcur + 4 * W24_WSTRIDE : wp_next;
-        const unsigned adv = more ? 4u * WG_KSTEP : 0u;
+        const unsigned adv = more ? 4u * KSTEP : 0u;
         __builtin_amdgcn_sched_barrier(0);
 #pragma unroll
         for (int s = 0; s < 4; s++) {
-            if (s < 2) W24_LOAD(D[s & 1], P0, P1, (s + 2) * WG_KSTEP)
+            if (s < 2) W24_LOAD(D[s & 1], P0, P1, (s + 2) * KSTEP)
             else {
                 if (s == 2) { P0 += adv; P1 += adv; }
                 if constexpr (INEXT >= 0) {
                     unsigned q0 = more ? P0 : RA[A1N], q1 = more ? P1 : RA[A2N];
-                    W24_LOAD(D[s & 1], q0, q1, (s - 2) * WG_KSTEP)
+                    W24_LOAD(D[s & 1], q0, q1, (s - 2) * KSTEP)
                 } else
-                    W24_LOAD(D[s & 1], P0, P1, (s - 2) * WG_KSTEP)
+                    W24_LOAD(D[s & 1], P0, P1, (s - 2) * KSTEP)
             }
             __builtin_amdgcn_sched_barrier(0);
 #pragma unroll
@@ -114,7 +114,7 @@
 #undef W24_XFORM
 }
 
-template <bool NOBIAS = false>
+template <bool NOBIAS = false, unsigned KSTEP = WG_KSTEP>
 __device__ __forceinline__ void w24_round(unsigned (&RA)[4], __amdgpu_buffer_rsrc_t rs, unsigned wp, unsigned wp_after, unsigned lofs4, unsigned lofs2,
                                           int niter, unsigned pstride, const float* __restrict__ bias_lane, wgf4 (&W4)[2][2], wgf2 (&W2)[2][2],
                                           wgf4 (&Y)[2][2][4])
@@ -142,7 +142,7 @@
             for (int n = 0; n < 2; n++) acc[n][1] += bv[n];
         }
         constexpr int ICHAIN = (INEXT != 0 && wg_chains(I)) ? INEXT : -1;
-        w24_pass<I, wg_chains(I - 1), ICHAIN>(RA, rs, wp + I * pstride, INEXT == 0 ? wp_after : wp + (I + 1) * pstride, lofs4, lofs2, niter, W4, W2, acc, D);
+        w24_pass<I, wg_chains(I - 1), ICHAIN, KSTEP>(RA, rs, wp + I * pstride, INEXT == 0 ? wp_after : wp + (I + 1) * pstride, lofs4, lofs2, niter, W4, W2, acc, D);
         __builtin_amdgcn_sched_barrier(0);
 #pragma unroll
         for (int n = 0; n < 2; n++) {
diff --git a/buffer_amd/csrc/costnet.hip b/buffer_amd/csrc/costnet.hip
--- a/buffer_amd/csrc/costnet.hip
+++ b/buffer_amd/csrc/costnet.hip
@@ -280,8 +280,15 @@
 #define CV_STAMP_AT(SLOT)
 #endif
 
+#define CW_CS5 72
+template <int C, int CS, int USED>
+__device__ __forceinline__ void cw24_zero_spare(float* __restrict__ map);
+template <int HIN, int RS, int CS, int NTX, int TYPM, int CIN, int RSO, int CSO>
+__device__ __forceinline__ void cw24_layer(float* __restrict__ map, const float* __restrict__ wt, const float* __restrict__ bias, int pair, int t);
+
+template <bool W24 = false>
 __device__ __forceinline__ void cost_net_body(const float* __restrict__ s_eq, const float* __restrict__ t_eq, const CostNetParams& P,
-                                              float* __restrict__ ind_out, float* __restrict__ lds)
+                                              float* __restrict__ ind_out, float* __restrict__ lds, const float* const* f24 = nullptr)
 {
     float* bufA = lds;
     float* bufB = lds;
@@ -384,19 +391,44 @@
         __syncthreads();
         CV_STAMP_AT(2)
     }
-    cw_layer<16, 16, CW_CS1, 2, 64, 2, 2, 0, 14, CW_CS2, false>(bufA, P.wt[2], P.bias[2], w & 1, 2 * (w >> 1));
+    bool f24_2 = false, f24_4 = false, f24_6 = false;
+    if constexpr (W24) { f24_2 = f24[0] != nullptr; f24_4 = f24[1] != nullptr; f24_6 = f24[2] != nullptr; }
+    if (W24 && f24_2) {
+        if constexpr (W24) {
+            cw24_zero_spare<64, CW_CS1, 256>(bufA);
+            __syncthreads();
+            cw24_layer<16, 16, CW_CS1, 4, 4, 64, 14, CW_CS2>(bufA, f24[0], P.bias[2], w & 1, w >> 1);
+        }
+    } else
+        cw_layer<16, 16, CW_CS1, 2, 64, 2, 2, 0, 14, CW_CS2, false>(bufA, P.wt[2], P.bias[2], w & 1, 2 * (w >> 1));
     __syncthreads();
     CV_STAMP_AT(3)
     cw_layer<14, 14, CW_CS2, 2, 64, 2, 2, 1, 12, CW_CS3, false>(bufA, P.wt[3], P.bias[3], w, 0);
     __syncthreads();
     CV_STAMP_AT(4)
-    cw_layer<12, 12, CW_CS3, 3, 128, 2, 2, 0, 12, CW_CS3, false>(bufA, P.wt[4], P.bias[4], w, 0);
+    if (W24 && f24_4) {
+        if constexpr (W24) {
+            cw24_zero_spare<128, CW_CS3, 144>(bufA);
+            __syncthreads();
+            cw24_layer<12, 12, CW_CS3, 3, 5, 128, 12, CW_CS3>(bufA, f24[1], P.bias[4], w, 0);
+        }
+    } else
+        cw_layer<12, 12, CW_CS3, 3, 128, 2, 2, 0, 12, CW_CS3, false>(bufA, P.wt[4], P.bias[4], w, 0);
     __syncthreads();
     CV_STAMP_AT(5)
-    cw_layer<10, 12, CW_CS3, 4, 128, 1, 1, 0, 0, CV_C64, true>(bufA, P.wt[5], P.bias[5], w, 0);
-    __syncthreads();
-    CV_STAMP_AT(6)
-    cv_conv_layer<3, 1, 64, 64, 8, 3, true>(bufA, bufA, P.wt[6], P.bias[6], w, true);
+    if (W24 && f24_6) {
+        if constexpr (W24) {
+            cw_layer<10, 12, CW_CS3, 4, 128, 1, 1, 0, 8, CW_CS5, false>(bufA, P.wt[5], P.bias[5], w, 0);
+            __syncthreads();
+            CV_STAMP_AT(6)
+            cw_layer<8, 8, CW_CS5, 3, 64, 1, 1, 0, 0, CV_C64, true>(bufA, f24[2], P.bias[6], w, 0);
+        }
+    } else {
+        cw_layer<10, 12, CW_CS3, 4, 128, 1, 1, 0, 0, CV_C64, true>(bufA, P.wt[5], P.bias[5], w, 0);
+        __syncthreads();
+        CV_STAMP_AT(6)
+        cv_conv_layer<3, 1, 64, 64, 8, 3, true>(bufA, bufA, P.wt[6], P.bias[6], w, true);
+    }
     __syncthreads();
     CV_STAMP_AT(7)
     float* hop1 = lds + 4096;
@@ -441,11 +473,9 @@
     return layer >= 0 && layer <= 5 ? group[layer] : 0;
 }
 
-static int cost_net_launch(const float* s_eq, const float* t_eq, int m, const float* const* wt_host, const float* const* bias_host,
-                           const long long* s_rows, const long long* t_rows, int ele_n, float* ind_out, void* stream, const char* who,
-                           const int* only_if = nullptr)
-{
-    CostNetParams P;
+static int cost_net_params(CostNetParams& P, const float* const* wt_host, const float* const* bias_host, const long long* s_rows,
+                           const long long* t_rows, int ele_n, const int* only_if, const char* who)
+{
     for (int l = 0; l < CV_LAYERS; l++) {
         P.wt[l] = wt_host[l]; P.bias[l] = bias_host[l];
         BUF_REQUIRE(P.wt[l] && P.bias[l], BUF_EINVAL, "%s: null weights for layer %d", who, l);
@@ -455,25 +485,23 @@
     P.row_floats = 32 * P.chan_floats;
     P.skip_floats = s_rows ? 20 : 0;
     P.only_if = only_if;
-    size_t lds = sizeof(float) * CV_BUF;
-    static LdsGrant grant, grant_rerun;
-    if (int rc = only_if ? grant_dynamic_lds((const void*)k_cost_net_rerun, lds, grant_rerun) : grant_dynamic_lds((const void*)k_cost_net, lds, grant)) return rc;
-    static const double macs_per_match =
-        60.0 * 480 * 32 + 54.0 * 288 * 32 + 16.0 * 64 * 96 * 64 +
-        16.0 * (49.0 * 64 * 64 + 36.0 * 64 * 128 + 25.0 * 128 * 128 + 16.0 * 128 * 64) +
-        36.0 * 576 * 64 + 16.0 * 576 * 32 + 4.0 * 288 * 32 + 1.0 * 128 * 20;
-    TimedSpan span;
-    bool timed = !only_if && timing_begin((hipStream_t)stream, &span, 2.0 * macs_per_match * m, BUF_TIMED_COST_NET);
+    return BUF_OK;
+}
+
+static const double cost_net_macs_per_match =
+    60.0 * 480 * 32 + 54.0 * 288 * 32 + 16.0 * 64 * 96 * 64 +
+    16.0 * (49.0 * 64 * 64 + 36.0 * 64 * 128 + 25.0 * 128 * 128 + 16.0 * 128 * 64) +
+    36.0 * 576 * 64 + 16.0 * 576 * 32 + 4.0 * 288 * 32 + 1.0 * 128 * 20;
+
 #ifdef CV_STAMP
-    long long* stamps = nullptr;
-    BUF_CHECK_HIP(hipMalloc(&stamps, (size_t)m * 16 * sizeof(long long)));
-    BUF_CHECK_HIP(hipMemcpyToSymbol(HIP_SYMBOL(cv_stamp_ptr), &stamps, sizeof(stamps)));
-#endif
-    if (only_if) k_cost_net_rerun<<<m, CV_THREADS, lds, (hipStream_t)stream>>>(s_eq, t_eq, P, ind_out);
-    else k_cost_net<<<m, CV_THREADS, lds, (hipStream_t)stream>>>(s_eq, t_eq, P, ind_out);
-    if (timed) timing_end((hipStream_t)stream, &span);
-    BUF_LAUNCH_CHECK();
-#ifdef CV_STAMP
+static int cv_stamp_begin(int m, long long** stamps)
+{
+    BUF_CHECK_HIP(hipMalloc(stamps, (size_t)m * 16 * sizeof(long long)));
+    BUF_CHECK_HIP(hipMemcpyToSymbol(HIP_SYMBOL(cv_stamp_ptr), stamps, sizeof(*stamps)));
+    return BUF_OK;
+}
+static int cv_stamp_end(int m, long long* stamps, void* stream, const char* kernel)
+{
     if (m >= 2048) {
         BUF_CHECK_HIP(hipStreamSynchronize((hipStream_t)stream));
         long long* h = (long long*)malloc((size_t)m * 16 * sizeof(long long));
@@ -482,10 +510,35 @@
         double d[8] = {};
         for (int b = m / 2; b < m; b++)
             for (int i = 0; i < 8; i++) d[i] += (double)(h[(size_t)b * 16 + i + 1] - h[(size_t)b * 16 + i]);
-        for (int i = 0; i < 8; i++) fprintf(stderr, "  CV_STAMP %-20s %8.0f cycles per match\n", name[i], d[i] / (m - m / 2));
+        for (int i = 0; i < 8; i++) fprintf(stderr, "  CV_STAMP %s %-20s %8.0f cycles per match\n", kernel, name[i], d[i] / (m - m / 2));
         free(h);
     }
     (void)hipFree(stamps);
+    return BUF_OK;
+}
+#endif
+
+static int cost_net_launch(const float* s_eq, const float* t_eq, int m, const float* const* wt_host, const float* const* bias_host,
+                           const long long* s_rows, const long long* t_rows, int ele_n, float* ind_out, void* stream, const char* who,
+                           const int* only_if = nullptr)
+{
+    CostNetParams P;
+    if (int rc = cost_net_params(P, wt_host, bias_host, s_rows, t_rows, ele_n, only_if, who)) return rc;
+    size_t lds = sizeof(float) * CV_BUF;
+    static LdsGrant grant, grant_rerun;
+    if (int rc = only_if ? grant_dynamic_lds((const void*)k_cost_net_rerun, lds, grant_rerun) : grant_dynamic_lds((const void*)k_cost_net, lds, grant)) return rc;
+    TimedSpan span;
+    bool timed = !only_if && timing_begin((hipStream_t)stream, &span, 2.0 * cost_net_macs_per_match * m, BUF_TIMED_COST_NET);
+#ifdef CV_STAMP
+    long long* stamps = nullptr;
+    if (int rc = cv_stamp_begin(m, &stamps)) return rc;
+#endif
+    if (only_if) k_cost_net_rerun<<<m, CV_THREADS, lds, (hipStream_t)stream>>>(s_eq, t_eq, P, ind_out);
+    else k_cost_net<<<m, CV_THREADS, lds, (hipStream_t)stream>>>(s_eq, t_eq, P, ind_out);
+    if (timed) timing_end((hipStream_t)stream, &span);
+    BUF_LAUNCH_CHECK();
+#ifdef CV_STAMP
+    if (int rc = cv_stamp_end(m, stamps, stream, "k_cost_net")) return rc;
 #endif
     return BUF_OK;
 }
diff --git a/buffer_amd/csrc/costnet_w24.hip b/buffer_amd/csrc/costnet_w24.hip
--- /dev/null
+++ b/buffer_amd/csrc/costnet_w24.hip
@@ -0,0 +1,129 @@
+#include "common.h"
+
+struct CostNetW24Params {
+    CostNetParams P;
+    const float* f24[3];
+};
+
+template <int C, int CS, int USED>
+__device__ __forceinline__ void cw24_zero_spare(float* __restrict__ map)
+{
+    static_assert(CS - USED == 16, "16 spare words per channel");
+    for (int i = threadIdx.x; i < C * 16; i += CV_THREADS) map[(i >> 4) * CS + USED + (i & 15)] = 0.f;
+}
+
+template <int HIN, int RS, int CS, int NTX, int TYPM, int CIN, int RSO, int CSO>
+__device__ __forceinline__ void cw24_layer(float* __restrict__ map, const float* __restrict__ wt, const float* __restrict__ bias, int pair, int t)
+{
+    constexpr int WOUT = HIN - 2, NTY = WOUT / 2;
+    static_assert(NTX * TYPM <= 16 && 4 * NTX >= WOUT && 4 * (NTX - 1) + 2 <= WOUT && RS % 2 == 0 && CS % 2 == 0 && RSO % 2 == 0 && CSO % 2 == 0 && CIN % 16 == 0, "");
+    static_assert((HIN - 1) * RS + 4 * (NTX - 1) + 6 <= CS, "the last window stays inside the channel");
+    constexpr unsigned KSTEP = 16u * CS;
+    constexpr int k4 = CIN / 4;
+    int lane = threadIdx.x & (WAVE - 1);
+    asm volatile("" : "+v"(lane));
+    const int lk = lane >> 4;
+    const unsigned base = (unsigned)(size_t)(__attribute__((address_space(3))) const float*)map;
+    unsigned RA[4];
+    {
+        const int li = lane & 15, q = li / NTX;
+        int ty = t * TYPM + q, tx = li - q * NTX;
+        if (!(q < TYPM && ty < NTY)) { ty = 0; tx = 0; }
+#pragma unroll
+        for (int a = 0; a < 4; a++) RA[a] = base + 4u * (unsigned)(lk * CS + (2 * ty + a) * RS + 4 * tx);
+    }
+    const __amdgpu_buffer_rsrc_t rs = wg_weights(wt);
+    const unsigned pstride = (unsigned)(k4 * W24_WSTRIDE);
+    const unsigned wp = (unsigned)pair * 4 * pstride;
+    const unsigned lofs4 = lane * 16, lofs2 = lane * 8;
+    const float* bv = bias + (2 * pair) * 16 + lk * 4;
+    wgf4 W4[2][2];
+    wgf2 W2[2][2];
+#pragma unroll
+    for (int n = 0; n < 2; n++)
+#pragma unroll
+        for (int k = 0; k < 2; k++) {
+            W4[n][k] = wg_ldw(rs, wp + k * W24_WSTRIDE + n * 256, lofs4);
+            W2[n][k] = w24_ldw2(rs, wp + k * W24_WSTRIDE + 512 + n * 128, lofs2);
+        }
+    wgf4 Y[2][2][4];
+    w24_round<false, KSTEP>(RA, rs, wp, wp, lofs4, lofs2, k4 >> 2, pstride, bv, W4, W2, Y);
+    __syncthreads();
+    int lane_s = threadIdx.x & (WAVE - 1);
+    asm volatile("" : "+v"(lane_s));
+    const int li = lane_s & 15, q = li / NTX, tx = li - q * NTX, ty = t * TYPM + q;
+    if (!(q < TYPM && ty < NTY)) return;
+    const bool wide = 4 * tx + 2 < WOUT;
+#pragma unroll
+    for (int n = 0; n < 2; n++) {
+        float* p = map + ((2 * pair + n) * 16 + (lane_s >> 4) * 4) * CSO + 2 * ty * RSO + 4 * tx;
+#pragma unroll
+        for (int u = 0; u < 2; u++)
+#pragma unroll
+            for (int r = 0; r < 4; r++) {
+                float* d = p + r * CSO + u * RSO;
+                *reinterpret_cast<wgf2*>(d) = (wgf2){ fmaxf(Y[n][u][0][r], 0.f), fmaxf(Y[n][u][1][r], 0.f) };
+                if (wide) *reinterpret_cast<wgf2*>(d + 2) = (wgf2){ fmaxf(Y[n][u][2][r], 0.f), fmaxf(Y[n][u][3][r], 0.f) };
+            }
+    }
+}
+
+__global__ void __launch_bounds__(CV_THREADS, 2) k_cost_net_w24(const float* __restrict__ s_eq, const float* __restrict__ t_eq, CostNetW24Params Q,
+                                                            float* __restrict__ ind_out)
+{
+    extern __shared__ float lds[];
+    cost_net_body<true>(s_eq, t_eq, Q.P, ind_out, lds, Q.f24);
+}
+
+__global__ void __launch_bounds__(CV_THREADS, 2) k_cost_net_w24_rerun(const float* __restrict__ s_eq, const float* __restrict__ t_eq, CostNetW24Params Q,
+                                                                  float* __restrict__ ind_out)
+{
+    extern __shared__ float lds[];
+    if (Q.P.only_if[blockIdx.x] == 0) return;
+    cost_net_body<true>(s_eq, t_eq, Q.P, ind_out, lds, Q.f24);
+}
+
+static int cost_net_w24_launch(const float* s_eq, const float* t_eq, int m, const float* const* wt_host, const float* const* bias_host,
+                               const float* const* f24_host, const long long* s_rows, const long long* t_rows, int ele_n, float* ind_out,
+                               void* stream, const char* who, const int* only_if = nullptr)
+{
+    CostNetW24Params Q;
+    if (int rc = cost_net_params(Q.P, wt_host, bias_host, s_rows, t_rows, ele_n, only_if, who)) return rc;
+    for (int i = 0; i < 3; i++) Q.f24[i] = f24_host[i];
+    size_t lds = sizeof(float) * CV_BUF;
+    static LdsGrant grant, grant_rerun;
+    if (int rc = only_if ? grant_dynamic_lds((const void*)k_cost_net_w24_rerun, lds, grant_rerun) : grant_dynamic_lds((const void*)k_cost_net_w24, lds, grant)) return rc;
+    TimedSpan span;
+    bool timed = !only_if && timing_begin((hipStream_t)stream, &span, 2.0 * cost_net_macs_per_match * m, BUF_TIMED_COST_NET);
+#ifdef CV_STAMP
+    long long* stamps = nullptr;
+    if (int rc = cv_stamp_begin(m, &stamps)) return rc;
+#endif
+    if (only_if) k_cost_net_w24_rerun<<<m, CV_THREADS, lds, (hipStream_t)stream>>>(s_eq, t_eq, Q, ind_out);
+    else k_cost_net_w24<<<m, CV_THREADS, lds, (hipStream_t)stream>>>(s_eq, t_eq, Q, ind_out);
+    if (timed) timing_end((hipStream_t)stream, &span);
+    BUF_LAUNCH_CHECK();
+#ifdef CV_STAMP
+    if (int rc = cv_stamp_end(m, stamps, stream, "k_cost_net_w24")) return rc;
+#endif
+    return BUF_OK;
+}
+
+extern "C" int buf_cost_volume_net_w24(const float* s_eq, const float* t_eq, int m, const float* const* wt_host, const float* const* bias_host,
+                                       const float* const* f24_host, float* ind_out, void* stream)
+{
+    BUF_REQUIRE(m >= 0, BUF_EINVAL, "buf_cost_volume_net_w24: m=%d", m);
+    if (m == 0) return BUF_OK;
+    BUF_REQUIRE(s_eq && t_eq && wt_host && bias_host && f24_host && ind_out, BUF_EINVAL, "buf_cost_volume_net_w24: null argument");
+    return cost_net_w24_launch(s_eq, t_eq, m, wt_host, bias_host, f24_host, nullptr, nullptr, 7, ind_out, stream, "buf_cost_volume_net_w24");
+}
+
+extern "C" int buf_cost_volume_net_w24_gather(const float* equi, int ele_n, const long long* s_rows, const long long* t_rows, int m,
+                                              const float* const* wt_host, const float* const* bias_host, const float* const* f24_host,
+                                              float* ind_out, void* stream)
+{
+    BUF_REQUIRE(m >= 0 && ele_n == 7, BUF_EINVAL, "buf_cost_volume_net_w24_gather: m=%d ele_n=%d (the kernel is built for ele_n = 7)", m, ele_n);
+    if (m == 0) return BUF_OK;
+    BUF_REQUIRE(equi && s_rows && t_rows && wt_host && bias_host && f24_host && ind_out, BUF_EINVAL, "buf_cost_volume_net_w24_gather: null argument");
+    return cost_net_w24_launch(equi, equi, m, wt_host, bias_host, f24_host, s_rows, t_rows, ele_n, ind_out, stream, "buf_cost_volume_net_w24_gather");
+}
diff --git a/buffer_amd/csrc/split_safe.hip b/buffer_amd/csrc/split_safe.hip
--- a/buffer_amd/csrc/split_safe.hip
+++ b/buffer_amd/csrc/split_safe.hip
@@ -84,3 +84,23 @@
     if (rc) return rc;
     return cost_net_launch(s_eq, t_eq, m, wt_f32_host, bias_f32_host, s_rows, t_rows, ele_n, ind_out, stream, "buf_cost_volume_net_split_safe", flags_ws);
 }
+
+extern "C" int buf_cost_volume_net_split_safe_w24(const float* s_eq, const float* t_eq, int ele_n, const long long* s_rows, const long long* t_rows,
+                                                  int m, const void* const* wt_split_host, const float* const* bias_split_host,
+                                                  const float* const* wt_f32_host, const float* const* bias_f32_host, const float* const* f24_host,
+                                                  float* ind_out, int* status_dev, int* flags_ws, void* stream)
+{
+    BUF_REQUIRE(m >= 0, BUF_EINVAL, "buf_cost_volume_net_split_safe_w24: m=%d", m);
+    if (m == 0) return BUF_OK;
+    BUF_REQUIRE(s_eq && t_eq && wt_split_host && bias_split_host && wt_f32_host && bias_f32_host && f24_host && ind_out && flags_ws, BUF_EINVAL,
+                "buf_cost_volume_net_split_safe_w24: null argument");
+    BUF_REQUIRE((s_rows == nullptr) == (t_rows == nullptr), BUF_EINVAL, "buf_cost_volume_net_split_safe_w24: one row list without the other");
+    BUF_REQUIRE(!s_rows || ele_n == 7, BUF_EINVAL, "buf_cost_volume_net_split_safe_w24: ele_n=%d (the kernels are built for ele_n = 7)", ele_n);
+    hipStream_t s = (hipStream_t)stream;
+    BUF_CHECK_HIP(hipMemsetAsync(flags_ws, 0, sizeof(int) * (size_t)m, s));
+    int rc = cost_net_h3_launch(s_eq, t_eq, m, wt_split_host, bias_split_host, s_rows, t_rows, ele_n, ind_out, status_dev, stream,
+                                "buf_cost_volume_net_split_safe_w24", flags_ws);
+    if (rc) return rc;
+    return cost_net_w24_launch(s_eq, t_eq, m, wt_f32_host, bias_f32_host, f24_host, s_rows, t_rows, ele_n, ind_out, stream,
+                               "buf_cost_volume_net_split_safe_w24", flags_ws);
+}
diff --git a/buffer_amd/ops.py b/buffer_amd/ops.py
--- a/buffer_amd/ops.py
+++ b/buffer_amd/ops.py
@@ -1095,10 +1095,42 @@
     return ws.reshape(-1, cout).astype(np.float32), wt.reshape(-1, cout).astype(np.float32)
 
 
+COST_F24_DEFAULT = 'all'
+COST_F24_PARTS = {'all': (2, 4, 6), 'l2': (2,), 'l4': (4,), 'l6': (6,), 'off': (), None: ()}
+
+
+def cost_f24_parts(f24):
+    if f24 is None:
+        f24 = COST_F24_DEFAULT
+    if f24 is True:
+        f24 = 'all'
+    if f24 is False:
+        f24 = 'off'
+    if f24 not in COST_F24_PARTS:
+        raise ValueError(f"f24 = {f24!r}: one of 'all', 'l2', 'l4', 'l6', 'off'")
+    return COST_F24_PARTS[f24]
+
+
+def cost_f24_filters(layers, parts):
+    sets = []
+    for l in (2, 4, 6):
+        if l not in parts:
+            sets.append(None)
+            continue
+        w = layers[l][0]
+        assert tuple(w.shape[2:]) == (3, 1, 3), w.shape
+        w2d = np.ascontiguousarray(w[:, :, :, 0, :])
+        sets.append(winograd_tile_weights(w2d, ng=1) if l == 6 else winograd_f24_tile_weights(w2d))
+    return sets
+
+
 class CostVolumeNet:
 
-    def __init__(self, layers, device):
+    def __init__(self, layers, device, f24=None):
         assert len(layers) == 10
+        self.parts = cost_f24_parts(f24)
+        self.wt24 = [None if a is None else torch.from_numpy(a).to(device) for a in cost_f24_filters(layers, self.parts)]
+        self._fp = (C.c_void_p * 3)(*[None if t is None else t.data_ptr() for t in self.wt24])
         self.wt, self.bias = [], []
         for i, (w, b) in enumerate(layers):
             cout, cin = w.shape[0], w.shape[1]
@@ -1135,6 +1167,10 @@
         s_eq, t_eq = s_eq.contiguous(), t_eq.contiguous()
         m = s_eq.shape[0]
         out = torch.empty((m,), dtype=torch.float32, device=s_eq.device)
+        if self.parts:
+            check(L.buf_cost_volume_net_w24(_ptr(s_eq), _ptr(t_eq), m, self._wp, self._bp, self._fp, _ptr(out), _stream()),
+                  "buf_cost_volume_net_w24")
+            return out
         check(L.buf_cost_volume_net(_ptr(s_eq), _ptr(t_eq), m, self._wp, self._bp, _ptr(out), _stream()),
               "buf_cost_volume_net")
         return out
@@ -1147,6 +1183,10 @@
         s_rows, t_rows = _dev(s_rows, torch.int64, "s_rows"), _dev(t_rows, torch.int64, "t_rows")
         m = int(s_rows.shape[0])
         out = torch.empty((m,), dtype=torch.float32, device=equi.device)
+        if self.parts:
+            check(L.buf_cost_volume_net_w24_gather(_ptr(equi), 7, _ptr(s_rows), _ptr(t_rows), m, self._wp, self._bp, self._fp, _ptr(out),
+                                                   _stream()), "buf_cost_volume_net_w24_gather")
+            return out
         check(L.buf_cost_volume_net_gather(_ptr(equi), 7, _ptr(s_rows), _ptr(t_rows), m, self._wp, self._bp, _ptr(out), _stream()),
               "buf_cost_volume_net_gather")
         return out
@@ -1154,8 +1194,9 @@
 
 class CostVolumeNetSplit:
 
-    def __init__(self, layers, device):
+    def __init__(self, layers, device, f24=None):
         assert len(layers) == 10
+        self.parts = cost_f24_parts(f24)
         mats = []
         w0 = layers[0][0]
         assert tuple(w0.shape) == (32, 32, 3, 3, 3), w0.shape
@@ -1183,13 +1224,18 @@
         self._wp = (C.c_void_p * 11)(*[t.data_ptr() for t in self.wt])
         self._bp = (C.c_void_p * 10)(*[t.data_ptr() for t in self.bias])
         self.safe = not os.environ.get('BUF_SPLIT_UNSAFE')
-        self.f32 = CostVolumeNet(layers, device) if self.safe else None
+        self.f32 = CostVolumeNet(layers, device, f24=f24) if self.safe else None
         self.last_flags = None
 
     def _safe(self, s_eq, t_eq, s_rows, t_rows, m, dev):
         L = _lib.lib()
         out = torch.empty((m,), dtype=torch.float32, device=dev)
         self.last_flags = torch.empty((max(m, 1),), dtype=torch.int32, device=dev)
+        if self.parts:
+            check(L.buf_cost_volume_net_split_safe_w24(_ptr(s_eq), _ptr(t_eq), 7, _ptr(s_rows), _ptr(t_rows), m, self._wp, self._bp, self.f32._wp,
+                                                       self.f32._bp, self.f32._fp, _ptr(out), _ptr(self.status), _ptr(self.last_flags), _stream()),
+                  "buf_cost_volume_net_split_safe_w24")
+            return out
         check(L.buf_cost_volume_net_split_safe(_ptr(s_eq), _ptr(t_eq), 7, _ptr(s_rows), _ptr(t_rows), m, self._wp, self._bp, self.f32._wp,
                                                self.f32._bp, _ptr(out), _ptr(self.status), _ptr(self.last_flags), _stream()),
               "buf_cost_volume_net_split_safe")
diff --git a/buffer_amd/registration.py b/buffer_amd/registration.py
--- a/buffer_amd/registration.py
+++ b/buffer_amd/registration.py
@@ -6,7 +6,7 @@
 
 class CostVolume:
 
-    def __init__(self, W, device, azi_n=20, arith='f32'):
+    def __init__(self, W, device, azi_n=20, arith='f32', f24=None):
         if arith not in ('f32', 'split'):
             raise ValueError(f"cnn_arith must be 'f32' or 'split', got {arith!r}")
         if azi_n != 20:
@@ -17,7 +17,7 @@
         for i, bn in ((0, 1), (3, 4), (6, 7), (9, 10), (12, 13), (15, 16), (18, 19), (21, 22), (24, 25)):
             layers.append(_fold_bn(W[f'{p}.{i}.weight'], W[f'{p}.{i}.bias'], W[f'{p}.{bn}.running_mean'], W[f'{p}.{bn}.running_var']))
         layers.append((np.asarray(W[f'{p}.27.weight'], np.float32), np.asarray(W[f'{p}.27.bias'], np.float32)))
-        self.fused = ops.CostVolumeNetSplit(layers, device) if arith == 'split' else ops.CostVolumeNet(layers, device)
+        self.fused = ops.CostVolumeNetSplit(layers, device, f24=f24) if arith == 'split' else ops.CostVolumeNet(layers, device, f24=f24)
 
     def __call__(self, d1, d2):
         if tuple(d1.shape[1:]) != (32, 5, 20) or d1.shape != d2.shape:
diff --git a/include/buffer_hip.h b/include/buffer_hip.h
--- a/include/buffer_hip.h
+++ b/include/buffer_hip.h
@@ -191,6 +191,11 @@
                             const float* const* bias_host, float* ind_out, void* stream);
 int     buf_cost_volume_net_gather(const float* equi, int ele_n, const long long* s_rows, const long long* t_rows, int m,
                                    const float* const* wt_host, const float* const* bias_host, float* ind_out, void* stream);
+int     buf_cost_volume_net_w24(const float* s_eq, const float* t_eq, int m, const float* const* wt_host, const float* const* bias_host,
+                                const float* const* f24_host, float* ind_out, void* stream);
+int     buf_cost_volume_net_w24_gather(const float* equi, int ele_n, const long long* s_rows, const long long* t_rows, int m,
+                                       const float* const* wt_host, const float* const* bias_host, const float* const* f24_host,
+                                       float* ind_out, void* stream);
 
 long long buf_split_gemm_count(int cout, int cin, int ntaps, int nt);
 int     buf_split_tile_gemm(const float* w_host, int cout, int cin, int ntaps, int nt, unsigned short* out_host);
@@ -203,6 +208,10 @@
                                        int m, const void* const* wt_split_host, const float* const* bias_split_host,
                                        const float* const* wt_f32_host, const float* const* bias_f32_host, float* ind_out,
                                        int* status_dev, int* flags_ws, void* stream);
+int     buf_cost_volume_net_split_safe_w24(const float* s_eq, const float* t_eq, int ele_n, const long long* s_rows, const long long* t_rows,
+                                           int m, const void* const* wt_split_host, const float* const* bias_split_host,
+                                           const float* const* wt_f32_host, const float* const* bias_f32_host, const float* const* f24_host,
+                                           float* ind_out, int* status_dev, int* flags_ws, void* stream);
 
 int     buf_hypotheses_score(const float* ind, const float* ss_kpts, const float* tt_kpts, const float* ss_R,
                              const float* tt_R, int m, int azi_n, float inlier_th, float* R_out, float* t_out,
```

Result: faster. 175.8 (median of 6 runs) (+1.2%).
